# eaton-lab/tetrad

Hardware: AMD Instinct MI355X
Metric: resolved quartets/sec (whole node) (higher is better)
Workload: dtype u8 scan / u32 counts / f64 SVD; 1 GPU; c3: 128 taxa x 50000 SNPs, 1000000 random quartets, subsample_snps=True, results delivered to host arrays inside the step; quartets=1000000, taxa=128, snps=50000, subsample_snps=True, parallelism=one GPU, result D2H overlapped inside tq_resolve_to_host, launcher=none (one process)

## Files before the change

include/tetrad_hip.h:

```cpp
#ifndef TETRAD_HIP_H
#define TETRAD_HIP_H

#include <stdint.h>

#ifdef __cplusplus
extern "C" {
#endif

typedef struct tq_ctx tq_ctx;

enum {
    TQ_OK = 0,
    TQ_ERR_INVALID_ARG = -1,
    TQ_ERR_NO_DEVICE = -2,
    TQ_ERR_HIP = -3,
    TQ_ERR_NO_DATA = -4,
    TQ_ERR_LOCUS_ORDER = -5,
    TQ_ERR_OOM = -6
};

enum {
    TQ_FLAG_ZERO_DATA = 1,
    TQ_FLAG_DEGENERATE = 2,
    TQ_FLAG_BAD_INDEX = 4,
    TQ_FLAG_NO_CONVERGENCE = 8,
    TQ_FLAG_INVALID_DIAGNOSTIC = 16
};

int tq_create(tq_ctx **out, int device_id);
void tq_destroy(tq_ctx *ctx);
const char *tq_last_error(const tq_ctx *ctx);

int tq_set_data(tq_ctx *ctx, const uint8_t *tmparr, int64_t T, int64_t S,
                const uint32_t *locus, int64_t locus_stride);

int tq_set_source(tq_ctx *ctx, const uint8_t *seqarr, int64_t T, int64_t S0,
                  const int64_t *spans, int64_t nloci);
int tq_bootstrap(tq_ctx *ctx, const int64_t *lidxs, int64_t n, uint64_t seed_shuffle,
                 uint64_t seed_ambig, int64_t *out_S);
int tq_bootstrap_async(tq_ctx *ctx, const int64_t *lidxs, int64_t n, uint64_t seed_shuffle,
                       uint64_t seed_ambig, int64_t *out_S, void *stream);
int tq_get_data(tq_ctx *ctx, uint8_t *tmparr, uint32_t *tmpmap);
int tq_data_shape(tq_ctx *ctx, int64_t *T, int64_t *S);

int tq_resolve(tq_ctx *ctx, const uint32_t *quartets, int64_t Q, int subsample,
               uint32_t *rstat, double *rscor, uint8_t *flags);

int tq_host_alloc(int64_t bytes, void **out);
int tq_host_free(void *p);

int tq_resolve_to_host(tq_ctx *ctx, const uint32_t *d_quartets, int64_t Q, int subsample,
                       uint32_t *rstat, double *rscor, uint8_t *flags);

int tq_resolve_dev(tq_ctx *ctx, const uint32_t *d_quartets, int64_t Q, int subsample,
                   uint32_t *d_rstat, double *d_rscor, uint8_t *d_flags, void *stream);

int tq_resolve_range_dev(tq_ctx *ctx, uint64_t first_rank, int64_t Q, int subsample,
                         uint32_t *d_quartets, uint32_t *d_rstat, double *d_rscor,
                         uint8_t *d_flags, void *stream);

int tq_scan_dev(tq_ctx *ctx, const uint32_t *d_quartets, int64_t Q, int subsample, void *stream);
int tq_svd_dev(tq_ctx *ctx, int64_t q0, int64_t n, uint32_t *d_rstat, double *d_rscor,
               uint8_t *d_flags, void *stream);

int tq_unrank_dev(tq_ctx *ctx, const uint64_t *d_ranks, int64_t Q, uint32_t *d_quartets,
                  void *stream);

int tq_sample_quartets_dev(tq_ctx *ctx, uint64_t seed, int64_t Q, uint64_t *d_ranks,
                           uint32_t *d_quartets, void *stream);

int tq_resolve_debug(tq_ctx *ctx, const uint32_t *quartets, int64_t Q, int subsample,
                     uint32_t *rstat, double *rscor, uint8_t *flags,
                     uint32_t *cmats, double *svds, int32_t *ranks);

int tq_timing_enable(tq_ctx *ctx, int on);
int tq_timing_read(tq_ctx *ctx, double *kernel_ms, int64_t *launches);
int tq_timing_read_split(tq_ctx *ctx, double *total_ms, double *scan_ms, double *svd_ms, int64_t *calls);
int tq_timing_read_kernels(tq_ctx *ctx, double *ms, int n_ms, int64_t *calls);

int tq_set_option(tq_ctx *ctx, const char *name, int64_t value);

int tq_debug_fetch(tq_ctx *ctx, int which, void *dst, int64_t bytes);

int tq_debug_bdsqr(tq_ctx *ctx, const double *de, int64_t nmat, double *sv, uint32_t *work, int reps, double *ms);

int tq_format_tsv(const uint32_t *quartets, const uint32_t *rstat, const double *rscor, int64_t Q,
                  char *out, int64_t cap, int64_t *written);
int tq_format_qmc(const uint32_t *quartets, const uint32_t *rstat, const double *rscor, int64_t Q,
                  int weights, int64_t min_snps, double min_ratio, char *out, int64_t cap,
                  int64_t *written, int64_t *n_lines);

int tq_numpy_choice_tail(void *np_bitgen, uint64_t pop, int64_t size, int64_t *out);

int tq_unrank(const uint64_t *ranks, uint64_t first_rank, int64_t Q, int64_t T, uint32_t *quartets);

int tq_qmc_splits(const uint32_t *quartets, const uint32_t *rstat, const double *rscor, int64_t Q, int weights,
                  int64_t min_snps, double min_ratio, uint32_t *splits, double *weights_out, int64_t *n_rows);

int tq_qmc_tree(const uint32_t *splits, const double *weights, int64_t n, int64_t ntaxa, uint64_t seed,
                char *out, int64_t cap, int64_t *written);

typedef struct tq_conc tq_conc;
int tq_conc_create(tq_conc **out, const int32_t *parent, int64_t n_nodes, int64_t T, int64_t min_snps, double min_ratio,
                   tq_ctx *ctx);
void tq_conc_destroy(tq_conc *acc);
int tq_conc_reset(tq_conc *acc);
int tq_conc_add(tq_conc *acc, const uint32_t *quartets, const uint32_t *rstat, const double *rscor, const uint8_t *flags,
                int64_t n);
int tq_conc_add_dev(tq_conc *acc, const uint32_t *d_quartets, const uint32_t *d_rstat, const double *d_rscor,
                    const uint8_t *d_flags, int64_t n, void *stream);
int tq_conc_shape(const tq_conc *acc, int64_t *T, int64_t *n_edges, int64_t *mask_words);
int tq_conc_read(tq_conc *acc, int64_t *edge_counts, double *edge_sums, uint64_t *masks, int64_t *tip_counts,
                 int64_t *skipped);

typedef struct tq_stree tq_stree;
int tq_stree_create(tq_stree **out, int64_t ntaxa, int64_t capacity_rows, int weights, int64_t min_snps, double min_ratio,
                    tq_ctx *ctx);
void tq_stree_destroy(tq_stree *acc);
int tq_stree_reset(tq_stree *acc);
int tq_stree_add(tq_stree *acc, const uint32_t *quartets, const uint32_t *rstat, const double *rscor, const uint8_t *flags,
                 int64_t n);
int tq_stree_add_dev(tq_stree *acc, const uint32_t *d_quartets, const uint32_t *d_rstat, const double *d_rscor,
                     const uint8_t *d_flags, int64_t n, void *stream);
int tq_stree_graph(tq_stree *acc, uint64_t *G, uint64_t *B, int64_t *kept, int64_t *skipped, uint64_t *sum_k);
int tq_stree_rows(tq_stree *acc, uint32_t *splits, uint64_t *k, int64_t *n);
int tq_stree_build(tq_stree *acc, uint64_t seed, void *stream, char *out, int64_t cap, int64_t *written, int64_t *levels);
int tq_stree_level_stats(const tq_stree *acc, int64_t *n_levels, double *out);

int tq_set_species(tq_ctx *ctx, const int32_t *species_of, int64_t T, int64_t K);
int tq_resolve_species(tq_ctx *ctx, const uint32_t *squartets, int64_t Q, uint32_t *rstat, double *rscor,
                       uint8_t *flags);
int tq_resolve_species_dev(tq_ctx *ctx, const uint32_t *d_squartets, int64_t Q, uint32_t *d_rstat, double *d_rscor,
                           uint8_t *d_flags, void *stream);
int tq_resolve_species_debug(tq_ctx *ctx, const uint32_t *squartets, int64_t Q, uint32_t *rstat, double *rscor,
                             uint8_t *flags, uint32_t *cmats, double *svds, int32_t *ranks);

int tq_device_info(tq_ctx *ctx, int32_t *num_cu, int32_t *waves_per_cu, int64_t *row_pitch);

#ifdef __cplusplus
}
#endif
#endif
```

tetrad_amd/_lib.py:

```python
from __future__ import annotations

import ctypes
import os
import sys
import shutil
import subprocess
from pathlib import Path

CSRC = Path(__file__).resolve().parent / "csrc"
LIB_PATH = CSRC / "libtetrad_hip.so"
SRC_PATH = CSRC / "tetrad_hip.hip"
HEADER = Path(__file__).resolve().parents[1] / "include" / "tetrad_hip.h"

TQ_OK = 0
ERR_NAMES = {
    -1: "TQ_ERR_INVALID_ARG", -2: "TQ_ERR_NO_DEVICE", -3: "TQ_ERR_HIP",
    -4: "TQ_ERR_NO_DATA", -5: "TQ_ERR_LOCUS_ORDER", -6: "TQ_ERR_OOM",
}
FLAG_ZERO_DATA, FLAG_DEGENERATE, FLAG_BAD_INDEX, FLAG_NO_CONVERGENCE, FLAG_INVALID_DIAGNOSTIC = 1, 2, 4, 8, 16

SYMBOLS = [
    "tq_create", "tq_destroy", "tq_last_error", "tq_set_data", "tq_resolve",
    "tq_set_source", "tq_bootstrap", "tq_bootstrap_async", "tq_sample_quartets_dev", "tq_get_data", "tq_data_shape",
    "tq_host_alloc", "tq_host_free", "tq_resolve_to_host", "tq_scan_dev", "tq_svd_dev",
    "tq_resolve_dev", "tq_resolve_range_dev", "tq_unrank_dev", "tq_resolve_debug",
    "tq_timing_enable", "tq_timing_read", "tq_timing_read_split", "tq_timing_read_kernels",
    "tq_set_option", "tq_device_info", "tq_debug_fetch", "tq_debug_bdsqr",
    "tq_format_tsv", "tq_format_qmc", "tq_qmc_tree", "tq_qmc_splits", "tq_unrank", "tq_numpy_choice_tail",
    "tq_conc_create", "tq_conc_destroy", "tq_conc_reset", "tq_conc_add", "tq_conc_add_dev", "tq_conc_shape", "tq_conc_read",
    "tq_stree_create", "tq_stree_destroy", "tq_stree_reset", "tq_stree_add", "tq_stree_add_dev", "tq_stree_graph",
    "tq_stree_rows", "tq_stree_build", "tq_stree_level_stats",
    "tq_set_species", "tq_resolve_species", "tq_resolve_species_dev", "tq_resolve_species_debug",
]


class TetradHipError(RuntimeError):
    def __init__(self, code: int, message: str):
        self.code = code
        super().__init__(f"{ERR_NAMES.get(code, code)}: {message}")


def build(force: bool = False, verbose: bool = False) -> Path:
    hipcc = shutil.which("hipcc") or "/opt/rocm/bin/hipcc"
    sources = [SRC_PATH, HEADER, *CSRC.glob("*.hpp")]
    newest_src = max(p.stat().st_mtime for p in sources)
    if not force and LIB_PATH.exists() and LIB_PATH.stat().st_mtime >= newest_src:
        return LIB_PATH
    cmd = [hipcc, "-O3", "-std=c++17", "--offload-arch=gfx950", "-fPIC", "-shared", "-Wno-inline-asm",
           "-o", str(LIB_PATH), str(SRC_PATH)]
    if verbose:
        print(" ".join(cmd))
    subprocess.check_call(cmd)
    _stamp_commit()
    return LIB_PATH


def _stamp_commit() -> None:
    repo = CSRC.parents[1]
    try:
        head = subprocess.check_output(["git", "-C", str(repo), "rev-parse", "--short", "HEAD"],
                                       stderr=subprocess.DEVNULL).decode().strip()
        dirty = subprocess.check_output(["git", "-C", str(repo), "status", "--porcelain", "--untracked-files=no"],
                                        stderr=subprocess.DEVNULL).decode().strip()
        (repo / ".build_commit").write_text(head + ("+uncommitted" if dirty else "") + "\n")
    except Exception:
        pass


_lib = None
LOADED_PATH = None


def load() -> ctypes.CDLL:
    global _lib
    if _lib is not None:
        return _lib
    if not LIB_PATH.exists():
        raise ImportError(
            f"{LIB_PATH} is missing: run `python -c 'import __graft_entry__ as g; g.build()'` "
            "(hipcc, gfx950).  tetrad_amd has no CPU fallback.")
    try:
        import torch
    except ImportError:
        pass
    alt = os.environ.get("TQ_LIB_PATH")
    if alt:
        print(f"tetrad_amd: TQ_LIB_PATH is set -- loading {alt} instead of {LIB_PATH}", file=sys.stderr)
    global LOADED_PATH
    LOADED_PATH = alt if alt else str(LIB_PATH)
    lib = ctypes.CDLL(LOADED_PATH)
    c = ctypes
    vp, i64, i32 = c.c_void_p, c.c_int64, c.c_int
    lib.tq_create.argtypes = [c.POINTER(vp), i32]
    lib.tq_create.restype = i32
    lib.tq_destroy.argtypes = [vp]
    lib.tq_destroy.restype = None
    lib.tq_last_error.argtypes = [vp]
    lib.tq_last_error.restype = c.c_char_p
    lib.tq_set_data.argtypes = [vp, vp, i64, i64, vp, i64]
    lib.tq_set_data.restype = i32
    lib.tq_set_source.argtypes = [vp, vp, i64, i64, vp, i64]
    lib.tq_set_source.restype = i32
    lib.tq_bootstrap.argtypes = [vp, vp, i64, c.c_uint64, c.c_uint64, c.POINTER(i64)]
    lib.tq_bootstrap.restype = i32
    lib.tq_bootstrap_async.argtypes = [vp, vp, i64, c.c_uint64, c.c_uint64, c.POINTER(i64), vp]
    lib.tq_bootstrap_async.restype = i32
    lib.tq_sample_quartets_dev.argtypes = [vp, c.c_uint64, i64, vp, vp, vp]
    lib.tq_sample_quartets_dev.restype = i32
    lib.tq_get_data.argtypes = [vp, vp, vp]
    lib.tq_get_data.restype = i32
    lib.tq_data_shape.argtypes = [vp, c.POINTER(i64), c.POINTER(i64)]
    lib.tq_data_shape.restype = i32
    lib.tq_resolve.argtypes = [vp, vp, i64, i32, vp, vp, vp]
    lib.tq_resolve.restype = i32
    lib.tq_host_alloc.argtypes = [i64, c.POINTER(vp)]
    lib.tq_host_alloc.restype = i32
    lib.tq_host_free.argtypes = [vp]
    lib.tq_host_free.restype = i32
    lib.tq_resolve_to_host.argtypes = [vp, vp, i64, i32, vp, vp, vp]
    lib.tq_resolve_to_host.restype = i32
    lib.tq_scan_dev.argtypes = [vp, vp, i64, i32, vp]
    lib.tq_scan_dev.restype = i32
    lib.tq_svd_dev.argtypes = [vp, i64, i64, vp, vp, vp, vp]
    lib.tq_svd_dev.restype = i32
    lib.tq_timing_read_kernels.argtypes = [vp, c.POINTER(c.c_double), i32, c.POINTER(i64)]
    lib.tq_timing_read_kernels.restype = i32
    lib.tq_resolve_dev.argtypes = [vp, vp, i64, i32, vp, vp, vp, vp]
    lib.tq_resolve_dev.restype = i32
    lib.tq_resolve_range_dev.argtypes = [vp, c.c_uint64, i64, i32, vp, vp, vp, vp, vp]
    lib.tq_resolve_range_dev.restype = i32
    lib.tq_unrank_dev.argtypes = [vp, vp, i64, vp, vp]
    lib.tq_unrank_dev.restype = i32
    lib.tq_resolve_debug.argtypes = [vp, vp, i64, i32, vp, vp, vp, vp, vp, vp]
    lib.tq_resolve_debug.restype = i32
    lib.tq_timing_enable.argtypes = [vp, i32]
    lib.tq_timing_enable.restype = i32
    lib.tq_timing_read.argtypes = [vp, c.POINTER(c.c_double), c.POINTER(i64)]
    lib.tq_timing_read.restype = i32
    lib.tq_timing_read_split.argtypes = [vp, c.POINTER(c.c_double), c.POINTER(c.c_double),
                                         c.POINTER(c.c_double), c.POINTER(i64)]
    lib.tq_timing_read_split.restype = i32
    lib.tq_debug_fetch.argtypes = [vp, i32, vp, i64]
    lib.tq_debug_fetch.restype = i32
    lib.tq_debug_bdsqr.argtypes = [vp, vp, i64, vp, vp, i32, c.POINTER(c.c_double)]
    lib.tq_debug_bdsqr.restype = i32
    lib.tq_set_option.argtypes = [vp, c.c_char_p, i64]
    lib.tq_set_option.restype = i32
    lib.tq_format_tsv.argtypes = [vp, vp, vp, i64, vp, i64, c.POINTER(i64)]
    lib.tq_format_tsv.restype = i32
    lib.tq_format_qmc.argtypes = [vp, vp, vp, i64, i32, i64, c.c_double, vp, i64, c.POINTER(i64), c.POINTER(i64)]
    lib.tq_format_qmc.restype = i32
    lib.tq_qmc_splits.argtypes = [vp, vp, vp, i64, i32, i64, c.c_double, vp, vp, c.POINTER(i64)]
    lib.tq_qmc_splits.restype = i32
    lib.tq_numpy_choice_tail.argtypes = [vp, c.c_uint64, i64, vp]
    lib.tq_numpy_choice_tail.restype = i32
    lib.tq_unrank.argtypes = [vp, c.c_uint64, i64, i64, vp]
    lib.tq_unrank.restype = i32
    lib.tq_qmc_tree.argtypes = [vp, vp, i64, i64, c.c_uint64, vp, i64, c.POINTER(i64)]
    lib.tq_qmc_tree.restype = i32
    lib.tq_conc_create.argtypes = [c.POINTER(vp), vp, i64, i64, i64, c.c_double, vp]
    lib.tq_conc_create.restype = i32
    lib.tq_conc_destroy.argtypes = [vp]
    lib.tq_conc_destroy.restype = None
    lib.tq_conc_reset.argtypes = [vp]
    lib.tq_conc_reset.restype = i32
    lib.tq_conc_add.argtypes = [vp, vp, vp, vp, vp, i64]
    lib.tq_conc_add.restype = i32
    lib.tq_conc_add_dev.argtypes = [vp, vp, vp, vp, vp, i64, vp]
    lib.tq_conc_add_dev.restype = i32
    lib.tq_conc_shape.argtypes = [vp, c.POINTER(i64), c.POINTER(i64), c.POINTER(i64)]
    lib.tq_conc_shape.restype = i32
    lib.tq_conc_read.argtypes = [vp, vp, vp, vp, vp, c.POINTER(i64)]
    lib.tq_conc_read.restype = i32
    lib.tq_stree_create.argtypes = [c.POINTER(vp), i64, i64, i32, i64, c.c_double, vp]
    lib.tq_stree_create.restype = i32
    lib.tq_stree_destroy.argtypes = [vp]
    lib.tq_stree_destroy.restype = None
    lib.tq_stree_reset.argtypes = [vp]
    lib.tq_stree_reset.restype = i32
    lib.tq_stree_add.argtypes = [vp, vp, vp, vp, vp, i64]
    lib.tq_stree_add.restype = i32
    lib.tq_stree_add_dev.argtypes = [vp, vp, vp, vp, vp, i64, vp]
    lib.tq_stree_add_dev.restype = i32
    lib.tq_stree_graph.argtypes = [vp, vp, vp, c.POINTER(i64), c.POINTER(i64), c.POINTER(c.c_uint64)]
    lib.tq_stree_graph.restype = i32
    lib.tq_stree_rows.argtypes = [vp, vp, vp, c.POINTER(i64)]
    lib.tq_stree_rows.restype = i32
    lib.tq_stree_build.argtypes = [vp, c.c_uint64, vp, vp, i64, c.POINTER(i64), c.POINTER(i64)]
    lib.tq_stree_build.restype = i32
    lib.tq_stree_level_stats.argtypes = [vp, c.POINTER(i64), vp]
    lib.tq_stree_level_stats.restype = i32
    lib.tq_set_species.argtypes = [vp, vp, i64, i64]
    lib.tq_set_species.restype = i32
    lib.tq_resolve_species.argtypes = [vp, vp, i64, vp, vp, vp]
    lib.tq_resolve_species.restype = i32
    lib.tq_resolve_species_dev.argtypes = [vp, vp, i64, vp, vp, vp, vp]
    lib.tq_resolve_species_dev.restype = i32
    lib.tq_resolve_species_debug.argtypes = [vp, vp, i64, vp, vp, vp, vp, vp, vp]
    lib.tq_resolve_species_debug.restype = i32
    lib.tq_device_info.argtypes = [vp, c.POINTER(c.c_int32), c.POINTER(c.c_int32), c.POINTER(i64)]
    lib.tq_device_info.restype = i32
    _lib = lib
    return lib
```

tetrad_amd/csrc/prepare.hpp:

```cpp
#pragma once

__device__ __forceinline__ void store_planes3(uint32_t *planes3, uint32_t *runbeg, int64_t t, int64_t W, int64_t w,
                                              uint32_t mm, uint32_t b0, uint32_t b1, uint32_t rb)
{
    uint32_t *p3 = planes3 + (t * W + w) * 3;
    p3[0] = mm;
    p3[1] = b0;
    p3[2] = b1;
    if (t == 0) runbeg[w] = rb;
}

__global__ void tq_prepare_rows(const uint8_t *__restrict__ raw, const uint32_t *__restrict__ locus,
                                int64_t S, int64_t Sp, int64_t W, int32_t T, uint8_t *__restrict__ rows,
                                uint8_t *__restrict__ nib, uint8_t *__restrict__ nib5, uint4 *__restrict__ planes,
                                uint32_t *__restrict__ planes3, uint32_t *__restrict__ runbeg)
{
    int64_t gid = (int64_t)blockIdx.x * blockDim.x + threadIdx.x;
    if (gid >= (int64_t)T * W) return;
    int64_t t = gid / W, w = gid - t * W;
    const uint8_t *src = raw + t * S + w * 32;
    uint8_t *dst = rows + t * Sp;
    uint32_t mm = 0, b0 = 0, b1 = 0, rb = 0;
    uint32_t nw[4] = {0, 0, 0, 0}, n5[4] = {0, 0, 0, 0};
    for (int i = 0; i < 32; ++i) {
        int64_t s = w * 32 + i;
        uint8_t v = (s < S) ? src[i] : (uint8_t)0xFF;
        bool missing = v > 3;
        uint8_t code = missing ? (uint8_t)0 : v;
        dst[row_offset(s)] = code;
        nw[i >> 3] |= (uint32_t)code << (8 * (i & 3) + 4 * ((i >> 2) & 1));
        n5[i >> 3] |= (uint32_t)(missing ? 4 : code) << (8 * (i & 3) + 4 * ((i >> 2) & 1));
        mm |= (uint32_t)missing << i;
        b0 |= (uint32_t)(code & 1) << i;
        b1 |= (uint32_t)((code >> 1) & 1) << i;
        if (s < S) {
            bool beg = (s == 0) || (locus[s] != locus[s - 1]);
            rb |= (uint32_t)beg << i;
        }
    }
    planes[t * W + w] = make_uint4(mm, b0, b1, rb);
    store_planes3(planes3, runbeg, t, W, w, mm, b0, b1, rb);
    reinterpret_cast<uint4 *>(nib + t * (Sp / 2))[w] = make_uint4(nw[0], nw[1], nw[2], nw[3]);
    reinterpret_cast<uint4 *>(nib5 + t * (Sp / 2))[w] = make_uint4(n5[0], n5[1], n5[2], n5[3]);
}

__device__ __forceinline__ uint64_t choose_k(uint64_t n, int k)
{
    switch (k) {
    case 0: return 1;
    case 1: return n;
    case 2: return n < 2 ? 0 : n * (n - 1) / 2;
    default: return n < 3 ? 0 : n * (n - 1) / 2 * (n - 2) / 3;
    }
}

__global__ void tq_unrank_kernel(const uint64_t *__restrict__ ranks, uint64_t first_rank, int64_t Q,
                                 int32_t T, uint32_t *__restrict__ quartets)
{
    int64_t i = (int64_t)blockIdx.x * blockDim.x + threadIdx.x;
    if (i >= Q) return;
    uint64_t index = ranks ? ranks[i] : first_rank + (uint64_t)i;
    uint32_t out[4] = {0, 0, 0, 0};
    int nsel = 0;
    for (int t = 0; t < T && nsel < 4; ++t) {
        uint64_t c = choose_k((uint64_t)(T - t - 1), 4 - nsel - 1);
        if (c > index) {
            out[nsel++] = (uint32_t)t;
        } else {
            index -= c;
        }
    }
    uint4 v = make_uint4(out[0], out[1], out[2], out[3]);
    reinterpret_cast<uint4 *>(quartets)[i] = v;
}

__global__ void tq_key_kernel(const uint32_t *__restrict__ quartets, int64_t Q, uint32_t T, int with_c,
                              uint32_t *__restrict__ keys, uint32_t *__restrict__ idx)
{
    int64_t i = (int64_t)blockIdx.x * blockDim.x + threadIdx.x;
    if (i >= Q) return;
    const uint4 q = reinterpret_cast<const uint4 *>(quartets)[i];
    const uint32_t a = q.x < T ? q.x : T - 1, b = q.y < T ? q.y : T - 1, c = q.z < T ? q.z : T - 1;
    const uint32_t ab = a * T + b;
    keys[i] = with_c ? ab * T + c : ab;
    idx[i] = (uint32_t)i;
}


__device__ __forceinline__ uint32_t feistel_round(uint32_t x, uint32_t key)
{
    x ^= key;
    x *= 0x7FEB352Du;
    x ^= x >> 15;
    x *= 0x846CA68Bu;
    x ^= x >> 16;
    return x;
}

struct FeistelKeys {
    uint32_t k[6];
};

__device__ __forceinline__ FeistelKeys feistel_keys(uint64_t seed)
{
    FeistelKeys ks;
    uint64_t x = seed;
#pragma unroll
    for (int r = 0; r < 6; ++r) {
        x += 0x9E3779B97F4A7C15ull;
        uint64_t z = x;
        z = (z ^ (z >> 30)) * 0xBF58476D1CE4E5B9ull;
        z = (z ^ (z >> 27)) * 0x94D049BB133111EBull;
        z ^= z >> 31;
        ks.k[r] = (uint32_t)(z >> 16);
    }
    return ks;
}

__device__ __forceinline__ uint64_t feistel_permute(uint64_t v, int half_bits, const FeistelKeys &ks)
{
    const uint32_t mask = half_bits >= 32 ? 0xFFFFFFFFu : ((1u << half_bits) - 1u);
    uint32_t L = (uint32_t)(v >> half_bits) & mask, R = (uint32_t)v & mask;
#pragma unroll
    for (int r = 0; r < 6; ++r) {
        const uint32_t t = L ^ (feistel_round(R, ks.k[r]) & mask);
        L = R;
        R = t;
    }
    return ((uint64_t)L << half_bits) | (uint64_t)R;
}

__global__ void tq_sample_kernel(uint64_t seed, uint64_t N, int half_bits, int64_t Q, int32_t T,
                                 uint64_t *__restrict__ ranks_out, uint32_t *__restrict__ quartets)
{
    int64_t i = (int64_t)blockIdx.x * blockDim.x + threadIdx.x;
    if (i >= Q) return;
    const FeistelKeys ks = feistel_keys(seed);
    uint64_t v = (uint64_t)i;
    do {
        v = feistel_permute(v, half_bits, ks);
    } while (v >= N);
    if (ranks_out) ranks_out[i] = v;
    uint64_t index = v;
    uint32_t out[4] = {0, 0, 0, 0};
    int nsel = 0;
    for (int t = 0; t < T && nsel < 4; ++t) {
        uint64_t c = choose_k((uint64_t)(T - t - 1), 4 - nsel - 1);
        if (c > index) {
            out[nsel++] = (uint32_t)t;
        } else {
            index -= c;
        }
    }
    reinterpret_cast<uint4 *>(quartets)[i] = make_uint4(out[0], out[1], out[2], out[3]);
}
```

tetrad_amd/csrc/tetrad_hip.hip:

```cpp
#include <hip/hip_runtime.h>
#include <hipcub/hipcub.hpp>

#include <algorithm>
#include <chrono>
#include <cmath>
#include <cstdarg>
#include <cstdlib>
#include <utility>
#include <cstdint>
#include <cstdio>
#include <cstring>
#include <map>
#include <mutex>
#include <new>
#include <string>
#include <unordered_map>
#include <unordered_set>
#include <vector>

#include "../../include/tetrad_hip.h"

namespace {

#include "common.hpp"
#include "prepare.hpp"
#include "scan.hpp"
#include "scan_pb.hpp"
#include "scan_dp.hpp"
#include "scan_f4.hpp"
#include "jacobi.hpp"
#include "hqr.hpp"
#include "bootstrap.hpp"
#include "format.hpp"
#include "qmc.hpp"
#include "concordance.hpp"
#include "species.hpp"
#include "supertree.hpp"

}

enum { TAG_ORIGIN = -1, TAG_ORDER = 0, TAG_SCAN = 1, TAG_BIDIAG = 2, TAG_BDSQR = 3, TAG_SCORE = 4, TAG_COUNT = 5 };

struct tq_ctx {
    int device = 0;
    std::string err;
    hipDeviceProp_t prop{};
    int64_t T = 0, S = 0, Sp = 0, W = 0;
    uint8_t *d_rows = nullptr;
    uint8_t *d_nib = nullptr;
    uint8_t *d_nib5 = nullptr;
    uint4 *d_planes = nullptr;
    uint32_t *d_planes3 = nullptr;
    bool have_data = false;
    bool locus_runs_ok = false;
    int64_t plane_cap_W = 0;
    int64_t data_capacity = 0;
    uint8_t *d_seqarr = nullptr;
    int64_t *d_spans = nullptr;
    int64_t src_T = 0, src_S0 = 0, nloci = 0, max_width = 0;
    int64_t *d_lidxs = nullptr;
    std::vector<int64_t> h_spans;
    int64_t *h_lidx_stage[2] = {nullptr, nullptr};
    hipEvent_t ev_lidx[2] = {nullptr, nullptr};
    unsigned lidx_turn = 0;
    uint32_t *d_boot = nullptr;
    int64_t boot_cap = 0;
    void *d_boot_tmp = nullptr;
    size_t boot_tmp_bytes = 0;
    void *d_scratch = nullptr;
    size_t scratch_bytes = 0;
    uint32_t *d_cm = nullptr;
    int64_t cm_quartets = 0;
    uint32_t *d_sort = nullptr;
    void *d_sort_tmp = nullptr;
    size_t sort_tmp_bytes = 0;
    int order = 1;
    uint2 *d_units = nullptr;
    int scan_f4 = -1;
    int scan_dp = 1;
    int64_t dp_min_quartets = 32768;
    double *d_de = nullptr, *d_sv = nullptr;
    uint32_t *d_nsnps = nullptr;
    int64_t svd_quartets = 0;
    int64_t svd_chunk = 1 << 18;
    int svd_streams = 2;
    hipStream_t sX = nullptr;
    hipEvent_t evFork = nullptr, evJoin = nullptr;
    int svd_method = 1;
    int bidiag_layout = 1;
    int bdsqr_maxit = 60;
    uint64_t *d_bdsqr_stats = nullptr;
    int scan_wg = 4;
    int64_t wg_min_quartets = 4096;
    int xcd_remap = 1;
    int count_invariant = 0;
    int scan_pair = 0;
    int park_t = 1;
    int share_c = 0;
    int svd_wpc = 0;
    int stree_lds = 1;
    const uint32_t *scanned_q = nullptr;
    int64_t scanned_Q = 0;
    int64_t scanned_T = 0;
    int64_t sp_T = 0, sp_K = 0;
    std::vector<int32_t> sp_size;
    uint64_t sp_bound = 0;
    int32_t sp_max = 0;
    int32_t *d_sp_members = nullptr;
    uint32_t *d_sp_tab = nullptr;
    int64_t sp_tab_cap = 0;
    int species_method = -1;
    uint64_t data_gen = 0;
    uint64_t sp_tab_gen = ~0ull;
    hipStream_t sK = nullptr, sC = nullptr;
    std::vector<hipEvent_t> pipe_events;
    hipEvent_t evDevApi = nullptr;
    bool dev_api_pending = false;
    hipStream_t last_dev_stream = nullptr;
    int nrep = 1;
    int waves_per_cu = 0;
    int phases = 3;
    int scan_method = -1;
    int pb_ok = 0;
    int64_t batch = 1 << 23;
    bool timing = false;
    struct Mark { int tag; int lane; hipEvent_t ev; };
    std::vector<Mark> marks;
    std::vector<hipEvent_t> event_pool;
    int64_t timed_calls = 0;
};

namespace {

std::string g_create_err;

int fail(tq_ctx *ctx, int code, const char *fmt, ...)
{
    char buf[512];
    va_list ap;
    va_start(ap, fmt);
    vsnprintf(buf, sizeof buf, fmt, ap);
    va_end(ap);
    try {
        if (ctx) ctx->err = buf; else g_create_err = buf;
    } catch (...) {
    }
    return code;
}

#define TQ_HIP(ctx, call)                                                                     \
    do {                                                                                      \
        hipError_t e_ = (call);                                                               \
        if (e_ != hipSuccess)                                                                 \
            return fail(ctx, e_ == hipErrorOutOfMemory ? TQ_ERR_OOM : TQ_ERR_HIP, "%s failed: %s", \
                        #call, hipGetErrorString(e_));                                        \
    } while (0)

struct PinnedPool {
    std::mutex mu;
    std::map<uintptr_t, size_t> live;
    std::multimap<size_t, void *> idle;
    size_t idle_bytes = 0;
    static constexpr size_t IDLE_CAP = (size_t)4 << 30;
    static size_t round_up(size_t b)
    {
        size_t g = (size_t)1 << 16;
        while (g < b && g < ((size_t)1 << 24)) g <<= 1;
        if (g >= b) return g;
        const size_t step = (size_t)1 << 24;
        return (b + step - 1) / step * step;
    }
    int alloc(size_t bytes, void **out)
    {
        const size_t want = round_up(bytes ? bytes : 1);
        std::lock_guard<std::mutex> g(mu);
        try {
            auto it = idle.lower_bound(want);
            if (it != idle.end() && it->first <= want * 2) {
                void *p = it->second;
                const size_t sz = it->first;
                idle.erase(it);
                idle_bytes -= sz;
                live[(uintptr_t)p] = sz;
                *out = p;
                return TQ_OK;
            }
            void *p = nullptr;
            if (hipHostMalloc(&p, want, hipHostMallocPortable) != hipSuccess || !p) return TQ_ERR_OOM;
            live[(uintptr_t)p] = want;
            *out = p;
            return TQ_OK;
        } catch (...) {
            return TQ_ERR_OOM;
        }
    }
    int release(void *p)
    {
        std::lock_guard<std::mutex> g(mu);
        auto it = live.find((uintptr_t)p);
        if (it == live.end()) return TQ_ERR_INVALID_ARG;
        const size_t sz = it->second;
        live.erase(it);
        bool cached = false;
        if (idle_bytes + sz <= IDLE_CAP) {
            try {
                idle.emplace(sz, p);
                idle_bytes += sz;
                cached = true;
            } catch (...) {
            }
        }
        if (!cached) (void)hipHostFree(p);
        return TQ_OK;
    }
    bool owns(const void *p, size_t bytes)
    {
        std::lock_guard<std::mutex> g(mu);
        auto it = live.upper_bound((uintptr_t)p);
        if (it == live.begin()) return false;
        --it;
        return (uintptr_t)p + bytes <= it->first + it->second;
    }
};

PinnedPool &pool()
{
    static PinnedPool *p = new PinnedPool();
    return *p;
}

bool is_pinned(const void *p, size_t bytes)
{
    if (!p) return false;
    if (pool().owns(p, bytes)) return true;
    hipPointerAttribute_t a{};
    if (hipPointerGetAttributes(&a, p) != hipSuccess) {
        (void)hipGetLastError();
        return false;
    }
    return a.type == hipMemoryTypeHost;
}

void free_data(tq_ctx *ctx)
{
    if (ctx->d_rows) (void)hipFree(ctx->d_rows);
    if (ctx->d_nib) (void)hipFree(ctx->d_nib);
    if (ctx->d_nib5) (void)hipFree(ctx->d_nib5);
    if (ctx->d_planes) (void)hipFree(ctx->d_planes);
    if (ctx->d_planes3) (void)hipFree(ctx->d_planes3);
    ctx->d_rows = nullptr;
    ctx->d_nib = nullptr;
    ctx->d_nib5 = nullptr;
    ctx->d_planes = nullptr;
    ctx->d_planes3 = nullptr;
    ctx->have_data = false;
    ctx->data_capacity = 0;
    ctx->scanned_Q = 0;
}

void free_source(tq_ctx *ctx)
{
    if (ctx->d_seqarr) (void)hipFree(ctx->d_seqarr);
    if (ctx->d_spans) (void)hipFree(ctx->d_spans);
    if (ctx->d_lidxs) (void)hipFree(ctx->d_lidxs);
    if (ctx->d_boot) (void)hipFree(ctx->d_boot);
    if (ctx->d_boot_tmp) (void)hipFree(ctx->d_boot_tmp);
    ctx->d_seqarr = nullptr;
    ctx->d_spans = nullptr;
    ctx->d_lidxs = nullptr;
    ctx->d_boot = nullptr;
    ctx->d_boot_tmp = nullptr;
    ctx->boot_cap = 0;
    ctx->nloci = 0;
    for (int i = 0; i < 2; ++i) {
        if (ctx->h_lidx_stage[i]) (void)pool().release(ctx->h_lidx_stage[i]);
        if (ctx->ev_lidx[i]) (void)hipEventDestroy(ctx->ev_lidx[i]);
        ctx->h_lidx_stage[i] = nullptr;
        ctx->ev_lidx[i] = nullptr;
    }
}

int ensure_scratch(tq_ctx *ctx, size_t bytes)
{
    if (bytes <= ctx->scratch_bytes) return TQ_OK;
    if (ctx->d_scratch) (void)hipFree(ctx->d_scratch);
    ctx->d_scratch = nullptr;
    ctx->scratch_bytes = 0;
    TQ_HIP(ctx, hipMalloc(&ctx->d_scratch, bytes));
    ctx->scratch_bytes = bytes;
    return TQ_OK;
}

int ensure_cm(tq_ctx *ctx, int64_t quartets)
{
    if (quartets <= ctx->cm_quartets) return TQ_OK;
    if (ctx->d_cm) (void)hipFree(ctx->d_cm);
    if (ctx->d_sort) (void)hipFree(ctx->d_sort);
    if (ctx->d_sort_tmp) (void)hipFree(ctx->d_sort_tmp);
    if (ctx->d_units) (void)hipFree(ctx->d_units);
    ctx->d_cm = nullptr;
    ctx->d_sort = nullptr;
    ctx->d_sort_tmp = nullptr;
    ctx->d_units = nullptr;
    ctx->cm_quartets = 0;
    ctx->scanned_Q = 0;
    TQ_HIP(ctx, hipMalloc((void **)&ctx->d_cm, (size_t)quartets * 1024));
    TQ_HIP(ctx, hipMalloc((void **)&ctx->d_sort, (size_t)quartets * 16));
    size_t tmp = 0;
    uint32_t *k = ctx->d_sort;
    TQ_HIP(ctx, hipcub::DeviceRadixSort::SortPairs(nullptr, tmp, k, k, k, k, (int)quartets));
    size_t tmp2 = 0;
    TQ_HIP(ctx, hipcub::DeviceScan::InclusiveSum(nullptr, tmp2, k, k, (int)quartets));
    if (tmp2 > tmp) tmp = tmp2;
    TQ_HIP(ctx, hipMalloc(&ctx->d_sort_tmp, tmp ? tmp : 16));
    TQ_HIP(ctx, hipMalloc((void **)&ctx->d_units, ((size_t)quartets + 2) * sizeof(uint2)));
    ctx->sort_tmp_bytes = tmp;
    ctx->cm_quartets = quartets;
    return TQ_OK;
}

int ensure_svd(tq_ctx *ctx, int64_t quartets)
{
    if (!ctx->sX) {
        TQ_HIP(ctx, hipStreamCreateWithFlags(&ctx->sX, hipStreamNonBlocking));
        TQ_HIP(ctx, hipEventCreateWithFlags(&ctx->evFork, hipEventDisableTiming));
        TQ_HIP(ctx, hipEventCreateWithFlags(&ctx->evJoin, hipEventDisableTiming));
    }
    if (quartets <= ctx->svd_quartets) return TQ_OK;
    if (ctx->d_de) (void)hipFree(ctx->d_de);
    if (ctx->d_sv) (void)hipFree(ctx->d_sv);
    if (ctx->d_nsnps) (void)hipFree(ctx->d_nsnps);
    ctx->d_de = ctx->d_sv = nullptr;
    ctx->d_nsnps = nullptr;
    ctx->svd_quartets = 0;
    TQ_HIP(ctx, hipMalloc((void **)&ctx->d_de, 2 * (size_t)quartets * 3 * 32 * sizeof(double)));
    TQ_HIP(ctx, hipMalloc((void **)&ctx->d_sv, 2 * (size_t)quartets * 3 * 16 * sizeof(double)));
    TQ_HIP(ctx, hipMalloc((void **)&ctx->d_nsnps, 2 * (size_t)quartets * sizeof(uint32_t)));
    ctx->svd_quartets = quartets;
    return TQ_OK;
}

int mark(tq_ctx *ctx, int tag, hipStream_t stream, int lane = 0)
{
    if (!ctx->timing) return TQ_OK;
    hipEvent_t ev;
    if (!ctx->event_pool.empty()) {
        ev = ctx->event_pool.back();
        ctx->event_pool.pop_back();
    } else {
        TQ_HIP(ctx, hipEventCreate(&ev));
    }
    try {
        ctx->marks.push_back({tag, lane, ev});
    } catch (...) {
        (void)hipEventDestroy(ev);
        return fail(ctx, TQ_ERR_OOM, "out of host memory");
    }
    TQ_HIP(ctx, hipEventRecord(ev, stream));
    return TQ_OK;
}

int make_order(tq_ctx *ctx, const uint32_t *dq, int64_t n, bool input_sorted, hipStream_t stream,
               const uint32_t **order)
{
    *order = nullptr;
    if (!ctx->order || n < 32768 || ctx->T > 65535 || input_sorted) return TQ_OK;
    uint32_t *keys_in = ctx->d_sort, *idx_in = keys_in + ctx->cm_quartets;
    uint32_t *keys_out = idx_in + ctx->cm_quartets, *idx_out = keys_out + ctx->cm_quartets;
    const uint64_t T = (uint64_t)ctx->T;
    const int with_c = T * T * T <= 0xFFFFFFFFull;
    hipLaunchKernelGGL(tq_key_kernel, dim3((unsigned)((n + 255) / 256)), dim3(256), 0, stream, dq, n,
                       (uint32_t)ctx->T, with_c, keys_in, idx_in);
    TQ_HIP(ctx, hipGetLastError());
    int bits = 1;
    while (bits < 32 && (1ull << bits) < (with_c ? T * T * T : T * T)) ++bits;
    size_t tmp = ctx->sort_tmp_bytes;
    TQ_HIP(ctx, hipcub::DeviceRadixSort::SortPairs(ctx->d_sort_tmp, tmp, keys_in, keys_out, idx_in, idx_out, (int)n,
                                                   0, bits, stream));
    *order = idx_out;
    return TQ_OK;
}

bool use_dp(const tq_ctx *ctx, int64_t n, int subsample, bool input_sorted)
{
    const uint64_t T = (uint64_t)ctx->T;
    return !subsample && ctx->scan_dp && ctx->scan_f4 <= 0 && ctx->scan_method < 0 && ctx->scan_wg == 4 && !ctx->count_invariant &&
           !ctx->share_c && !ctx->scan_pair && ctx->waves_per_cu == 0 && (ctx->order || input_sorted) &&
           n >= ctx->dp_min_quartets && n >= 2 && n <= 0x7FFFFFFF && T * T * T <= 0xFFFFFFFFull &&
           T * (uint64_t)ctx->Sp < 0xFFFF0000ull;
}

int make_units(tq_ctx *ctx, const uint32_t *dq, int64_t n, bool input_sorted, hipStream_t stream)
{
    uint32_t *keys_in = ctx->d_sort, *idx_in = keys_in + ctx->cm_quartets;
    uint32_t *keys_out = idx_in + ctx->cm_quartets, *idx_out = keys_out + ctx->cm_quartets;
    const uint64_t T = (uint64_t)ctx->T;
    const unsigned blocks = (unsigned)((n + 255) / 256);
    hipLaunchKernelGGL(tq_key_kernel, dim3(blocks), dim3(256), 0, stream, dq, n, (uint32_t)ctx->T, 1, keys_in, idx_in);
    TQ_HIP(ctx, hipGetLastError());
    const uint32_t *keys = keys_in, *idx = idx_in;
    uint32_t *flags = keys_out;
    if (!input_sorted) {
        int bits = 1;
        while (bits < 32 && (1ull << bits) < T * T * T) ++bits;
        size_t tmp = ctx->sort_tmp_bytes;
        TQ_HIP(ctx, hipcub::DeviceRadixSort::SortPairs(ctx->d_sort_tmp, tmp, keys_in, keys_out, idx_in, idx_out, (int)n,
                                                       0, bits, stream));
        keys = keys_out;
        idx = idx_out;
        flags = keys_in;
    }
    hipLaunchKernelGGL(tq_dp_flag_kernel, dim3(blocks), dim3(256), 0, stream, keys, idx, dq, n, (uint32_t)ctx->T, flags);
    TQ_HIP(ctx, hipGetLastError());
    size_t tmp = ctx->sort_tmp_bytes;
    TQ_HIP(ctx, hipcub::DeviceScan::InclusiveSum(ctx->d_sort_tmp, tmp, flags, flags, (int)n, stream));
    hipLaunchKernelGGL(tq_dp_units_kernel, dim3(blocks), dim3(256), 0, stream, keys, idx, (const uint32_t *)flags, n,
                       ctx->d_units, reinterpret_cast<uint32_t *>(ctx->d_units + ctx->cm_quartets));
    TQ_HIP(ctx, hipGetLastError());
    return TQ_OK;
}

DevData dev_data(const tq_ctx *ctx)
{
    DevData d;
    d.rows = ctx->d_rows;
    d.nib = ctx->d_nib;
    d.nib5 = ctx->d_nib5;
    d.planes = ctx->d_planes;
    d.planes3 = ctx->d_planes3;
    d.runbeg = ctx->d_planes3 + (size_t)ctx->T * (size_t)ctx->plane_cap_W * 3;
    d.pitch = ctx->Sp;
    d.W = ctx->W;
    d.T = (int32_t)ctx->T;
    d.ntiles = (int32_t)(ctx->Sp / TILE);
    d.inv = ctx->count_invariant ? 0xFFFFFFFFu : 0u;
    return d;
}

template <typename K>
int grid_for(tq_ctx *ctx, K kern, int64_t items, int64_t *grid, int wpc_kernel = 0)
{
    int wpc = wpc_kernel > 0 ? wpc_kernel : ctx->waves_per_cu;
    if (wpc <= 0) {
        int nb = 0;
        TQ_HIP(ctx, hipOccupancyMaxActiveBlocksPerMultiprocessor(&nb, kern, WAVE, 0));
        wpc = nb > 0 ? nb : 8;
    }
    int64_t g = (int64_t)ctx->prop.multiProcessorCount * wpc;
    if (g > items) g = items;
    if (g < 1) g = 1;
    *grid = g;
    return TQ_OK;
}

template <int NREP, bool SUB, int METHOD>
int launch_scan(tq_ctx *ctx, const uint32_t *dq, const uint32_t *order, int64_t Q, hipStream_t stream)
{
    auto kern = tq_scan_kernel<NREP, SUB, METHOD>;
    int64_t grid;
    int rc = grid_for(ctx, kern, Q, &grid);
    if (rc) return rc;
    hipLaunchKernelGGL(kern, dim3((unsigned)grid), dim3(WAVE), 0, stream, dev_data(ctx), dq, order, Q, ctx->d_cm);
    TQ_HIP(ctx, hipGetLastError());
    return TQ_OK;
}

template <bool SUB, int METHOD, int NW, bool SHC = false, bool PARK_T = false>
int launch_scan_wg(tq_ctx *ctx, const uint32_t *dq, const uint32_t *order, int64_t Q, hipStream_t stream)
{
    auto kern = tq_scan_wg_kernel<SUB, METHOD, NW, SHC, PARK_T>;
    const int wgs = ctx->waves_per_cu > 0 ? (ctx->waves_per_cu + NW - 1) / NW : 0;
    const int64_t nblk = (Q + NW - 1) / NW;
    int64_t grid = wgs > 0 ? (int64_t)ctx->prop.multiProcessorCount * wgs : nblk;
    int64_t xcd_chunk = 0;
    if (grid >= nblk) {
        grid = nblk;
        if (ctx->xcd_remap && nblk >= 64) {
            xcd_chunk = (nblk + 7) / 8;
            grid = xcd_chunk * 8;
        }
    }
    if (grid < 1) grid = 1;
    hipLaunchKernelGGL(kern, dim3((unsigned)grid), dim3(NW * WAVE), 0, stream, dev_data(ctx), dq, order, Q,
                       ctx->d_cm, xcd_chunk);
    TQ_HIP(ctx, hipGetLastError());
    return TQ_OK;
}

template <bool SUB>
int launch_scan_pb(tq_ctx *ctx, const uint32_t *dq, const uint32_t *order, int64_t Q, hipStream_t stream)
{
    auto kern = tq_scan_pb_kernel<SUB>;
    const int64_t nblk = (Q + PB_NW - 1) / PB_NW;
    int64_t grid = nblk, xcd_chunk = 0;
    if (ctx->xcd_remap && nblk >= 64) {
        xcd_chunk = (nblk + 7) / 8;
        grid = xcd_chunk * 8;
    }
    if (grid < 1) grid = 1;
    hipLaunchKernelGGL(kern, dim3((unsigned)grid), dim3(PB_NW * WAVE), 0, stream, dev_data(ctx), dq, order, Q, ctx->d_cm,
                       xcd_chunk, (uint32_t *)nullptr);
    TQ_HIP(ctx, hipGetLastError());
    return TQ_OK;
}

int probe_scan_pb(tq_ctx *ctx)
{
    uint32_t *d = nullptr, h[2] = {0, 0};
    TQ_HIP(ctx, hipMalloc(&d, sizeof h));
    hipError_t e = hipMemset(d, 0, sizeof h);
    if (e == hipSuccess) {
        DevData none{};
        hipLaunchKernelGGL(tq_scan_pb_kernel<false>, dim3(1), dim3(PB_NW * WAVE), 0, 0, none, (const uint32_t *)nullptr,
                           (const uint32_t *)nullptr, (int64_t)-1, (uint32_t *)nullptr, (int64_t)0, d);
        hipLaunchKernelGGL(tq_scan_pb_kernel<true>, dim3(1), dim3(PB_NW * WAVE), 0, 0, none, (const uint32_t *)nullptr,
                           (const uint32_t *)nullptr, (int64_t)-1, (uint32_t *)nullptr, (int64_t)0, d + 1);
        e = hipGetLastError();
    }
    if (e == hipSuccess) e = hipMemcpy(h, d, sizeof h, hipMemcpyDeviceToHost);
    (void)hipFree(d);
    if (e != hipSuccess) return fail(ctx, TQ_ERR_HIP, "probe of tq_scan_pb_kernel failed: %s", hipGetErrorString(e));
    ctx->pb_ok = (h[0] == 0x80000000u && h[1] == 0x80000000u) ? 1 : -1;
    return TQ_OK;
}

template <bool SUB, int METHOD, int NW>
int launch_scan_wg2(tq_ctx *ctx, const uint32_t *dq, const uint32_t *order, int64_t Q, hipStream_t stream)
{
    auto kern = tq_scan_wg2_kernel<SUB, METHOD, NW>;
    const int64_t nblk = (Q + 2 * NW - 1) / (2 * NW);
    int64_t grid = nblk, xcd_chunk = 0;
    if (ctx->xcd_remap && nblk >= 64) {
        xcd_chunk = (nblk + 7) / 8;
        grid = xcd_chunk * 8;
    }
    if (grid < 1) grid = 1;
    hipLaunchKernelGGL(kern, dim3((unsigned)grid), dim3(NW * WAVE), 0, stream, dev_data(ctx), dq, order, Q, ctx->d_cm,
                       xcd_chunk);
    TQ_HIP(ctx, hipGetLastError());
    return TQ_OK;
}

int launch_scan_dp(tq_ctx *ctx, const uint32_t *dq, int64_t Q, hipStream_t stream)
{
    const int64_t least = ((Q + 1) / 2 + DP_NW - 1) / DP_NW;
    const int64_t grid = (least + 7) / 8 * 8;
    hipLaunchKernelGGL(tq_scan_dp_kernel<DP_NW>, dim3((unsigned)grid), dim3(DP_NW * WAVE), 0, stream, dev_data(ctx), dq,
                       (const uint2 *)ctx->d_units, reinterpret_cast<const uint32_t *>(ctx->d_units + ctx->cm_quartets),
                       ctx->d_cm);
    TQ_HIP(ctx, hipGetLastError());
    return TQ_OK;
}

int launch_scan_n(tq_ctx *ctx, const uint32_t *dq, const uint32_t *order, int64_t Q, int subsample,
                  hipStream_t stream)
{
    if (ctx->scan_pair && ctx->scan_wg == 4 && Q >= 64 && !ctx->count_invariant && !ctx->share_c && ctx->waves_per_cu == 0 &&
        ctx->scan_method < 2 && (uint64_t)ctx->T * (uint64_t)ctx->Sp < 0xFFFF0000ull) {
        const int m = ctx->scan_method < 0 ? (subsample ? 1 : 0) : ctx->scan_method;
        if (subsample)
            return m ? launch_scan_wg2<true, 1, 4>(ctx, dq, order, Q, stream) : launch_scan_wg2<true, 0, 4>(ctx, dq, order, Q, stream);
        return m ? launch_scan_wg2<false, 1, 4>(ctx, dq, order, Q, stream) : launch_scan_wg2<false, 0, 4>(ctx, dq, order, Q, stream);
    }
    const bool f4 = ctx->scan_f4 < 0 ? (subsample != 0 && ctx->scan_method < 0 && ctx->park_t) : ctx->scan_f4 != 0;
    if (f4 && (ctx->scan_wg == 4 || ctx->scan_wg == 8 || ctx->scan_wg == 2) && Q >= ctx->wg_min_quartets && !ctx->count_invariant &&
        !ctx->share_c && !ctx->scan_pair && ctx->waves_per_cu == 0 && (ctx->scan_method < 0 || ctx->scan_method == 1) &&
        (uint64_t)ctx->T * (uint64_t)ctx->Sp < 0xFFFF0000ull) {
        const int nw = ctx->scan_wg;
        const int64_t nblk = (Q + nw - 1) / nw;
        int64_t grid = nblk, xcd_chunk = 0;
        if (ctx->xcd_remap && nblk >= 64) {
            xcd_chunk = (nblk + 7) / 8;
            grid = xcd_chunk * 8;
        }
#define TQ_F4_CASE(SUBF, NWF)                                                                                         \
        if ((subsample != 0) == SUBF && nw == NWF)                                                                    \
            hipLaunchKernelGGL((tq_scan_f4_kernel<SUBF, NWF>), dim3((unsigned)grid), dim3(NWF * WAVE), 0, stream,      \
                               dev_data(ctx), dq, order, Q, ctx->d_cm, xcd_chunk);
        TQ_F4_CASE(true, 4) TQ_F4_CASE(false, 4) TQ_F4_CASE(true, 8) TQ_F4_CASE(false, 8) TQ_F4_CASE(true, 2) TQ_F4_CASE(false, 2)
#undef TQ_F4_CASE
        TQ_HIP(ctx, hipGetLastError());
        return TQ_OK;
    }
    const bool pb_fits = ctx->pb_ok == 1 && ctx->scan_wg == 4 && Q >= 64 && !ctx->count_invariant && !ctx->share_c &&
                         !ctx->scan_pair && ctx->waves_per_cu == 0 && ctx->Sp / TILE <= PB_MAX_TILES &&
                         (uint64_t)ctx->T * (uint64_t)ctx->Sp < 0xFFFF0000ull;
    if (pb_fits && ctx->scan_method == 6)
        return subsample ? launch_scan_pb<true>(ctx, dq, order, Q, stream) : launch_scan_pb<false>(ctx, dq, order, Q, stream);
    if (ctx->scan_wg >= 2 && Q >= ctx->wg_min_quartets && !ctx->count_invariant &&
        (uint64_t)ctx->T * (uint64_t)ctx->Sp < 0xFFFF0000ull) {
        int m = ctx->scan_method < 0 ? (subsample ? 1 : 0) : ctx->scan_method;
        if (m == 6) m = subsample ? 1 : 0;
#define TQ_WG_CASE(NW)                                                                                   \
    if (ctx->scan_wg == NW) {                                                                            \
        if (m == 2) return launch_scan_wg<true, 2, NW>(ctx, dq, order, Q, stream);                       \
        if (m == 3) return launch_scan_wg<true, 3, NW>(ctx, dq, order, Q, stream);                       \
        if (NW == 4 && m == 4) return launch_scan_wg<true, 4, 4>(ctx, dq, order, Q, stream);             \
        if (NW == 4 && m == 5) return launch_scan_wg<true, 5, 4>(ctx, dq, order, Q, stream);             \
        if (subsample)                                                                                   \
            return m ? launch_scan_wg<true, 1, NW>(ctx, dq, order, Q, stream)                            \
                     : launch_scan_wg<true, 0, NW>(ctx, dq, order, Q, stream);                           \
        return m ? launch_scan_wg<false, 1, NW>(ctx, dq, order, Q, stream)                               \
                 : launch_scan_wg<false, 0, NW>(ctx, dq, order, Q, stream);                              \
    }
        TQ_WG_CASE(2)
        if (ctx->scan_wg == 4 && ctx->park_t && m == 1 && !ctx->share_c)
            return subsample ? launch_scan_wg<true, 1, 4, false, true>(ctx, dq, order, Q, stream)
                             : launch_scan_wg<false, 1, 4, false, true>(ctx, dq, order, Q, stream);
        if ((ctx->scan_wg == 8 || ctx->scan_wg == 6) && ctx->park_t && m == 1 && subsample && !ctx->share_c)
            return ctx->scan_wg == 8 ? launch_scan_wg<true, 1, 8, false, true>(ctx, dq, order, Q, stream)
                                     : launch_scan_wg<true, 1, 6, false, true>(ctx, dq, order, Q, stream);
        if (ctx->scan_wg == 4 && ctx->share_c && m <= 1) {
            if (subsample)
                return m ? launch_scan_wg<true, 1, 4, true>(ctx, dq, order, Q, stream)
                         : launch_scan_wg<true, 0, 4, true>(ctx, dq, order, Q, stream);
            return m ? launch_scan_wg<false, 1, 4, true>(ctx, dq, order, Q, stream)
                     : launch_scan_wg<false, 0, 4, true>(ctx, dq, order, Q, stream);
        }
        TQ_WG_CASE(4)
        TQ_WG_CASE(3)
        TQ_WG_CASE(6)
        TQ_WG_CASE(16)
        TQ_WG_CASE(8)
#undef TQ_WG_CASE
    }
#define TQ_SCAN_CASE(N)                                                                              \
    case N:                                                                                          \
        if (method == 0)                                                                             \
            return subsample ? launch_scan<N, true, 0>(ctx, dq, order, Q, stream)                    \
                             : launch_scan<N, false, 0>(ctx, dq, order, Q, stream);                  \
        return subsample ? launch_scan<N, true, 1>(ctx, dq, order, Q, stream)                        \
                         : launch_scan<N, false, 1>(ctx, dq, order, Q, stream)
    const int method = (ctx->scan_method < 0 || ctx->scan_method == 6) ? (subsample ? 1 : 0) : ctx->scan_method;
    switch (ctx->nrep) {
        TQ_SCAN_CASE(2);
        TQ_SCAN_CASE(4);
        TQ_SCAN_CASE(8);
        TQ_SCAN_CASE(16);
        TQ_SCAN_CASE(32);
    default:
        TQ_SCAN_CASE(1);
    }
#undef TQ_SCAN_CASE
}

template <bool DEBUG>
int launch_svd(tq_ctx *ctx, const uint32_t *cm, const uint32_t *dq, int64_t n, const OutPtrs &out, hipStream_t stream,
               int lane)
{
    auto kern = tq_svd_kernel<DEBUG>;
    int64_t grid;
    int rc = grid_for(ctx, kern, (n + QPW - 1) / QPW, &grid);
    if (rc) return rc;
    hipLaunchKernelGGL(kern, dim3((unsigned)grid), dim3(WAVE), 0, stream, cm, dq, n, (int32_t)ctx->scanned_T, out);
    TQ_HIP(ctx, hipGetLastError());
    return mark(ctx, TAG_BIDIAG, stream, lane);
}

template <bool DEBUG>
int launch_hqr(tq_ctx *ctx, const uint32_t *cm, const uint32_t *dq, int64_t n, const OutPtrs &out, hipStream_t stream,
               int lane)
{
    double *de = ctx->d_de + (size_t)lane * (size_t)ctx->svd_quartets * 96;
    double *sv = ctx->d_sv + (size_t)lane * (size_t)ctx->svd_quartets * 48;
    uint32_t *nsnps = ctx->d_nsnps + (size_t)lane * (size_t)ctx->svd_quartets;
    int64_t grid;
    auto k1 = ctx->bidiag_layout ? tq_bidiag2_kernel<DEBUG> : tq_bidiag_kernel<DEBUG>;
    const int svd_wpc = ctx->svd_wpc > 0 ? ctx->svd_wpc : (1 << 20);
    const int tsplit = n < 32768 ? 1 : 0;
    int rc = grid_for(ctx, k1, (tsplit ? 3 : 1) * ((n + 15) / 16), &grid, svd_wpc);
    if (rc) return rc;
    hipLaunchKernelGGL(k1, dim3((unsigned)grid), dim3(WAVE), 0, stream, cm, n, de, nsnps, out.cmats, tsplit);
    TQ_HIP(ctx, hipGetLastError());
    if ((rc = mark(ctx, TAG_BIDIAG, stream, lane))) return rc;
    const int64_t nmat = 3 * n;
    rc = grid_for(ctx, tq_bdsqr_kernel, (nmat + WAVE - 1) / WAVE, &grid, svd_wpc);
    if (rc) return rc;
    hipLaunchKernelGGL(tq_bdsqr_kernel, dim3((unsigned)grid), dim3(WAVE), 0, stream, (const double *)de, nmat, sv,
                       ctx->bdsqr_maxit, (unsigned long long *)ctx->d_bdsqr_stats);
    TQ_HIP(ctx, hipGetLastError());
    if ((rc = mark(ctx, TAG_BDSQR, stream, lane))) return rc;
    hipLaunchKernelGGL(tq_score_kernel<DEBUG>, dim3((unsigned)((n + 255) / 256)), dim3(256), 0, stream,
                       (const double *)sv, (const uint32_t *)nsnps, dq, n, (int32_t)ctx->scanned_T, out);
    TQ_HIP(ctx, hipGetLastError());
    return mark(ctx, TAG_SCORE, stream, lane);
}

bool diagnostic_mode(const tq_ctx *ctx)
{
    return (ctx->scan_method >= 2 && ctx->scan_method <= 5) || ctx->phases != 3;
}

OutPtrs offset_out(const OutPtrs &o, int64_t q0)
{
    OutPtrs r = o;
    r.rstat = o.rstat + q0 * 2;
    r.rscor = o.rscor + q0 * 3;
    r.flags = o.flags ? o.flags + q0 : nullptr;
    r.cmats = o.cmats ? o.cmats + q0 * 768 : nullptr;
    r.svds = o.svds ? o.svds + q0 * 48 : nullptr;
    r.ranks = o.ranks ? o.ranks + q0 * 3 : nullptr;
    return r;
}

int check_ready(tq_ctx *ctx, int subsample)
{
    if (!ctx->have_data) return fail(ctx, TQ_ERR_NO_DATA, "tq_set_data has not been called");
    if (subsample && !ctx->locus_runs_ok)
        return fail(ctx, TQ_ERR_LOCUS_ORDER,
                    "subsample mode needs each locus id in one contiguous run of sites (and no id 0xFFFFFFFF)");
    return TQ_OK;
}

int stage_scan(tq_ctx *ctx, const uint32_t *dq, int64_t n, int subsample, bool input_sorted, hipStream_t stream)
{
    int rc = ensure_cm(ctx, n);
    if (rc) return rc;
    ctx->scanned_Q = 0;
    if ((rc = mark(ctx, TAG_ORIGIN, stream))) return rc;
    if (ctx->phases & 1) {
        if (use_dp(ctx, n, subsample, input_sorted)) {
            rc = make_units(ctx, dq, n, input_sorted, stream);
            if (rc) return rc;
            if ((rc = mark(ctx, TAG_ORDER, stream))) return rc;
            rc = launch_scan_dp(ctx, dq, n, stream);
        } else {
            const uint32_t *order = nullptr;
            rc = make_order(ctx, dq, n, input_sorted, stream, &order);
            if (rc) return rc;
            if ((rc = mark(ctx, TAG_ORDER, stream))) return rc;
            rc = launch_scan_n(ctx, dq, order, n, subsample, stream);
        }
        if (rc) return rc;
        if ((rc = mark(ctx, TAG_SCAN, stream))) return rc;
    }
    ctx->scanned_q = dq;
    ctx->scanned_Q = n;
    ctx->scanned_T = ctx->T;
    return TQ_OK;
}

int species_ready(tq_ctx *ctx, const char *who)
{
    if (!ctx->have_data) return fail(ctx, TQ_ERR_NO_DATA, "%s: tq_set_data has not been called", who);
    if (!ctx->sp_K) return fail(ctx, TQ_ERR_NO_DATA, "%s: no species map (call tq_set_species first)", who);
    if (ctx->sp_T != ctx->T)
        return fail(ctx, TQ_ERR_INVALID_ARG, "%s: the species map covers T=%lld samples, the resident replicate has T=%lld",
                    who, (long long)ctx->sp_T, (long long)ctx->T);
    if ((unsigned __int128)ctx->S * ctx->sp_bound >= ((unsigned __int128)1 << 32))
        return fail(ctx, TQ_ERR_INVALID_ARG,
                    "%s: pooled counts may exceed u32: S=%lld x product of the four largest species sizes %llu >= 2^32",
                    who, (long long)ctx->S, (unsigned long long)ctx->sp_bound);
    if (ctx->species_method == 1 && ctx->sp_max > SPECIES_MFMA_MAX)
        return fail(ctx, TQ_ERR_INVALID_ARG, "%s: species_method 1 (MFMA, i8 operands) takes species of at most %d lineages, "
                    "the map has one of %d", who, SPECIES_MFMA_MAX, (int)ctx->sp_max);
    return TQ_OK;
}

int stage_species(tq_ctx *ctx, const uint32_t *dsq, int64_t n, hipStream_t stream)
{
    int rc = ensure_cm(ctx, n);
    if (rc) return rc;
    ctx->scanned_Q = 0;
    if ((rc = mark(ctx, TAG_ORIGIN, stream))) return rc;
    if (ctx->sp_tab_gen != ctx->data_gen) {
        const int64_t entries = ctx->sp_K * ctx->Sp;
        if (entries > ctx->sp_tab_cap) {
            if (ctx->d_sp_tab) {
                TQ_HIP(ctx, hipDeviceSynchronize());
                (void)hipFree(ctx->d_sp_tab);
            }
            ctx->d_sp_tab = nullptr;
            ctx->sp_tab_cap = 0;
            TQ_HIP(ctx, hipMalloc((void **)&ctx->d_sp_tab, (size_t)entries * 8));
            ctx->sp_tab_cap = entries;
        }
        hipLaunchKernelGGL(tq_species_table_kernel, dim3((unsigned)((entries + 255) / 256)), dim3(256), 0, stream,
                           (const uint8_t *)ctx->d_nib5, ctx->Sp, ctx->S, (const int32_t *)(ctx->d_sp_members + ctx->sp_K + 1),
                           (const int32_t *)ctx->d_sp_members, (int32_t)ctx->sp_K, ctx->d_sp_tab,
                           (uint8_t *)(ctx->d_sp_tab + entries));
        TQ_HIP(ctx, hipGetLastError());
        ctx->sp_tab_gen = ctx->data_gen;
    }
    if ((rc = mark(ctx, TAG_ORDER, stream))) return rc;
    const bool mfma = ctx->species_method == 1 || (ctx->species_method < 0 && ctx->sp_max <= SPECIES_MFMA_MAX);
    const int32_t *offsets = ctx->d_sp_members;
    if (mfma)
        hipLaunchKernelGGL(tq_species_mfma_kernel, dim3((unsigned)n), dim3(WAVE * SPECIES_WAVES), 0, stream,
                           (const uint8_t *)(ctx->d_sp_tab + ctx->sp_K * ctx->Sp), ctx->Sp, ctx->S, dsq, n,
                           (int32_t)ctx->sp_K, offsets, ctx->d_cm);
    else
        hipLaunchKernelGGL(tq_species_pool_kernel, dim3((unsigned)n), dim3(WAVE * SPECIES_WAVES), 0, stream,
                           (const uint32_t *)ctx->d_sp_tab, ctx->Sp, ctx->S, dsq, n, (int32_t)ctx->sp_K, offsets, ctx->d_cm);
    TQ_HIP(ctx, hipGetLastError());
    if ((rc = mark(ctx, TAG_SCAN, stream))) return rc;
    ctx->scanned_q = dsq;
    ctx->scanned_Q = n;
    ctx->scanned_T = ctx->sp_K;
    return TQ_OK;
}

int64_t svd_chunk_rows(const tq_ctx *ctx, int64_t n)
{
    int64_t chunk = ctx->svd_chunk < n ? ctx->svd_chunk : n;
    if (ctx->svd_streams > 1 && n >= 65536 && n < 2 * ctx->svd_chunk && chunk > (n + 1) / 2) chunk = (n + 1) / 2;
    return chunk < 1 ? 1 : chunk;
}

template <typename F>
int stage_svd(tq_ctx *ctx, int64_t q0, int64_t n, bool debug, const OutPtrs &out, hipStream_t stream, F &&after_chunk)
{
    if (q0 < 0 || n < 0 || q0 + n > ctx->scanned_Q)
        return fail(ctx, TQ_ERR_INVALID_ARG, "rows [%lld,+%lld) are outside the scanned batch of %lld quartets",
                    (long long)q0, (long long)n, (long long)ctx->scanned_Q);
    const int64_t chunk = svd_chunk_rows(ctx, n);
    int rc = ensure_svd(ctx, chunk);
    if (rc) return rc;
    const bool diag = diagnostic_mode(ctx);
    if (diag && !out.flags)
        return fail(ctx, TQ_ERR_INVALID_ARG, "a timing-diagnostic mode is set (scan_method 2..5 or phases 1 / 2): its rows are "
                                             "not results and are only handed out with a flags array (TQ_FLAG_INVALID_DIAGNOSTIC)");
    const bool two = ctx->svd_streams > 1 && n > chunk;
    if (two) {
        TQ_HIP(ctx, hipEventRecord(ctx->evFork, stream));
        TQ_HIP(ctx, hipStreamWaitEvent(ctx->sX, ctx->evFork, 0));
    }
    int64_t ci = 0;
    for (int64_t c0 = 0; c0 < n; c0 += chunk, ++ci) {
        const int64_t cn = (n - c0) < chunk ? (n - c0) : chunk;
        const int lane = two ? (int)(ci & 1) : 0;
        hipStream_t st = lane ? ctx->sX : stream;
        if (!(ctx->phases & 2)) {
            if (hipMemsetAsync(out.flags + c0, TQ_FLAG_INVALID_DIAGNOSTIC, (size_t)cn, st) != hipSuccess) {
                rc = fail(ctx, TQ_ERR_HIP, "hipMemsetAsync(flags) failed");
                break;
            }
        }
        if (ctx->phases & 2) {
            const uint32_t *cm = ctx->d_cm + (size_t)(q0 + c0) * 256;
            const uint32_t *dq = ctx->scanned_q + (q0 + c0) * 4;
            OutPtrs o = offset_out(out, c0);
            o.flag_or = diag ? (uint32_t)TQ_FLAG_INVALID_DIAGNOSTIC : 0u;
            if ((rc = mark(ctx, TAG_ORIGIN, st, lane))) break;
            if (ctx->svd_method == 0)
                rc = debug ? launch_svd<true>(ctx, cm, dq, cn, o, st, lane) : launch_svd<false>(ctx, cm, dq, cn, o, st, lane);
            else
                rc = debug ? launch_hqr<true>(ctx, cm, dq, cn, o, st, lane) : launch_hqr<false>(ctx, cm, dq, cn, o, st, lane);
            if (rc) break;
        }
        if ((rc = after_chunk(c0, cn, st))) break;
    }
    if (two) {
        if (hipEventRecord(ctx->evJoin, ctx->sX) != hipSuccess || hipStreamWaitEvent(stream, ctx->evJoin, 0) != hipSuccess)
            if (!rc) rc = fail(ctx, TQ_ERR_HIP, "stream join failed");
    }
    return rc;
}

struct NoChunkHook {
    int operator()(int64_t, int64_t, hipStream_t) const { return TQ_OK; }
};

template <typename F>
int launch(tq_ctx *ctx, const uint32_t *dq, int64_t Q, int subsample, bool debug, bool input_sorted,
           const OutPtrs &out, hipStream_t stream, F &&after_chunk, bool species = false)
{
    int rc = species ? species_ready(ctx, "species resolve") : check_ready(ctx, subsample);
    if (rc) return rc;
    if (Q == 0) return TQ_OK;
    if (ctx->timing) ctx->timed_calls++;
    const int64_t batch = Q < ctx->batch ? Q : ctx->batch;
    for (int64_t q0 = 0; q0 < Q; q0 += batch) {
        const int64_t n = (Q - q0) < batch ? (Q - q0) : batch;
        rc = species ? stage_species(ctx, dq + q0 * 4, n, stream) : stage_scan(ctx, dq + q0 * 4, n, subsample, input_sorted, stream);
        if (rc) return rc;
        rc = stage_svd(ctx, 0, n, debug, offset_out(out, q0), stream,
                       [&](int64_t c0, int64_t cn, hipStream_t st) { return after_chunk(q0 + c0, cn, st); });
        if (rc) return rc;
    }
    ctx->scanned_Q = 0;
    return TQ_OK;
}

size_t align_up(size_t v, size_t a) { return (v + a - 1) / a * a; }

int ensure_streams(tq_ctx *ctx)
{
    if (!ctx->sK) {
        TQ_HIP(ctx, hipStreamCreateWithFlags(&ctx->sK, hipStreamNonBlocking));
        TQ_HIP(ctx, hipStreamCreateWithFlags(&ctx->sC, hipStreamNonBlocking));
    }
    if (ctx->dev_api_pending) {
        TQ_HIP(ctx, hipStreamWaitEvent(ctx->sK, ctx->evDevApi, 0));
        ctx->dev_api_pending = false;
    }
    return TQ_OK;
}

int enter_dev_api(tq_ctx *ctx, hipStream_t stream)
{
    if (ctx->dev_api_pending && ctx->evDevApi && stream != ctx->last_dev_stream)
        TQ_HIP(ctx, hipStreamWaitEvent(stream, ctx->evDevApi, 0));
    return TQ_OK;
}

int note_dev_api(tq_ctx *ctx, hipStream_t stream, int rc)
{
    if (!ctx->evDevApi) TQ_HIP(ctx, hipEventCreateWithFlags(&ctx->evDevApi, hipEventDisableTiming));
    TQ_HIP(ctx, hipEventRecord(ctx->evDevApi, stream));
    ctx->dev_api_pending = true;
    ctx->last_dev_stream = stream;
    return rc;
}

int pipe_event(tq_ctx *ctx, size_t i, hipEvent_t *ev)
{
    try {
        while (ctx->pipe_events.size() <= i) {
            hipEvent_t e;
            TQ_HIP(ctx, hipEventCreateWithFlags(&e, hipEventDisableTiming));
            ctx->pipe_events.push_back(e);
        }
    } catch (...) {
        return fail(ctx, TQ_ERR_OOM, "out of host memory");
    }
    *ev = ctx->pipe_events[i];
    return TQ_OK;
}

struct HostSink {
    tq_ctx *ctx;
    uint32_t *rstat;
    double *rscor;
    uint8_t *flags;
    const OutPtrs *dev;
// ... 246 lines not shown
            hipLaunchKernelGGL((tq_conc_kernel<true, 128, 128>), dim3(G), dim3(CONC_THREADS), 0, stream, a);
        } else if (t.T <= 256) {
            hipLaunchKernelGGL((tq_conc_kernel<true, 256, 256>), dim3(G), dim3(CONC_THREADS), 0, stream, a);
        } else {
            for (int32_t e0 = 0; e0 < t.E || e0 == 0; e0 += CONC_EDGE_TILE) {
                a.e_lo = e0;
                a.e_n = std::min<int32_t>(CONC_EDGE_TILE, t.E - e0);
                a.tips = e0 == 0;
                hipLaunchKernelGGL((tq_conc_kernel<false, CONC_T_MAX, CONC_EDGE_TILE>), dim3(G), dim3(CONC_THREADS), 0,
                                   stream, a);
            }
        }
        hipLaunchKernelGGL(tq_conc_fold_kernel, dim3((unsigned)((acc->words + CONC_THREADS - 1) / CONC_THREADS)),
                           dim3(CONC_THREADS), 0, stream, (const uint64_t *)acc->d_slab, G, acc->words, t.E, acc->d_tot);
        const hipError_t e = hipGetLastError();
        if (e != hipSuccess) return fail(ctx, TQ_ERR_HIP, "tq_conc_add_dev: launch failed: %s", hipGetErrorString(e));
    }
    return TQ_OK;
}

int conc_wait(tq_conc *acc)
{
    if (!acc->pending) return TQ_OK;
    TQ_HIP(acc->ctx, hipSetDevice(acc->ctx->device));
    TQ_HIP(acc->ctx, hipEventSynchronize(acc->ev));
    acc->pending = false;
    return TQ_OK;
}

}

struct tq_stree {
    tq_ctx *ctx = nullptr;
    int64_t ntaxa = 0, capacity = 0;
    int weights = 0;
    uint32_t min_snps = 1;
    double min_ratio = 1.0;
    int mode = 0;
    int64_t rows_in = 0;
    std::vector<uint64_t> h_t, h_k;
    int64_t h_skipped = 0;
    unsigned __int128 h_sum = 0;
    uint64_t *d_root_t = nullptr, *d_root_k = nullptr;
    uint64_t *d_wt[2] = {nullptr, nullptr}, *d_wk[2] = {nullptr, nullptr};
    uint32_t *d_wn[2] = {nullptr, nullptr};
    unsigned long long *d_cnt = nullptr, *d_mat = nullptr;
    StreeNode *d_nodes = nullptr;
    uint32_t *d_map = nullptr;
    uint64_t *p_mat = nullptr;
    StreeNode *p_nodes = nullptr;
    uint32_t *p_map = nullptr;
    unsigned long long *p_cnt = nullptr;
    int64_t max_cells = 0, max_nodes = 0;
    int num_cu = 1;
    hipEvent_t ev = nullptr;
    bool pending = false;
    hipStream_t last = nullptr;
    hipStream_t own = nullptr;
    std::vector<StreeLevelStat> stats;
};

namespace {

void stree_free_dev(tq_stree *a)
{
    void *dev[] = {a->d_root_t, a->d_root_k, a->d_wt[0], a->d_wt[1], a->d_wk[0], a->d_wk[1], a->d_wn[0], a->d_wn[1],
                   a->d_cnt, a->d_mat, a->d_nodes, a->d_map};
    for (void *p : dev)
        if (p) (void)hipFree(p);
    void *pin[] = {a->p_mat, a->p_nodes, a->p_map, a->p_cnt};
    for (void *p : pin)
        if (p) (void)hipHostFree(p);
    if (a->ev) (void)hipEventDestroy(a->ev);
    if (a->own) (void)hipStreamDestroy(a->own);
}

#define STREE_HIP(call)                                                                       \
    do {                                                                                      \
        hipError_t e_ = (call);                                                               \
        if (e_ != hipSuccess) {                                                               \
            err = std::string(#call) + " failed: " + hipGetErrorString(e_);                   \
            return e_ == hipErrorOutOfMemory ? TQ_ERR_OOM : TQ_ERR_HIP;                       \
        }                                                                                     \
    } while (0)

struct StreeDevBackend : StreeBackend {
    tq_stree *a = nullptr;
    hipStream_t st = nullptr;
    int cur = -1;
    int64_t n_live = 0;

    void fill(StreePassArgs &p) const
    {
        p.t4 = cur < 0 ? a->d_root_t : a->d_wt[cur];
        p.k = cur < 0 ? a->d_root_k : a->d_wk[cur];
        p.node = cur < 0 ? nullptr : a->d_wn[cur];
        p.n_live = &a->d_cnt[cur < 0 ? SC_KEPT : SC_LIVE0 + cur];
        p.nodes = a->d_nodes;
        p.mat = a->d_mat;
    }
    int begin(int64_t &live, std::string &err) override
    {
        STREE_HIP(hipMemcpyAsync(a->p_cnt, a->d_cnt, SC_WORDS * 8, hipMemcpyDeviceToHost, st));
        STREE_HIP(hipStreamSynchronize(st));
        cur = -1;
        live = n_live = (int64_t)a->p_cnt[SC_KEPT];
        return TQ_OK;
    }
    int graphs(const std::vector<StreeNode> &nodes, int64_t cells, int, const uint64_t *&mat, std::string &err) override
    {
        if (cells > a->max_cells || (int64_t)nodes.size() > a->max_nodes) {
            err = "a level exceeds the cells or nodes the accumulator was created for";
            return TQ_ERR_INVALID_ARG;
        }
        memcpy(a->p_nodes, nodes.data(), nodes.size() * sizeof(StreeNode));
        STREE_HIP(hipMemcpyAsync(a->d_nodes, a->p_nodes, nodes.size() * sizeof(StreeNode), hipMemcpyHostToDevice, st));
        STREE_HIP(hipMemsetAsync(a->d_mat, 0, (size_t)(2 * cells) * 8, st));
        StreePassArgs p{};
        fill(p);
        p.n_nodes = (int32_t)nodes.size();
        p.cells = cells;
        if (a->ctx->stree_lds && cells <= STREE_LDS_CELLS && n_live >= 4096) {
            const int pairs = (int)std::max<int64_t>(1, std::min<int64_t>((n_live + 16383) / 16384, 64));
            hipLaunchKernelGGL(tq_stree_graph_lds_kernel, dim3(2 * pairs), dim3(STREE_LDS_THREADS), 0, st, p);
        } else {
            const int G = (int)std::max<int64_t>(1, std::min<int64_t>((n_live + STREE_THREADS - 1) / STREE_THREADS,
                                                                     8 * (int64_t)a->num_cu));
            hipLaunchKernelGGL(tq_stree_graph_kernel, dim3(G), dim3(STREE_THREADS), 0, st, p);
        }
        STREE_HIP(hipGetLastError());
        STREE_HIP(hipMemcpyAsync(a->p_mat, a->d_mat, (size_t)(2 * cells) * 8, hipMemcpyDeviceToHost, st));
        STREE_HIP(hipStreamSynchronize(st));
        mat = a->p_mat;
        return TQ_OK;
    }
    int partition(const std::vector<StreeNode> &nodes, const std::vector<uint32_t> &map, int, int64_t &live,
                  std::string &err) override
    {
        if ((int64_t)nodes.size() > a->max_nodes || (int64_t)map.size() > 3 * a->max_nodes) {
            err = "a level exceeds the nodes the accumulator was created for";
            return TQ_ERR_INVALID_ARG;
        }
        const int dst = cur < 0 ? 0 : cur ^ 1;
        memcpy(a->p_nodes, nodes.data(), nodes.size() * sizeof(StreeNode));
        memcpy(a->p_map, map.data(), map.size() * 4);
        STREE_HIP(hipMemcpyAsync(a->d_nodes, a->p_nodes, nodes.size() * sizeof(StreeNode), hipMemcpyHostToDevice, st));
        STREE_HIP(hipMemcpyAsync(a->d_map, a->p_map, map.size() * 4, hipMemcpyHostToDevice, st));
        STREE_HIP(hipMemsetAsync(&a->d_cnt[SC_LIVE0 + dst], 0, 8, st));
        StreePassArgs p{};
        fill(p);
        p.n_nodes = (int32_t)nodes.size();
        p.map = a->d_map;
        p.out_t4 = a->d_wt[dst];
        p.out_k = a->d_wk[dst];
        p.out_node = a->d_wn[dst];
        p.out_live = &a->d_cnt[SC_LIVE0 + dst];
        const int G = (int)std::max<int64_t>(1, std::min<int64_t>((n_live + STREE_THREADS - 1) / STREE_THREADS,
                                                                 8 * (int64_t)a->num_cu));
        hipLaunchKernelGGL(tq_stree_partition_kernel, dim3(G), dim3(STREE_THREADS), 0, st, p);
        STREE_HIP(hipGetLastError());
        STREE_HIP(hipMemcpyAsync(&a->p_cnt[SC_LIVE0 + dst], &a->d_cnt[SC_LIVE0 + dst], 8, hipMemcpyDeviceToHost, st));
        STREE_HIP(hipStreamSynchronize(st));
        cur = dst;
        live = n_live = (int64_t)a->p_cnt[SC_LIVE0 + dst];
        return TQ_OK;
    }
};

int stree_join(tq_stree *acc, hipStream_t st)
{
    TQ_HIP(acc->ctx, hipSetDevice(acc->ctx->device));
    if (acc->pending && st != acc->last) TQ_HIP(acc->ctx, hipStreamWaitEvent(st, acc->ev, 0));
    return TQ_OK;
}

int stree_counts(tq_stree *acc, hipStream_t st, int64_t &kept, int64_t &skipped, unsigned __int128 &sum)
{
    if (acc->mode == 2) {
        if (int rc = stree_join(acc, st)) return rc;
        TQ_HIP(acc->ctx, hipMemcpyAsync(acc->p_cnt, acc->d_cnt, SC_WORDS * 8, hipMemcpyDeviceToHost, st));
        TQ_HIP(acc->ctx, hipStreamSynchronize(st));
        kept = (int64_t)acc->p_cnt[SC_KEPT];
        skipped = (int64_t)acc->p_cnt[SC_SKIPPED];
        sum = (unsigned __int128)acc->p_cnt[SC_SUM_LO] + ((unsigned __int128)acc->p_cnt[SC_SUM_HI] << 32);
    } else {
        kept = (int64_t)acc->h_t.size();
        skipped = acc->h_skipped;
        sum = acc->h_sum;
    }
    return TQ_OK;
}

}

extern "C" {

int tq_create(tq_ctx **out, int device_id)
{
    if (!out) return fail(nullptr, TQ_ERR_INVALID_ARG, "tq_create: out is NULL");
    *out = nullptr;
    int n = 0;
    hipError_t e = hipGetDeviceCount(&n);
    if (e != hipSuccess || n <= 0)
        return fail(nullptr, TQ_ERR_NO_DEVICE, "no HIP device available (%s)", hipGetErrorString(e));
    if (device_id < 0 || device_id >= n)
        return fail(nullptr, TQ_ERR_INVALID_ARG, "device_id %d out of range (0..%d)", device_id, n - 1);
    tq_ctx *ctx = new (std::nothrow) tq_ctx();
    if (!ctx) return fail(nullptr, TQ_ERR_OOM, "out of host memory");
    ctx->device = device_id;
    e = hipSetDevice(device_id);
    if (e == hipSuccess) e = hipGetDeviceProperties(&ctx->prop, device_id);
    if (e != hipSuccess) {
        int rc = fail(nullptr, TQ_ERR_HIP, "device %d not usable: %s", device_id, hipGetErrorString(e));
        delete ctx;
        return rc;
    }
    if (int rc = probe_scan_pb(ctx)) {
        g_create_err = ctx->err;
        delete ctx;
        return rc;
    }
    *out = ctx;
    return TQ_OK;
}

void tq_destroy(tq_ctx *ctx)
{
    if (!ctx) return;
    (void)hipSetDevice(ctx->device);
    free_data(ctx);
    free_source(ctx);
    if (ctx->d_scratch) (void)hipFree(ctx->d_scratch);
    if (ctx->d_cm) (void)hipFree(ctx->d_cm);
    if (ctx->d_sort) (void)hipFree(ctx->d_sort);
    if (ctx->d_sort_tmp) (void)hipFree(ctx->d_sort_tmp);
    if (ctx->d_units) (void)hipFree(ctx->d_units);
    if (ctx->d_de) (void)hipFree(ctx->d_de);
    if (ctx->d_sv) (void)hipFree(ctx->d_sv);
    if (ctx->d_nsnps) (void)hipFree(ctx->d_nsnps);
    if (ctx->d_bdsqr_stats) (void)hipFree(ctx->d_bdsqr_stats);
    if (ctx->d_sp_members) (void)hipFree(ctx->d_sp_members);
    if (ctx->d_sp_tab) (void)hipFree(ctx->d_sp_tab);
    if (ctx->sK) (void)hipStreamDestroy(ctx->sK);
    if (ctx->sC) (void)hipStreamDestroy(ctx->sC);
    if (ctx->sX) {
        (void)hipStreamDestroy(ctx->sX);
        (void)hipEventDestroy(ctx->evFork);
        (void)hipEventDestroy(ctx->evJoin);
    }
    if (ctx->evDevApi) (void)hipEventDestroy(ctx->evDevApi);
    for (auto e : ctx->pipe_events) (void)hipEventDestroy(e);
    for (auto &m : ctx->marks) (void)hipEventDestroy(m.ev);
    for (auto e : ctx->event_pool) (void)hipEventDestroy(e);
    delete ctx;
}

const char *tq_last_error(const tq_ctx *ctx) { return ctx ? ctx->err.c_str() : g_create_err.c_str(); }

int tq_host_alloc(int64_t bytes, void **out)
{
    if (!out || bytes < 0) return TQ_ERR_INVALID_ARG;
    *out = nullptr;
    return pool().alloc((size_t)bytes, out);
}

int tq_host_free(void *p)
{
    if (!p) return TQ_OK;
    return pool().release(p);
}

int tq_set_data(tq_ctx *ctx, const uint8_t *tmparr, int64_t T, int64_t S, const uint32_t *locus,
                int64_t locus_stride)
{
    if (!ctx) return TQ_ERR_INVALID_ARG;
    if (!tmparr || !locus) return fail(ctx, TQ_ERR_INVALID_ARG, "tq_set_data: NULL pointer");
    if (T < 1 || S < 1 || locus_stride < 1 || T > 0x7FFFFFFF)
        return fail(ctx, TQ_ERR_INVALID_ARG, "tq_set_data: bad shape T=%lld S=%lld stride=%lld", (long long)T,
                    (long long)S, (long long)locus_stride);
    TQ_HIP(ctx, hipSetDevice(ctx->device));
    free_data(ctx);
    ctx->data_gen++;

    std::vector<uint32_t> loc;
    bool ok = true, sorted = true;
    try {
        loc.resize((size_t)S);
        for (int64_t i = 0; i < S; ++i) {
            loc[(size_t)i] = locus[i * locus_stride];
            if (loc[(size_t)i] == 0xFFFFFFFFu) ok = false;
            if (i && loc[(size_t)i] < loc[(size_t)i - 1]) sorted = false;
        }
        if (ok && !sorted) {
            std::unordered_set<uint32_t> seen;
            seen.insert(loc[0]);
            for (int64_t i = 1; i < S && ok; ++i)
                if (loc[(size_t)i] != loc[(size_t)i - 1] && !seen.insert(loc[(size_t)i]).second) ok = false;
        }
    } catch (const std::bad_alloc &) {
        return fail(ctx, TQ_ERR_OOM, "tq_set_data: out of host memory");
    }
    ctx->locus_runs_ok = ok;

    const int64_t Sp = (int64_t)align_up((size_t)S, TILE);
    const int64_t W = Sp / 32;
    ctx->T = T; ctx->S = S; ctx->Sp = Sp; ctx->W = W;
    ctx->data_capacity = Sp;
    uint8_t *d_raw = nullptr;
    uint32_t *d_loc = nullptr;
    hipError_t e = hipMalloc((void **)&ctx->d_rows, (size_t)(T * Sp));
    if (e == hipSuccess) e = hipMalloc((void **)&ctx->d_nib, (size_t)(T * Sp / 2));
    if (e == hipSuccess) e = hipMalloc((void **)&ctx->d_nib5, (size_t)(T * Sp / 2));
    if (e == hipSuccess) e = hipMalloc((void **)&ctx->d_planes, (size_t)(T * W) * sizeof(uint4));
    if (e == hipSuccess) e = hipMalloc((void **)&ctx->d_planes3, (size_t)(T * W * 3 + W) * sizeof(uint32_t));
    ctx->plane_cap_W = W;
    if (e == hipSuccess) e = hipMalloc((void **)&d_raw, (size_t)(T * S));
    if (e == hipSuccess) e = hipMalloc((void **)&d_loc, (size_t)S * sizeof(uint32_t));
    if (e != hipSuccess) {
        if (d_raw) (void)hipFree(d_raw);
        if (d_loc) (void)hipFree(d_loc);
        free_data(ctx);
        return fail(ctx, e == hipErrorOutOfMemory ? TQ_ERR_OOM : TQ_ERR_HIP, "tq_set_data: hipMalloc failed: %s",
                    hipGetErrorString(e));
    }
    e = hipMemcpy(d_raw, tmparr, (size_t)(T * S), hipMemcpyHostToDevice);
    if (e == hipSuccess) e = hipMemcpy(d_loc, loc.data(), (size_t)S * sizeof(uint32_t), hipMemcpyHostToDevice);
    if (e == hipSuccess) {
        const int64_t n = T * W;
        hipLaunchKernelGGL(tq_prepare_rows, dim3((unsigned)((n + 255) / 256)), dim3(256), 0, 0, d_raw, d_loc, S, Sp,
                           W, (int32_t)T, ctx->d_rows, ctx->d_nib, ctx->d_nib5, ctx->d_planes,
                           ctx->d_planes3,
                           ctx->d_planes3 + (size_t)T * (size_t)W * 3);
        e = hipGetLastError();
        if (e == hipSuccess) e = hipDeviceSynchronize();
    }
    (void)hipFree(d_raw);
    (void)hipFree(d_loc);
    if (e != hipSuccess) {
        free_data(ctx);
        return fail(ctx, TQ_ERR_HIP, "tq_set_data: %s", hipGetErrorString(e));
    }
    ctx->have_data = true;
    return TQ_OK;
}

int tq_resolve_dev(tq_ctx *ctx, const uint32_t *d_quartets, int64_t Q, int subsample, uint32_t *d_rstat,
                   double *d_rscor, uint8_t *d_flags, void *stream)
{
    if (!ctx) return TQ_ERR_INVALID_ARG;
    if (Q < 0 || (Q > 0 && (!d_quartets || !d_rstat || !d_rscor)))
        return fail(ctx, TQ_ERR_INVALID_ARG, "tq_resolve_dev: NULL pointer or negative Q");
    TQ_HIP(ctx, hipSetDevice(ctx->device));
    OutPtrs out{d_rstat, d_rscor, d_flags, nullptr, nullptr, nullptr};
    if (int rc = enter_dev_api(ctx, (hipStream_t)stream)) return rc;
    return note_dev_api(ctx, (hipStream_t)stream,
                        launch(ctx, d_quartets, Q, subsample, false, false, out, (hipStream_t)stream, NoChunkHook()));
}

int tq_scan_dev(tq_ctx *ctx, const uint32_t *d_quartets, int64_t Q, int subsample, void *stream)
{
    if (!ctx) return TQ_ERR_INVALID_ARG;
    if (Q < 1 || !d_quartets) return fail(ctx, TQ_ERR_INVALID_ARG, "tq_scan_dev: NULL pointer or Q < 1");
    if (Q > ctx->batch)
        return fail(ctx, TQ_ERR_INVALID_ARG, "tq_scan_dev: Q=%lld exceeds the scan batch of %lld quartets (option 'batch')",
                    (long long)Q, (long long)ctx->batch);
    int rc = check_ready(ctx, subsample);
    if (rc) return rc;
    TQ_HIP(ctx, hipSetDevice(ctx->device));
    if (ctx->timing) ctx->timed_calls++;
    if ((rc = enter_dev_api(ctx, (hipStream_t)stream))) return rc;
    return note_dev_api(ctx, (hipStream_t)stream, stage_scan(ctx, d_quartets, Q, subsample, false, (hipStream_t)stream));
}

int tq_svd_dev(tq_ctx *ctx, int64_t q0, int64_t n, uint32_t *d_rstat, double *d_rscor, uint8_t *d_flags, void *stream)
{
    if (!ctx) return TQ_ERR_INVALID_ARG;
    if (n < 0 || (n > 0 && (!d_rstat || !d_rscor)))
        return fail(ctx, TQ_ERR_INVALID_ARG, "tq_svd_dev: NULL pointer or negative n");
    if (ctx->scanned_Q == 0) return fail(ctx, TQ_ERR_NO_DATA, "tq_svd_dev: no scanned batch (call tq_scan_dev first)");
    if (n == 0) return TQ_OK;
    TQ_HIP(ctx, hipSetDevice(ctx->device));
    OutPtrs out{d_rstat, d_rscor, d_flags, nullptr, nullptr, nullptr};
    if (int rc = enter_dev_api(ctx, (hipStream_t)stream)) return rc;
    return note_dev_api(ctx, (hipStream_t)stream, stage_svd(ctx, q0, n, false, out, (hipStream_t)stream, NoChunkHook()));
}

int tq_unrank_dev(tq_ctx *ctx, const uint64_t *d_ranks, int64_t Q, uint32_t *d_quartets, void *stream)
{
    if (!ctx) return TQ_ERR_INVALID_ARG;
    if (!ctx->have_data) return fail(ctx, TQ_ERR_NO_DATA, "tq_set_data has not been called");
    if (Q < 0 || (Q > 0 && (!d_ranks || !d_quartets)))
        return fail(ctx, TQ_ERR_INVALID_ARG, "tq_unrank_dev: NULL pointer or negative Q");
    if (Q == 0) return TQ_OK;
    TQ_HIP(ctx, hipSetDevice(ctx->device));
    hipLaunchKernelGGL(tq_unrank_kernel, dim3((unsigned)((Q + 255) / 256)), dim3(256), 0, (hipStream_t)stream,
                       d_ranks, (uint64_t)0, Q, (int32_t)ctx->T, d_quartets);
    TQ_HIP(ctx, hipGetLastError());
    return TQ_OK;
}

int tq_resolve_range_dev(tq_ctx *ctx, uint64_t first_rank, int64_t Q, int subsample, uint32_t *d_quartets,
                         uint32_t *d_rstat, double *d_rscor, uint8_t *d_flags, void *stream)
{
    if (!ctx) return TQ_ERR_INVALID_ARG;
    if (!ctx->have_data) return fail(ctx, TQ_ERR_NO_DATA, "tq_set_data has not been called");
    if (Q < 0 || (Q > 0 && (!d_rstat || !d_rscor)))
        return fail(ctx, TQ_ERR_INVALID_ARG, "tq_resolve_range_dev: NULL pointer or negative Q");
    if (Q == 0) return TQ_OK;
    const uint64_t T = (uint64_t)ctx->T;
    const uint64_t total = T < 4 ? 0 : T * (T - 1) / 2 * (T - 2) / 3 * (T - 3) / 4;
    if (first_rank + (uint64_t)Q > total)
        return fail(ctx, TQ_ERR_INVALID_ARG, "rank range [%llu,+%lld) exceeds C(%lld,4)=%llu",
                    (unsigned long long)first_rank, (long long)Q, (long long)ctx->T, (unsigned long long)total);
    TQ_HIP(ctx, hipSetDevice(ctx->device));
    uint32_t *dq = d_quartets;
    if (!dq) {
        int rc = ensure_scratch(ctx, (size_t)Q * 16);
        if (rc) return rc;
        dq = (uint32_t *)ctx->d_scratch;
    }
    hipLaunchKernelGGL(tq_unrank_kernel, dim3((unsigned)((Q + 255) / 256)), dim3(256), 0, (hipStream_t)stream,
                       (const uint64_t *)nullptr, first_rank, Q, (int32_t)ctx->T, dq);
    TQ_HIP(ctx, hipGetLastError());
    OutPtrs out{d_rstat, d_rscor, d_flags, nullptr, nullptr, nullptr};
    if (int rc2 = enter_dev_api(ctx, (hipStream_t)stream)) return rc2;
    return note_dev_api(ctx, (hipStream_t)stream,
                        launch(ctx, dq, Q, subsample, false, true, out, (hipStream_t)stream, NoChunkHook()));
}

int tq_resolve_to_host(tq_ctx *ctx, const uint32_t *d_quartets, int64_t Q, int subsample, uint32_t *rstat,
                       double *rscor, uint8_t *flags)
{
    if (!ctx) return TQ_ERR_INVALID_ARG;
    if (Q < 0 || (Q > 0 && (!d_quartets || !rstat || !rscor)))
        return fail(ctx, TQ_ERR_INVALID_ARG, "tq_resolve_to_host: NULL pointer or negative Q");
    int rc = check_ready(ctx, subsample);
    if (rc) return rc;
    if (Q == 0) return TQ_OK;
    TQ_HIP(ctx, hipSetDevice(ctx->device));
    if ((rc = ensure_streams(ctx))) return rc;
    const size_t o_rstat = 0;
    const size_t o_rscor = align_up(o_rstat + (size_t)Q * 8, 256);
    const size_t o_flags = align_up(o_rscor + (size_t)Q * 24, 256);
    if ((rc = ensure_scratch(ctx, align_up(o_flags + (size_t)Q, 256)))) return rc;
    char *base = (char *)ctx->d_scratch;
    return resolve_to_host(ctx, d_quartets, Q, subsample, false, rstat, rscor, flags, (uint32_t *)(base + o_rstat),
                           (double *)(base + o_rscor), (uint8_t *)(base + o_flags));
}

int tq_resolve_debug(tq_ctx *ctx, const uint32_t *quartets, int64_t Q, int subsample, uint32_t *rstat,
                     double *rscor, uint8_t *flags, uint32_t *cmats, double *svds, int32_t *ranks)
{
    if (!ctx) return TQ_ERR_INVALID_ARG;
    if (Q < 0 || (Q > 0 && (!quartets || !rstat || !rscor)))
        return fail(ctx, TQ_ERR_INVALID_ARG, "tq_resolve: NULL pointer or negative Q");
    int rc = check_ready(ctx, subsample);
    if (rc) return rc;
    if (Q == 0) return TQ_OK;
    TQ_HIP(ctx, hipSetDevice(ctx->device));
    constexpr int64_t CHECK_FIRST = 1 << 16;
    auto check_indices = [ctx, quartets, Q]() -> int {
        const uint32_t T = (uint32_t)ctx->T;
        uint32_t worst = 0;
        for (int64_t i = 0; i < 4 * Q; ++i) worst = quartets[i] > worst ? quartets[i] : worst;
        if (worst < T) return TQ_OK;
        for (int64_t i = 0; i < 4 * Q; ++i)
            if (quartets[i] >= T)
                return fail(ctx, TQ_ERR_INVALID_ARG, "quartet %lld has taxon index %u >= T=%lld", (long long)(i / 4),
                            quartets[i], (long long)ctx->T);
        return TQ_OK;
    };
    bool input_sorted = false;
    if (Q <= CHECK_FIRST) {
        if ((rc = check_indices())) return rc;
        bool sorted = true;
        uint64_t prev_key = 0;
        for (int64_t i = 0; i < Q; ++i) {
            const uint32_t *q = quartets + i * 4;
            const uint64_t key = ((uint64_t)q[0] << 42) | ((uint64_t)q[1] << 21) | (uint64_t)q[2];
            sorted &= key >= prev_key;
            prev_key = key;
        }
        input_sorted = sorted && ctx->T < (1 << 21);
    }
    HostScratch h;
    if ((rc = host_scratch(ctx, quartets, Q, cmats, svds, ranks, &h))) return rc;
    if (!(cmats || svds || ranks)) {
        if (Q <= CHECK_FIRST)
            return resolve_to_host(ctx, h.dq(), Q, subsample, input_sorted, rstat, rscor, flags, h.rstat(), h.rscor(),
                                   h.flags());
        return resolve_to_host(ctx, h.dq(), Q, subsample, false, rstat, rscor, flags, h.rstat(), h.rscor(), h.flags(),
                               check_indices);
    }
    if (Q > CHECK_FIRST && (rc = check_indices())) {
        (void)hipStreamSynchronize(ctx->sK);
        return rc;
    }
    return debug_to_host(ctx, h, Q, subsample, false, input_sorted, rstat, rscor, flags, cmats, svds, ranks);
}

int tq_resolve(tq_ctx *ctx, const uint32_t *quartets, int64_t Q, int subsample, uint32_t *rstat, double *rscor,
               uint8_t *flags)
{
    return tq_resolve_debug(ctx, quartets, Q, subsample, rstat, rscor, flags, nullptr, nullptr, nullptr);
}

int tq_set_species(tq_ctx *ctx, const int32_t *species_of, int64_t T, int64_t K)
{
    if (!ctx) return TQ_ERR_INVALID_ARG;
    if (!species_of) return fail(ctx, TQ_ERR_INVALID_ARG, "tq_set_species: NULL pointer");
    if (K < 4 || K > 0x7FFFFFFF)
        return fail(ctx, TQ_ERR_INVALID_ARG, "tq_set_species: K=%lld species (a species quartet needs K >= 4)", (long long)K);
    const int64_t known = ctx->have_data ? ctx->T : ctx->d_seqarr ? ctx->src_T : 0;
    if (T < 1 || (known && T != known))
        return fail(ctx, TQ_ERR_INVALID_ARG, "tq_set_species: T=%lld, the resident / source data have T=%lld", (long long)T,
                    (long long)known);
    std::vector<int32_t> size, members;
    try {
        size.assign((size_t)K, 0);
        for (int64_t i = 0; i < T; ++i) {
            const int32_t k = species_of[i];
            if (k < -1 || k >= K)
                return fail(ctx, TQ_ERR_INVALID_ARG, "tq_set_species: sample %lld has species id %d outside [-1, %lld)",
                            (long long)i, k, (long long)K);
            if (k >= 0 && ++size[(size_t)k] > 255)
                return fail(ctx, TQ_ERR_INVALID_ARG, "tq_set_species: species %d has more than 255 lineages", k);
        }
        members.assign((size_t)(K + 1 + T), 0);
        for (int64_t k = 0; k < K; ++k) members[(size_t)k + 1] = members[(size_t)k] + size[(size_t)k];
        std::vector<int32_t> fill(members.begin(), members.begin() + K);
        for (int64_t i = 0; i < T; ++i)
            if (species_of[i] >= 0) members[(size_t)(K + 1 + fill[(size_t)species_of[i]]++)] = (int32_t)i;
    } catch (const std::bad_alloc &) {
        return fail(ctx, TQ_ERR_OOM, "tq_set_species: out of host memory");
    }
    std::vector<int32_t> top(size);
    std::sort(top.begin(), top.end(), [](int32_t a, int32_t b) { return a > b; });
    uint64_t bound = 1;
    for (int i = 0; i < 4; ++i) bound *= (uint64_t)top[(size_t)i];
    TQ_HIP(ctx, hipSetDevice(ctx->device));
    TQ_HIP(ctx, hipDeviceSynchronize());
    if (ctx->d_sp_members) (void)hipFree(ctx->d_sp_members);
    ctx->d_sp_members = nullptr;
    ctx->sp_K = 0;
    TQ_HIP(ctx, hipMalloc((void **)&ctx->d_sp_members, members.size() * sizeof(int32_t)));
    TQ_HIP(ctx, hipMemcpy(ctx->d_sp_members, members.data(), members.size() * sizeof(int32_t), hipMemcpyHostToDevice));
    ctx->sp_size.swap(size);
    ctx->sp_T = T;
    ctx->sp_K = K;
    ctx->sp_bound = bound;
    ctx->sp_max = top[0];
    ctx->sp_tab_gen = ~0ull;
    return TQ_OK;
}

int tq_resolve_species_dev(tq_ctx *ctx, const uint32_t *d_squartets, int64_t Q, uint32_t *d_rstat, double *d_rscor,
                           uint8_t *d_flags, void *stream)
{
    if (!ctx) return TQ_ERR_INVALID_ARG;
    if (Q < 0 || (Q > 0 && (!d_squartets || !d_rstat || !d_rscor)))
        return fail(ctx, TQ_ERR_INVALID_ARG, "tq_resolve_species_dev: NULL pointer or negative Q");
    if (int rc = species_ready(ctx, "tq_resolve_species_dev")) return rc;
    if (Q == 0) return TQ_OK;
    TQ_HIP(ctx, hipSetDevice(ctx->device));
    if (int rc = enter_dev_api(ctx, (hipStream_t)stream)) return rc;
    OutPtrs out{d_rstat, d_rscor, d_flags, nullptr, nullptr, nullptr};
    return note_dev_api(ctx, (hipStream_t)stream,
                        launch(ctx, d_squartets, Q, 0, false, false, out, (hipStream_t)stream, NoChunkHook(), true));
}

int tq_resolve_species_debug(tq_ctx *ctx, const uint32_t *squartets, int64_t Q, uint32_t *rstat, double *rscor,
                             uint8_t *flags, uint32_t *cmats, double *svds, int32_t *ranks)
{
    if (!ctx) return TQ_ERR_INVALID_ARG;
    if (Q < 0 || (Q > 0 && (!squartets || !rstat || !rscor)))
        return fail(ctx, TQ_ERR_INVALID_ARG, "tq_resolve_species: NULL pointer or negative Q");
    int rc = species_ready(ctx, "tq_resolve_species");
    if (rc) return rc;
    if (Q == 0) return TQ_OK;
    const uint32_t K = (uint32_t)ctx->sp_K;
    const bool per_row = (unsigned __int128)ctx->S * ((uint64_t)ctx->sp_max * ctx->sp_max * ctx->sp_max * ctx->sp_max) >=
                         ((unsigned __int128)1 << 32);
    for (int64_t i = 0; i < Q; ++i) {
        const uint32_t *q = squartets + 4 * i;
        if ((q[0] >= K) | (q[1] >= K) | (q[2] >= K) | (q[3] >= K))
            return fail(ctx, TQ_ERR_INVALID_ARG, "species quartet %lld has a species id >= K=%u", (long long)i, K);
        if (per_row) {
            const uint64_t p = (uint64_t)ctx->sp_size[q[0]] * ctx->sp_size[q[1]] * ctx->sp_size[q[2]] * ctx->sp_size[q[3]];
            if ((unsigned __int128)ctx->S * p >= ((unsigned __int128)1 << 32))
                return fail(ctx, TQ_ERR_INVALID_ARG, "species quartet %lld: S=%lld x its lineage product %llu >= 2^32",
                            (long long)i, (long long)ctx->S, (unsigned long long)p);
        }
    }
    TQ_HIP(ctx, hipSetDevice(ctx->device));
    HostScratch h;
    if ((rc = host_scratch(ctx, squartets, Q, cmats, svds, ranks, &h))) return rc;
    if (!(cmats || svds || ranks)) return species_to_host(ctx, h.dq(), Q, rstat, rscor, flags, h.rstat(), h.rscor(), h.flags());
    return debug_to_host(ctx, h, Q, 0, true, false, rstat, rscor, flags, cmats, svds, ranks);
}

int tq_resolve_species(tq_ctx *ctx, const uint32_t *squartets, int64_t Q, uint32_t *rstat, double *rscor, uint8_t *flags)
{
    return tq_resolve_species_debug(ctx, squartets, Q, rstat, rscor, flags, nullptr, nullptr, nullptr);
}

int tq_timing_enable(tq_ctx *ctx, int on)
{
    if (!ctx) return TQ_ERR_INVALID_ARG;
    ctx->timing = on != 0;
    return TQ_OK;
}

int tq_timing_read_kernels(tq_ctx *ctx, double *ms, int n_ms, int64_t *calls)
{
    if (!ctx || (n_ms > 0 && !ms)) return TQ_ERR_INVALID_ARG;
    double t[TAG_COUNT] = {0, 0, 0, 0, 0};
    hipEvent_t prev[2] = {nullptr, nullptr};
    int rc = TQ_OK;
    for (auto &m : ctx->marks) {
        if (!rc && hipEventSynchronize(m.ev) != hipSuccess) rc = fail(ctx, TQ_ERR_HIP, "timing event failed");
        if (!rc && m.tag >= 0 && m.tag < TAG_COUNT && prev[m.lane]) {
            float a = 0.f;
            if (hipEventElapsedTime(&a, prev[m.lane], m.ev) == hipSuccess) t[m.tag] += a;
        }
        prev[m.lane] = m.ev;
        ctx->event_pool.push_back(m.ev);
    }
    ctx->marks.clear();
    for (int i = 0; i < n_ms; ++i) ms[i] = i < TAG_COUNT ? t[i] : 0.0;
    if (calls) *calls = ctx->timed_calls;
    ctx->timed_calls = 0;
    return rc;
}

int tq_timing_read_split(tq_ctx *ctx, double *total_ms, double *scan_ms, double *svd_ms, int64_t *calls)
{
    double t[TAG_COUNT];
    const int rc = tq_timing_read_kernels(ctx, t, TAG_COUNT, calls);
    if (rc) return rc;
    const double a = t[TAG_ORDER] + t[TAG_SCAN], b = t[TAG_BIDIAG] + t[TAG_BDSQR] + t[TAG_SCORE];
    if (total_ms) *total_ms = a + b;
    if (scan_ms) *scan_ms = a;
    if (svd_ms) *svd_ms = b;
    return TQ_OK;
}

int tq_timing_read(tq_ctx *ctx, double *kernel_ms, int64_t *launches)
{
    return tq_timing_read_split(ctx, kernel_ms, nullptr, nullptr, launches);
}

int tq_set_option(tq_ctx *ctx, const char *name, int64_t value)
{
    if (!ctx || !name) return TQ_ERR_INVALID_ARG;
    if (!strcmp(name, "nrep")) {
        if (value == 1 || value == 2 || value == 4 || value == 8 || value == 16 || value == 32) ctx->nrep = (int)value;
        else if (value != 0) return fail(ctx, TQ_ERR_INVALID_ARG, "nrep must be 1,2,4,8,16 or 32");
        else ctx->nrep = 1;
        return TQ_OK;
    }
    if (!strcmp(name, "waves_per_cu")) {
        if (value < 0 || value > (1 << 20)) return fail(ctx, TQ_ERR_INVALID_ARG, "waves_per_cu must be 0..2^20");
        ctx->waves_per_cu = (int)value;
        return TQ_OK;
    }
    if (!strcmp(name, "xcd_remap")) {
        ctx->xcd_remap = value != 0;
        return TQ_OK;
    }
    if (!strcmp(name, "count_invariant")) {
        ctx->count_invariant = value != 0;
        return TQ_OK;
    }
    if (!strcmp(name, "scan_pair")) {
        ctx->scan_pair = value != 0;
        return TQ_OK;
    }
    if (!strcmp(name, "scan_f4")) {
        if (value < -1 || value > 1) return fail(ctx, TQ_ERR_INVALID_ARG, "scan_f4 must be -1 (subsample mode only), 0 or 1");
        ctx->scan_f4 = (int)value;
        return TQ_OK;
    }
    if (!strcmp(name, "scan_dp")) {
        if (value != 0 && value != 1) return fail(ctx, TQ_ERR_INVALID_ARG, "scan_dp must be 0 or 1");
        ctx->scan_dp = (int)value;
        return TQ_OK;
    }
    if (!strcmp(name, "dp_min_quartets")) {
        if (value < 0) return fail(ctx, TQ_ERR_INVALID_ARG, "dp_min_quartets must be >= 0");
        ctx->dp_min_quartets = value ? value : 32768;
        return TQ_OK;
    }
    if (!strcmp(name, "wg_min_quartets")) {
        if (value < 0) return fail(ctx, TQ_ERR_INVALID_ARG, "wg_min_quartets must be >= 0");
        ctx->wg_min_quartets = value ? value : 4096;
        return TQ_OK;
    }
    if (!strcmp(name, "bidiag_layout")) {
        if (value < -1 || value > 1) return fail(ctx, TQ_ERR_INVALID_ARG, "bidiag_layout must be -1 (default), 0 or 1");
        ctx->bidiag_layout = value < 0 ? 1 : (int)value;
        return TQ_OK;
    }
    if (!strcmp(name, "park_t")) {
        ctx->park_t = value != 0;
        return TQ_OK;
    }
    if (!strcmp(name, "share_c")) {
        ctx->share_c = value != 0;
        return TQ_OK;
    }
    if (!strcmp(name, "stree_lds")) {
        if (value < 0 || value > 1) return fail(ctx, TQ_ERR_INVALID_ARG, "stree_lds must be 0 or 1");
        ctx->stree_lds = (int)value;
        return TQ_OK;
    }
    if (!strcmp(name, "svd_wpc")) {
        if (value < 0 || value > (1 << 20)) return fail(ctx, TQ_ERR_INVALID_ARG, "svd_wpc must be 0..2^20");
        ctx->svd_wpc = (int)value;
        return TQ_OK;
    }
    if (!strcmp(name, "svd_chunk")) {
        if (value < 0) return fail(ctx, TQ_ERR_INVALID_ARG, "svd_chunk must be >= 0");
        ctx->svd_chunk = value ? value : (1 << 18);
        return TQ_OK;
    }
    if (!strcmp(name, "svd_streams")) {
        if (value < 0 || value > 2) return fail(ctx, TQ_ERR_INVALID_ARG, "svd_streams must be 0 (default), 1 or 2");
        ctx->svd_streams = value ? (int)value : 2;
        return TQ_OK;
    }
    if (!strcmp(name, "bdsqr_stats")) {
        if (ctx->d_bdsqr_stats) (void)hipFree(ctx->d_bdsqr_stats);
        ctx->d_bdsqr_stats = nullptr;
        if (value) {
            TQ_HIP(ctx, hipMalloc((void **)&ctx->d_bdsqr_stats, 8 * sizeof(uint64_t)));
            TQ_HIP(ctx, hipMemset(ctx->d_bdsqr_stats, 0, 8 * sizeof(uint64_t)));
        }
        return TQ_OK;
    }
    if (!strcmp(name, "bdsqr_maxit")) {
        if (value < 0 || value > 1000) return fail(ctx, TQ_ERR_INVALID_ARG, "bdsqr_maxit must be 0..1000");
        ctx->bdsqr_maxit = value ? (int)value : 60;
        return TQ_OK;
    }
    if (!strcmp(name, "scan_wg")) {
        if (value != 0 && value != 1 && value != 2 && value != 3 && value != 4 && value != 6 && value != 8 && value != 16)
            return fail(ctx, TQ_ERR_INVALID_ARG, "scan_wg must be 0 (default), 1, 2, 3, 4, 6, 8 or 16");
        ctx->scan_wg = value ? (int)value : 4;
        return TQ_OK;
    }
    if (!strcmp(name, "svd_method")) {
        if (value != 0 && value != 1) return fail(ctx, TQ_ERR_INVALID_ARG, "svd_method must be 0 (Jacobi) or 1 (HQR)");
        ctx->svd_method = (int)value;
        return TQ_OK;
    }
    if (!strcmp(name, "order")) {
        if (value != 0 && value != 1) return fail(ctx, TQ_ERR_INVALID_ARG, "order must be 0 or 1");
        ctx->order = (int)value;
        return TQ_OK;
    }
    if (!strcmp(name, "scan_method")) {
        if (value < -1 || value > 6)
            return fail(ctx, TQ_ERR_INVALID_ARG, "scan_method must be -1 (auto), 0, 1, 6 (or 2..5: timing diagnostics)");
        ctx->scan_method = (int)value;
        return TQ_OK;
    }
    if (!strcmp(name, "batch")) {
        if (value < 0) return fail(ctx, TQ_ERR_INVALID_ARG, "batch must be >= 0");
        if (value > 0x7FFFFFFFll) value = 0x7FFFFFFFll;
        ctx->batch = value ? value : (1 << 23);
        return TQ_OK;
    }
    if (!strcmp(name, "species_method")) {
        if (value < -1 || value > 1)
            return fail(ctx, TQ_ERR_INVALID_ARG, "species_method must be -1 (auto), 0 (VALU form) or 1 (MFMA form)");
        ctx->species_method = (int)value;
        return TQ_OK;
    }
    if (!strcmp(name, "phases")) {
        if (value != 0 && value != 1 && value != 2 && value != 3)
            return fail(ctx, TQ_ERR_INVALID_ARG, "phases must be 1, 2 or 3");
        ctx->phases = value ? (int)value : 3;
        return TQ_OK;
    }
    return fail(ctx, TQ_ERR_INVALID_ARG, "unknown option '%s'", name);
}

int tq_set_source(tq_ctx *ctx, const uint8_t *seqarr, int64_t T, int64_t S0, const int64_t *spans, int64_t nloci)
{
    if (!ctx) return TQ_ERR_INVALID_ARG;
    if (!seqarr || !spans) return fail(ctx, TQ_ERR_INVALID_ARG, "tq_set_source: NULL pointer");
    if (T < 1 || S0 < 1 || nloci < 1 || T > 0x7FFFFFFF)
        return fail(ctx, TQ_ERR_INVALID_ARG, "tq_set_source: bad shape T=%lld S0=%lld nloci=%lld", (long long)T,
                    (long long)S0, (long long)nloci);
    int64_t maxw = 0;
    for (int64_t i = 0; i < nloci; ++i) {
        const int64_t a = spans[2 * i], b = spans[2 * i + 1];
        if (a < 0 || b <= a || b > S0)
            return fail(ctx, TQ_ERR_INVALID_ARG, "tq_set_source: span %lld = [%lld,%lld) outside [0,%lld)",
                        (long long)i, (long long)a, (long long)b, (long long)S0);
        if (b - a > maxw) maxw = b - a;
    }
    TQ_HIP(ctx, hipSetDevice(ctx->device));
    free_source(ctx);
    TQ_HIP(ctx, hipMalloc((void **)&ctx->d_seqarr, (size_t)(T * S0)));
    TQ_HIP(ctx, hipMalloc((void **)&ctx->d_spans, (size_t)nloci * 16));
    TQ_HIP(ctx, hipMalloc((void **)&ctx->d_lidxs, (size_t)nloci * 8));
    TQ_HIP(ctx, hipMemcpy(ctx->d_seqarr, seqarr, (size_t)(T * S0), hipMemcpyHostToDevice));
    TQ_HIP(ctx, hipMemcpy(ctx->d_spans, spans, (size_t)nloci * 16, hipMemcpyHostToDevice));
    try {
        ctx->h_spans.assign(spans, spans + 2 * nloci);
    } catch (const std::bad_alloc &) {
        return fail(ctx, TQ_ERR_OOM, "tq_set_source: out of host memory");
    }
    for (int i = 0; i < 2; ++i) {
        if (pool().alloc((size_t)nloci * 8, (void **)&ctx->h_lidx_stage[i]) != TQ_OK)
            return fail(ctx, TQ_ERR_OOM, "tq_set_source: out of page-locked host memory");
        TQ_HIP(ctx, hipEventCreateWithFlags(&ctx->ev_lidx[i], hipEventDisableTiming));
    }
    ctx->src_T = T;
    ctx->src_S0 = S0;
    ctx->nloci = nloci;
    ctx->max_width = maxw;
    return TQ_OK;
}

int tq_bootstrap_async(tq_ctx *ctx, const int64_t *lidxs, int64_t n, uint64_t seed_shuffle, uint64_t seed_ambig,
                       int64_t *out_S, void *stream_)
{
    if (!ctx) return TQ_ERR_INVALID_ARG;
    if (!ctx->d_seqarr) return fail(ctx, TQ_ERR_NO_DATA, "tq_set_source has not been called");
    if (!lidxs || n != ctx->nloci)
        return fail(ctx, TQ_ERR_INVALID_ARG, "tq_bootstrap: lidxs must hold nloci=%lld locus indices", (long long)ctx->nloci);
    hipStream_t stream = (hipStream_t)stream_;
    int64_t S = 0;
    for (int64_t i = 0; i < n; ++i) {
        if (lidxs[i] < 0 || lidxs[i] >= ctx->nloci)
            return fail(ctx, TQ_ERR_INVALID_ARG, "tq_bootstrap: locus index %lld out of range", (long long)lidxs[i]);
        S += ctx->h_spans[2 * lidxs[i] + 1] - ctx->h_spans[2 * lidxs[i]];
    }
    TQ_HIP(ctx, hipSetDevice(ctx->device));
    if (int rc0 = enter_dev_api(ctx, stream)) return rc0;
    const int64_t T = ctx->src_T;
    const int64_t cap = n * ctx->max_width;
    if (cap > ctx->boot_cap) {
        TQ_HIP(ctx, hipDeviceSynchronize());
        if (ctx->d_boot) (void)hipFree(ctx->d_boot);
        if (ctx->d_boot_tmp) (void)hipFree(ctx->d_boot_tmp);
        ctx->d_boot = nullptr;
        ctx->d_boot_tmp = nullptr;
        ctx->boot_cap = 0;
        TQ_HIP(ctx, hipMalloc((void **)&ctx->d_boot, (size_t)(2 * (n + 1) + 2 * cap) * sizeof(uint32_t)));
        size_t tmp = 0;
        uint32_t *u = ctx->d_boot;
        TQ_HIP(ctx, hipcub::DeviceScan::ExclusiveSum(nullptr, tmp, u, u, (int)(n + 1)));
        size_t tmp2 = 0;
        TQ_HIP(ctx, hipcub::DeviceScan::ExclusiveSum(nullptr, tmp2, u, u, (int)(cap / 32 + 2)));
        if (tmp2 > tmp) tmp = tmp2;
        TQ_HIP(ctx, hipMalloc(&ctx->d_boot_tmp, tmp ? tmp : 16));
        ctx->boot_tmp_bytes = tmp;
        ctx->boot_cap = cap;
    }
    if (S < 1 || S > ctx->boot_cap) return fail(ctx, TQ_ERR_INVALID_ARG, "tq_bootstrap: replicate length %lld", (long long)S);
    const int64_t Sp = (int64_t)align_up((size_t)S, TILE);
    const int64_t W = Sp / 32;
    if (Sp > ctx->data_capacity || T != ctx->T) {
        TQ_HIP(ctx, hipDeviceSynchronize());
        free_data(ctx);
        const int64_t capSp = (int64_t)align_up((size_t)(Sp + Sp / 8), TILE);
        TQ_HIP(ctx, hipMalloc((void **)&ctx->d_rows, (size_t)(T * capSp)));
        TQ_HIP(ctx, hipMalloc((void **)&ctx->d_nib, (size_t)(T * capSp / 2)));
        TQ_HIP(ctx, hipMalloc((void **)&ctx->d_nib5, (size_t)(T * capSp / 2)));
        TQ_HIP(ctx, hipMalloc((void **)&ctx->d_planes, (size_t)(T * (capSp / 32)) * sizeof(uint4)));
        TQ_HIP(ctx, hipMalloc((void **)&ctx->d_planes3, (size_t)(T * (capSp / 32) * 3 + capSp / 32) * sizeof(uint32_t)));
        ctx->plane_cap_W = capSp / 32;
        ctx->data_capacity = capSp;
    }
    uint32_t *widths = ctx->d_boot, *offsets = widths + (n + 1);
    uint32_t *src_col = offsets + (n + 1), *site_locus = src_col + ctx->boot_cap;
    const unsigned turn = ctx->lidx_turn++ & 1u;
    TQ_HIP(ctx, hipEventSynchronize(ctx->ev_lidx[turn]));
    memcpy(ctx->h_lidx_stage[turn], lidxs, (size_t)n * 8);
    TQ_HIP(ctx, hipMemcpyAsync(ctx->d_lidxs, ctx->h_lidx_stage[turn], (size_t)n * 8, hipMemcpyHostToDevice, stream));
    TQ_HIP(ctx, hipEventRecord(ctx->ev_lidx[turn], stream));
    TQ_HIP(ctx, hipMemsetAsync(widths + n, 0, sizeof(uint32_t), stream));
    hipLaunchKernelGGL(tq_boot_width_kernel, dim3((unsigned)((n + 255) / 256)), dim3(256), 0, stream, ctx->d_spans,
                       ctx->d_lidxs, n, ctx->nloci, widths);
    size_t tmp = ctx->boot_tmp_bytes;
    TQ_HIP(ctx, hipcub::DeviceScan::ExclusiveSum(ctx->d_boot_tmp, tmp, widths, offsets, (int)(n + 1), stream));
    hipLaunchKernelGGL(tq_boot_perm_kernel, dim3((unsigned)((n + 255) / 256)), dim3(256), 0, stream, ctx->d_spans,
                       ctx->d_lidxs, offsets, n, ctx->nloci, seed_shuffle, src_col, site_locus);
    const int64_t nw = T * W;
    hipLaunchKernelGGL(tq_boot_build_kernel, dim3((unsigned)((nw + 255) / 256)), dim3(256), 0, stream, ctx->d_seqarr,
                       ctx->src_S0, src_col, site_locus, S, Sp, W, (int32_t)T, seed_ambig, ctx->d_rows, ctx->d_nib, ctx->d_nib5,
                       ctx->d_planes, ctx->d_planes3, ctx->d_planes3 + (size_t)T * (size_t)ctx->plane_cap_W * 3);
    TQ_HIP(ctx, hipGetLastError());
    ctx->T = T;
    ctx->S = S;
    ctx->Sp = Sp;
    ctx->W = W;
    ctx->have_data = true;
    ctx->locus_runs_ok = true;
    ctx->scanned_Q = 0;
    ctx->data_gen++;
    if (out_S) *out_S = S;
    return note_dev_api(ctx, stream, TQ_OK);
}

int tq_bootstrap(tq_ctx *ctx, const int64_t *lidxs, int64_t n, uint64_t seed_shuffle, uint64_t seed_ambig,
                 int64_t *out_S)
{
    const int rc = tq_bootstrap_async(ctx, lidxs, n, seed_shuffle, seed_ambig, out_S, nullptr);
    if (rc) return rc;
    TQ_HIP(ctx, hipStreamSynchronize(nullptr));
    return TQ_OK;
}

int tq_sample_quartets_dev(tq_ctx *ctx, uint64_t seed, int64_t Q, uint64_t *d_ranks, uint32_t *d_quartets, void *stream)
{
    if (!ctx) return TQ_ERR_INVALID_ARG;
    if (!ctx->have_data && !ctx->d_seqarr) return fail(ctx, TQ_ERR_NO_DATA, "no data on the device (T unknown)");
    if (Q < 0 || (Q > 0 && !d_quartets)) return fail(ctx, TQ_ERR_INVALID_ARG, "tq_sample_quartets_dev: NULL pointer or negative Q");
    const uint64_t T = (uint64_t)(ctx->have_data ? ctx->T : ctx->src_T);
    const uint64_t total = T < 4 ? 0 : T * (T - 1) / 2 * (T - 2) / 3 * (T - 3) / 4;
    if ((uint64_t)Q > total)
        return fail(ctx, TQ_ERR_INVALID_ARG, "cannot draw %lld distinct quartets from C(%llu,4)=%llu", (long long)Q,
                    (unsigned long long)T, (unsigned long long)total);
    if (Q == 0) return TQ_OK;
    int half = 1;
    while (half < 32 && (1ull << (2 * half)) < total) ++half;
    TQ_HIP(ctx, hipSetDevice(ctx->device));
    hipLaunchKernelGGL(tq_sample_kernel, dim3((unsigned)((Q + 255) / 256)), dim3(256), 0, (hipStream_t)stream, seed, total,
                       half, Q, (int32_t)T, d_ranks, d_quartets);
    TQ_HIP(ctx, hipGetLastError());
    return TQ_OK;
}

int tq_get_data(tq_ctx *ctx, uint8_t *tmparr, uint32_t *tmpmap)
{
    if (!ctx) return TQ_ERR_INVALID_ARG;
    if (!ctx->have_data) return fail(ctx, TQ_ERR_NO_DATA, "no replicate on the device");
    if (!tmparr || !tmpmap) return fail(ctx, TQ_ERR_INVALID_ARG, "tq_get_data: NULL pointer");
    TQ_HIP(ctx, hipSetDevice(ctx->device));
    TQ_HIP(ctx, hipDeviceSynchronize());
    const int64_t T = ctx->T, S = ctx->S, W = ctx->W;
    const size_t bytes = align_up((size_t)(T * S), 256) + align_up((size_t)S * 8, 256) + align_up((size_t)(W + 1) * 8, 256);
    int rc = ensure_scratch(ctx, bytes);
    if (rc) return rc;
    uint8_t *d_arr = (uint8_t *)ctx->d_scratch;
    uint32_t *d_map = (uint32_t *)((char *)ctx->d_scratch + align_up((size_t)(T * S), 256));
    uint32_t *d_cnt = (uint32_t *)((char *)d_map + align_up((size_t)S * 8, 256));
    uint32_t *d_base = d_cnt + (W + 1);
    hipLaunchKernelGGL(tq_export_kernel, dim3((unsigned)((T * S + 255) / 256)), dim3(256), 0, 0, ctx->d_rows,
                       ctx->d_planes, S, ctx->Sp, W, (int32_t)T, d_arr, d_map);
    hipLaunchKernelGGL(tq_export_runcount_kernel, dim3((unsigned)((W + 255) / 256)), dim3(256), 0, 0, ctx->d_planes, W,
                       d_cnt);
    size_t tmp = 0;
    TQ_HIP(ctx, hipcub::DeviceScan::ExclusiveSum(nullptr, tmp, d_cnt, d_base, (int)W));
    void *d_tmp = nullptr;
    TQ_HIP(ctx, hipMalloc(&d_tmp, tmp ? tmp : 16));
    hipError_t e = hipcub::DeviceScan::ExclusiveSum(d_tmp, tmp, d_cnt, d_base, (int)W);
    if (e == hipSuccess) {
        hipLaunchKernelGGL(tq_export_locus_kernel, dim3((unsigned)((W + 255) / 256)), dim3(256), 0, 0, ctx->d_planes,
                           (const uint32_t *)d_base, S, W, d_map);
        e = hipGetLastError();
    }
    if (e == hipSuccess) e = hipMemcpy(tmparr, d_arr, (size_t)(T * S), hipMemcpyDeviceToHost);
    if (e == hipSuccess) e = hipMemcpy(tmpmap, d_map, (size_t)S * 8, hipMemcpyDeviceToHost);
    (void)hipFree(d_tmp);
    if (e != hipSuccess) return fail(ctx, TQ_ERR_HIP, "tq_get_data: %s", hipGetErrorString(e));
    return TQ_OK;
}

int tq_data_shape(tq_ctx *ctx, int64_t *T, int64_t *S)
{
    if (!ctx) return TQ_ERR_INVALID_ARG;
    if (T) *T = ctx->have_data ? ctx->T : 0;
    if (S) *S = ctx->have_data ? ctx->S : 0;
    return TQ_OK;
}

int tq_debug_fetch(tq_ctx *ctx, int which, void *dst, int64_t bytes)
{
    if (!ctx || !dst || bytes < 0) return TQ_ERR_INVALID_ARG;
    const void *src = which == 0 ? (const void *)ctx->d_cm : which == 1 ? (const void *)ctx->d_de
                      : which == 2 ? (const void *)ctx->d_sv : which == 3 ? (const void *)ctx->d_bdsqr_stats : nullptr;
    if (!src) return fail(ctx, TQ_ERR_INVALID_ARG, "tq_debug_fetch: nothing to fetch (which=%d)", which);
    TQ_HIP(ctx, hipSetDevice(ctx->device));
    TQ_HIP(ctx, hipDeviceSynchronize());
    TQ_HIP(ctx, hipMemcpy(dst, src, (size_t)bytes, hipMemcpyDeviceToHost));
    return TQ_OK;
}

int tq_debug_bdsqr(tq_ctx *ctx, const double *de, int64_t nmat, double *sv, uint32_t *work, int reps, double *ms)
{
    if (!ctx || !de || nmat < 1 || reps < 1) return TQ_ERR_INVALID_ARG;
    TQ_HIP(ctx, hipSetDevice(ctx->device));
    double *d_de = nullptr, *d_sv = nullptr;
    uint32_t *d_work = nullptr;
    hipEvent_t e0 = nullptr, e1 = nullptr;
    int rc = TQ_OK;
    auto step = [&](hipError_t e, const char *what) {
        if (!rc && e != hipSuccess) rc = fail(ctx, e == hipErrorOutOfMemory ? TQ_ERR_OOM : TQ_ERR_HIP, "tq_debug_bdsqr: %s: %s", what, hipGetErrorString(e));
    };
    step(hipMalloc(&d_de, (size_t)nmat * 256), "hipMalloc");
    if (!rc) step(hipMalloc(&d_sv, (size_t)nmat * 128), "hipMalloc");
    if (!rc) step(hipMalloc(&d_work, (size_t)nmat * 4), "hipMalloc");
    if (!rc) step(hipMemcpy(d_de, de, (size_t)nmat * 256, hipMemcpyHostToDevice), "H2D");
    if (!rc) step(hipEventCreate(&e0), "event");
    if (!rc) step(hipEventCreate(&e1), "event");
    const unsigned grid = (unsigned)((nmat + WAVE - 1) / WAVE);
    if (!rc) {
        hipLaunchKernelGGL(tq_bdsqr_kernel, dim3(grid), dim3(WAVE), 0, 0, (const double *)d_de, nmat, d_sv, ctx->bdsqr_maxit,
                           (unsigned long long *)nullptr, d_work);
        step(hipGetLastError(), "launch");
        if (!rc) step(hipEventRecord(e0, 0), "record");
        for (int i = 0; i < reps && !rc; ++i)
            hipLaunchKernelGGL(tq_bdsqr_kernel, dim3(grid), dim3(WAVE), 0, 0, (const double *)d_de, nmat, d_sv, ctx->bdsqr_maxit,
                               (unsigned long long *)nullptr, (uint32_t *)nullptr);
        if (!rc) step(hipEventRecord(e1, 0), "record");
        if (!rc) step(hipEventSynchronize(e1), "sync");
        float t = 0.f;
        if (!rc) step(hipEventElapsedTime(&t, e0, e1), "elapsed");
        if (ms) *ms = (double)t / reps;
    }
    if (!rc && sv) step(hipMemcpy(sv, d_sv, (size_t)nmat * 128, hipMemcpyDeviceToHost), "D2H");
    if (!rc && work) step(hipMemcpy(work, d_work, (size_t)nmat * 4, hipMemcpyDeviceToHost), "D2H");
    if (e0) (void)hipEventDestroy(e0);
    if (e1) (void)hipEventDestroy(e1);
    if (d_de) (void)hipFree(d_de);
    if (d_sv) (void)hipFree(d_sv);
    if (d_work) (void)hipFree(d_work);
    return rc;
}

int tq_format_tsv(const uint32_t *quartets, const uint32_t *rstat, const double *rscor, int64_t Q, char *out,
                  int64_t cap, int64_t *written)
{
    if (Q < 0 || cap < 0 || !written || (Q > 0 && (!quartets || !rstat || !rscor || !out))) return TQ_ERR_INVALID_ARG;
    const int64_t n = format_tsv(quartets, rstat, rscor, Q, out, cap);
    *written = n < 0 ? -n : n;
    return n < 0 ? TQ_ERR_OOM : TQ_OK;
}

int tq_format_qmc(const uint32_t *quartets, const uint32_t *rstat, const double *rscor, int64_t Q, int weights,
                  int64_t min_snps, double min_ratio, char *out, int64_t cap, int64_t *written, int64_t *n_lines)
{
    if (Q < 0 || cap < 0 || !written || weights < 0 || weights > 3 ||
        (Q > 0 && (!quartets || !rstat || !rscor || !out)))
        return TQ_ERR_INVALID_ARG;
    const int64_t n = format_qmc(quartets, rstat, rscor, Q, weights, min_snps, min_ratio, out, cap, n_lines);
    *written = n < 0 ? -n : n;
    return n < 0 ? TQ_ERR_OOM : TQ_OK;
}

int tq_qmc_splits(const uint32_t *quartets, const uint32_t *rstat, const double *rscor, int64_t Q, int weights,
                  int64_t min_snps, double min_ratio, uint32_t *splits, double *wout, int64_t *n_rows)
{
    if (Q < 0 || !n_rows || weights < 0 || weights > 3 || (Q > 0 && (!quartets || !rstat || !rscor || !splits || !wout)))
        return TQ_ERR_INVALID_ARG;
    *n_rows = qmc_splits(quartets, rstat, rscor, Q, weights, min_snps, min_ratio, splits, wout);
    return TQ_OK;
}

int tq_numpy_choice_tail(void *np_bitgen, uint64_t pop, int64_t size, int64_t *out)
{
    if (!np_bitgen || !out || size < 1 || (uint64_t)size > pop || pop < 2 || pop > 0xFFFFFFFEull) return TQ_ERR_INVALID_ARG;
    return numpy_choice_tail((NpBitgen *)np_bitgen, pop, size, out);
}

int tq_unrank(const uint64_t *ranks, uint64_t first_rank, int64_t Q, int64_t T, uint32_t *quartets)
{
    if (Q < 0 || T < 4 || T > 100000 || (Q > 0 && !quartets)) return TQ_ERR_INVALID_ARG;
    const uint64_t t = (uint64_t)T, total = t * (t - 1) / 2 * (t - 2) / 3 * (t - 3) / 4;
    if (ranks) {
        for (int64_t i = 0; i < Q; ++i)
            if (ranks[i] >= total) return TQ_ERR_INVALID_ARG;
    } else if (first_rank + (uint64_t)Q > total) {
        return TQ_ERR_INVALID_ARG;
    }
    unrank_host(ranks, first_rank, Q, (int32_t)T, quartets);
    return TQ_OK;
}

int tq_qmc_tree(const uint32_t *splits, const double *weights, int64_t n, int64_t ntaxa, uint64_t seed, char *out,
                int64_t cap, int64_t *written)
{
    if (n < 0 || cap < 0 || !written || ntaxa < 1 || ntaxa > (1 << 24) || (n > 0 && !splits) || (cap > 0 && !out))
        return TQ_ERR_INVALID_ARG;
    try {
        std::string nwk;
        const int rc = qmc_tree(splits, weights, n, ntaxa, seed, nwk);
        if (rc) return rc;
        *written = (int64_t)nwk.size();
        if ((int64_t)nwk.size() > cap) return TQ_ERR_OOM;
        memcpy(out, nwk.data(), nwk.size());
        return TQ_OK;
    } catch (const std::bad_alloc &) {
        *written = 0;
        return TQ_ERR_OOM;
    }
}

int tq_conc_create(tq_conc **out, const int32_t *parent, int64_t n_nodes, int64_t T, int64_t min_snps, double min_ratio,
                   tq_ctx *ctx)
{
    if (!out) return fail(ctx, TQ_ERR_INVALID_ARG, "tq_conc_create: out is NULL");
    *out = nullptr;
    if (!parent) return fail(ctx, TQ_ERR_INVALID_ARG, "tq_conc_create: parent is NULL");
    if (std::isnan(min_ratio)) return fail(ctx, TQ_ERR_INVALID_ARG, "tq_conc_create: min_ratio is NaN");
    tq_conc *acc = new (std::nothrow) tq_conc();
    if (!acc) return fail(ctx, TQ_ERR_OOM, "out of host memory");
    try {
        const std::string err = conc_build_tree(parent, n_nodes, T, acc->t);
        if (!err.empty()) {
            delete acc;
            return fail(ctx, TQ_ERR_INVALID_ARG, "tq_conc_create: %s", err.c_str());
        }
        acc->ctx = ctx;
        acc->min_snps = (uint32_t)std::min<int64_t>(std::max<int64_t>(1, min_snps), 0xFFFFFFFFll);
        acc->min_ratio = min_ratio;
        acc->words = (int64_t)acc->t.E * CONC_EDGE_WORDS + 2 * T + 1;
        acc->hi.assign(acc->words, 0);
        acc->hf.assign(acc->words, 0.0);
    } catch (const std::bad_alloc &) {
        delete acc;
        return fail(ctx, TQ_ERR_OOM, "tq_conc_create: out of host memory");
    }
    if (ctx) {
        const ConcTree &t = acc->t;
        acc->num_cu = std::max(1, ctx->prop.multiProcessorCount);
        acc->gmax = (int)std::max<int64_t>(1, std::min<int64_t>(acc->num_cu, (int64_t(64) << 20) / (acc->words * 8)));
        hipError_t e = hipSetDevice(ctx->device);
        if (e == hipSuccess) e = hipMalloc((void **)&acc->d_lca, (size_t)T * T * 2);
        if (e == hipSuccess) e = hipMalloc((void **)&acc->d_dep, (size_t)t.N * 2);
        if (e == hipSuccess) e = hipMalloc((void **)&acc->d_eid, (size_t)t.N * 4);
        if (e == hipSuccess) e = hipMalloc((void **)&acc->d_slab, (size_t)acc->gmax * acc->words * 8);
        if (e == hipSuccess) e = hipMalloc((void **)&acc->d_tot, (size_t)acc->words * 8);
        if (e == hipSuccess) e = hipMemcpy(acc->d_lca, t.lca.data(), (size_t)T * T * 2, hipMemcpyHostToDevice);
        if (e == hipSuccess) e = hipMemcpy(acc->d_dep, t.dep.data(), (size_t)t.N * 2, hipMemcpyHostToDevice);
        if (e == hipSuccess) e = hipMemcpy(acc->d_eid, t.eid.data(), (size_t)t.N * 4, hipMemcpyHostToDevice);
        if (e == hipSuccess) e = hipMemset(acc->d_tot, 0, (size_t)acc->words * 8);
        if (e == hipSuccess) e = hipEventCreateWithFlags(&acc->ev, hipEventDisableTiming);
        if (e != hipSuccess) {
            conc_free_dev(acc);
            delete acc;
            return fail(ctx, e == hipErrorOutOfMemory ? TQ_ERR_OOM : TQ_ERR_HIP, "tq_conc_create: %s", hipGetErrorString(e));
        }
    }
    *out = acc;
    return TQ_OK;
}

void tq_conc_destroy(tq_conc *acc)
{
    if (!acc) return;
    if (acc->ctx) {
        (void)hipSetDevice(acc->ctx->device);
        if (acc->pending) (void)hipEventSynchronize(acc->ev);
        conc_free_dev(acc);
    }
    delete acc;
}

int tq_conc_reset(tq_conc *acc)
{
    if (!acc) return TQ_ERR_INVALID_ARG;
    std::fill(acc->hi.begin(), acc->hi.end(), 0);
    std::fill(acc->hf.begin(), acc->hf.end(), 0.0);
    if (acc->ctx) {
        if (int rc = conc_wait(acc)) return rc;
        TQ_HIP(acc->ctx, hipMemset(acc->d_tot, 0, (size_t)acc->words * 8));
    }
    return TQ_OK;
}

int tq_conc_add(tq_conc *acc, const uint32_t *quartets, const uint32_t *rstat, const double *rscor, const uint8_t *flags,
                int64_t n)
{
    if (!acc) return TQ_ERR_INVALID_ARG;
    if (n < 0 || (n > 0 && (!quartets || !rstat || !rscor)))
        return fail(acc->ctx, TQ_ERR_INVALID_ARG, "tq_conc_add: NULL pointer or negative n");
    conc_add_host(acc->t, acc->min_snps, acc->min_ratio, quartets, rstat, rscor, flags, n, acc->hi, acc->hf);
    return TQ_OK;
}

int tq_conc_add_dev(tq_conc *acc, const uint32_t *d_quartets, const uint32_t *d_rstat, const double *d_rscor,
                    const uint8_t *d_flags, int64_t n, void *stream)
{
    if (!acc) return TQ_ERR_INVALID_ARG;
    tq_ctx *ctx = acc->ctx;
    if (!ctx) return fail(nullptr, TQ_ERR_INVALID_ARG, "tq_conc_add_dev: the accumulator was created without a context");
    if (n < 0 || (n > 0 && (!d_quartets || !d_rstat || !d_rscor)))
        return fail(ctx, TQ_ERR_INVALID_ARG, "tq_conc_add_dev: NULL pointer or negative n");
    if (n == 0) return TQ_OK;
    hipStream_t st = (hipStream_t)stream;
    TQ_HIP(ctx, hipSetDevice(ctx->device));
    if (acc->pending && st != acc->last) TQ_HIP(ctx, hipStreamWaitEvent(st, acc->ev, 0));
    if (int rc = conc_launch(acc, d_quartets, d_rstat, d_rscor, d_flags, n, st)) return rc;
    TQ_HIP(ctx, hipEventRecord(acc->ev, st));
    acc->pending = true;
    acc->last = st;
    return TQ_OK;
}

int tq_conc_shape(const tq_conc *acc, int64_t *T, int64_t *n_edges, int64_t *mask_words)
{
    if (!acc) return TQ_ERR_INVALID_ARG;
    if (T) *T = acc->t.T;
    if (n_edges) *n_edges = acc->t.E;
    if (mask_words) *mask_words = acc->t.W;
    return TQ_OK;
}

int tq_conc_read(tq_conc *acc, int64_t *edge_counts, double *edge_sums, uint64_t *masks, int64_t *tip_counts,
                 int64_t *skipped)
{
    if (!acc) return TQ_ERR_INVALID_ARG;
    const ConcTree &t = acc->t;
    std::vector<uint64_t> dv;
    try {
        dv.assign(acc->words, 0);
    } catch (const std::bad_alloc &) {
        return fail(acc->ctx, TQ_ERR_OOM, "tq_conc_read: out of host memory");
    }
    if (acc->ctx) {
        if (int rc = conc_wait(acc)) return rc;
        TQ_HIP(acc->ctx, hipMemcpy(dv.data(), acc->d_tot, (size_t)acc->words * 8, hipMemcpyDeviceToHost));
    }
    for (int32_t e = 0; e < t.E; ++e) {
        const uint64_t *d = &dv[(size_t)e * CONC_EDGE_WORDS];
        const uint64_t *h = &acc->hi[(size_t)e * CONC_EDGE_WORDS];
        if (edge_counts) {
            int64_t *o = edge_counts + 6 * (int64_t)e;
            o[0] = (int64_t)t.nqrts[e];
            for (int k = 0; k < 5; ++k) o[1 + k] = (int64_t)(d[k] + h[k]);
        }
        if (edge_sums)
            for (int k = 0; k < 2; ++k) {
                double dvf;
                memcpy(&dvf, &d[CW_WEIGHT + k], 8);
                edge_sums[2 * (int64_t)e + k] = dvf + acc->hf[(size_t)e * CONC_EDGE_WORDS + CW_WEIGHT + k];
            }
    }
    if (masks) memcpy(masks, t.masks.data(), t.masks.size() * 8);
    const int64_t tb = (int64_t)t.E * CONC_EDGE_WORDS;
    if (tip_counts)
        for (int64_t i = 0; i < 2 * (int64_t)t.T; ++i) tip_counts[i] = (int64_t)(dv[tb + i] + acc->hi[tb + i]);
    if (skipped) *skipped = (int64_t)(dv[tb + 2 * t.T] + acc->hi[tb + 2 * t.T]);
    return TQ_OK;
}

int tq_stree_create(tq_stree **out, int64_t ntaxa, int64_t capacity_rows, int weights, int64_t min_snps, double min_ratio,
                    tq_ctx *ctx)
{
    if (!out) return fail(ctx, TQ_ERR_INVALID_ARG, "tq_stree_create: out is NULL");
    *out = nullptr;
    if (ntaxa < 1 || ntaxa > 65535) return fail(ctx, TQ_ERR_INVALID_ARG, "tq_stree_create: ntaxa must be 1..65535");
    if (ctx && (ntaxa < 4 || ntaxa > STREE_T_MAX))
        return fail(ctx, TQ_ERR_INVALID_ARG, "tq_stree_create: the device path takes 4 <= ntaxa <= %d", STREE_T_MAX);
    if (capacity_rows < 0 || capacity_rows >= (int64_t(1) << 31))
        return fail(ctx, TQ_ERR_INVALID_ARG, "tq_stree_create: capacity_rows must be 0..2^31-1");
    if (weights < 0 || weights > 3) return fail(ctx, TQ_ERR_INVALID_ARG, "tq_stree_create: no weight strategy %d", weights);
    if (std::isnan(min_ratio)) return fail(ctx, TQ_ERR_INVALID_ARG, "tq_stree_create: min_ratio is NaN");
    tq_stree *acc = new (std::nothrow) tq_stree();
    if (!acc) return fail(ctx, TQ_ERR_OOM, "out of host memory");
    acc->ctx = ctx;
    acc->ntaxa = ntaxa;
    acc->capacity = capacity_rows;
    acc->weights = weights;
    acc->min_snps = (uint32_t)std::min<int64_t>(std::max<int64_t>(1, min_snps), 0xFFFFFFFFll);
    acc->min_ratio = min_ratio;
    if (ctx) {
        acc->num_cu = std::max(1, ctx->prop.multiProcessorCount);
        acc->max_nodes = 3 * ntaxa;
        acc->max_cells = 3 * ntaxa * ntaxa / 2 + 16;
        const size_t rows = (size_t)std::max<int64_t>(1, capacity_rows);
        hipError_t e = hipSetDevice(ctx->device);
        if (e == hipSuccess) e = hipMalloc((void **)&acc->d_root_t, rows * 8);
        if (e == hipSuccess) e = hipMalloc((void **)&acc->d_root_k, rows * 8);
        for (int b = 0; b < 2; ++b) {
            if (e == hipSuccess) e = hipMalloc((void **)&acc->d_wt[b], rows * 8);
            if (e == hipSuccess) e = hipMalloc((void **)&acc->d_wk[b], rows * 8);
            if (e == hipSuccess) e = hipMalloc((void **)&acc->d_wn[b], rows * 4);
        }
        if (e == hipSuccess) e = hipMalloc((void **)&acc->d_cnt, SC_WORDS * 8);
        if (e == hipSuccess) e = hipMalloc((void **)&acc->d_mat, (size_t)acc->max_cells * 16);
// ... 259 lines not shown
```

tetrad_amd/engine.py:

```python
from __future__ import annotations

import ctypes

import numpy as np

from . import _lib
from ._lib import TetradHipError


def _ptr(a):
    return ctypes.c_void_p(a.ctypes.data) if a is not None else None


class _PinnedBlock:
    __slots__ = ("ptr", "nbytes", "_free", "__weakref__")

    def __init__(self, nbytes: int):
        lib = _lib.load()
        p = ctypes.c_void_p()
        rc = lib.tq_host_alloc(int(nbytes), ctypes.byref(p))
        if rc != 0 or not p.value:
            raise TetradHipError(rc or -6, f"tq_host_alloc({nbytes}) failed")
        self.ptr, self.nbytes, self._free = p.value, int(nbytes), lib.tq_host_free

    @property
    def __array_interface__(self):
        return {"shape": (self.nbytes,), "typestr": "|u1", "data": (self.ptr, False), "version": 3}

    def __del__(self):
        try:
            self._free(ctypes.c_void_p(self.ptr))
        except Exception:
            pass


def pinned_empty(shape, dtype) -> np.ndarray:
    dtype = np.dtype(dtype)
    shape = (shape,) if np.isscalar(shape) else tuple(shape)
    n = int(np.prod(shape, dtype=np.int64)) * dtype.itemsize
    raw = np.asarray(_PinnedBlock(max(n, 1)))
    return raw[:n].view(dtype).reshape(shape)


class QuartetEngine:
    def __init__(self, device_id: int = 0):
        self._lib = _lib.load()
        h = ctypes.c_void_p()
        rc = self._lib.tq_create(ctypes.byref(h), int(device_id))
        if rc != 0:
            raise TetradHipError(rc, self._lib.tq_last_error(None).decode())
        self._h = h
        self.device_id = int(device_id)
        self.T = self.S = 0
        self.data_generation = 0

    def close(self):
        if getattr(self, "_h", None):
            self._lib.tq_destroy(self._h)
            self._h = None

    def __enter__(self):
        return self

    def __exit__(self, *exc):
        self.close()

    def __del__(self):
        try:
            self.close()
        except Exception:
            pass

    def _check(self, rc: int):
        if rc != 0:
            raise TetradHipError(rc, self._lib.tq_last_error(self._h).decode())

    def set_data(self, tmparr: np.ndarray, tmpmap: np.ndarray):
        tmparr = np.ascontiguousarray(tmparr, dtype=np.uint8)
        if tmparr.ndim != 2:
            raise ValueError("tmparr must be 2-D [ntaxa, nsites]")
        tmpmap = np.asarray(tmpmap)
        if tmpmap.ndim == 2:
            tm = np.ascontiguousarray(tmpmap, dtype=np.uint32)
            stride = tm.shape[1]
        else:
            tm = np.ascontiguousarray(tmpmap, dtype=np.uint32)
            stride = 1
        if tm.shape[0] != tmparr.shape[1]:
            raise ValueError("tmpmap rows must equal tmparr columns")
        T, S = tmparr.shape
        self.data_generation += 1
        self._check(self._lib.tq_set_data(self._h, _ptr(tmparr), T, S, _ptr(tm), stride))
        self.T, self.S = T, S

    def set_source(self, seqarr: np.ndarray, spans: np.ndarray):
        seqarr = np.ascontiguousarray(seqarr, dtype=np.uint8)
        spans = np.ascontiguousarray(spans, dtype=np.int64).reshape(-1, 2)
        T, S0 = seqarr.shape
        self._check(self._lib.tq_set_source(self._h, _ptr(seqarr), T, S0, _ptr(spans), spans.shape[0]))
        self.nloci = spans.shape[0]

    def bootstrap(self, lidxs: np.ndarray, seed_shuffle: int, seed_ambig: int, stream: int | None = None) -> int:
        lidxs = np.ascontiguousarray(lidxs, dtype=np.int64)
        S = ctypes.c_int64()
        self.data_generation += 1
        if stream is None:
            self._check(self._lib.tq_bootstrap(self._h, _ptr(lidxs), lidxs.shape[0], int(seed_shuffle),
                                               int(seed_ambig), ctypes.byref(S)))
        else:
            self._check(self._lib.tq_bootstrap_async(self._h, _ptr(lidxs), lidxs.shape[0], int(seed_shuffle),
                                                     int(seed_ambig), ctypes.byref(S), stream or None))
        T = ctypes.c_int64()
        self._check(self._lib.tq_data_shape(self._h, ctypes.byref(T), None))
        self.T, self.S = T.value, S.value
        return S.value

    def get_data(self):
        T, S = ctypes.c_int64(), ctypes.c_int64()
        self._check(self._lib.tq_data_shape(self._h, ctypes.byref(T), ctypes.byref(S)))
        tmparr = np.zeros((T.value, S.value), np.uint8)
        tmpmap = np.zeros((S.value, 2), np.uint32)
        self._check(self._lib.tq_get_data(self._h, _ptr(tmparr), _ptr(tmpmap)))
        return tmparr, tmpmap

    def set_option(self, name: str, value: int) -> int:
        self._check(self._lib.tq_set_option(self._h, name.encode(), int(value)))
        return int(value)

    def resolve(self, quartets: np.ndarray, subsample_snps: bool = True, debug: bool = False):
        q = quartets
        if not (isinstance(q, np.ndarray) and q.dtype == np.uint32 and q.flags.c_contiguous):
            src = np.asarray(quartets)
            q = pinned_empty((src.size // 4, 4), np.uint32)
            q[...] = src.reshape(-1, 4)
        q = q.reshape(-1, 4)
        Q = q.shape[0]
        rstat = pinned_empty((Q, 2), np.uint32)
        rscor = pinned_empty((Q, 3), np.float64)
        flags = pinned_empty(Q, np.uint8)
        if debug:
            cm = np.zeros((Q, 3, 16, 16), np.uint32)
            sv = np.zeros((Q, 3, 16), np.float64)
            rk = np.zeros((Q, 3), np.int32)
            self._check(self._lib.tq_resolve_debug(
                self._h, _ptr(q), Q, int(bool(subsample_snps)), _ptr(rstat), _ptr(rscor),
                _ptr(flags), _ptr(cm), _ptr(sv), _ptr(rk)))
            return rstat, rscor, flags, dict(cmats=cm, svds=sv, ranks=rk)
        self._check(self._lib.tq_resolve(
            self._h, _ptr(q), Q, int(bool(subsample_snps)), _ptr(rstat), _ptr(rscor), _ptr(flags)))
        return rstat, rscor, flags

    def resolve_to_host(self, d_quartets: int, Q: int, subsample_snps: bool = True, out=None):
        if out is None:
            out = (pinned_empty((Q, 2), np.uint32), pinned_empty((Q, 3), np.float64), pinned_empty(Q, np.uint8))
        rstat, rscor, flags = out
        self._check(self._lib.tq_resolve_to_host(
            self._h, d_quartets, Q, int(bool(subsample_snps)), _ptr(rstat), _ptr(rscor), _ptr(flags)))
        return rstat, rscor, flags

    def set_species(self, species_of, K: int | None = None):
        sp = np.ascontiguousarray(species_of, dtype=np.int32).reshape(-1)
        if K is None:
            K = int(sp.max()) + 1 if sp.size else 0
        self._check(self._lib.tq_set_species(self._h, _ptr(sp), sp.shape[0], int(K)))

    def resolve_species(self, squartets: np.ndarray, debug: bool = False):
        q = squartets
        if not (isinstance(q, np.ndarray) and q.dtype == np.uint32 and q.flags.c_contiguous):
            src = np.asarray(squartets)
            q = pinned_empty((src.size // 4, 4), np.uint32)
            q[...] = src.reshape(-1, 4)
        q = q.reshape(-1, 4)
        Q = q.shape[0]
        rstat = pinned_empty((Q, 2), np.uint32)
        rscor = pinned_empty((Q, 3), np.float64)
        flags = pinned_empty(Q, np.uint8)
        if debug:
            cm = np.zeros((Q, 3, 16, 16), np.uint32)
            sv = np.zeros((Q, 3, 16), np.float64)
            rk = np.zeros((Q, 3), np.int32)
            self._check(self._lib.tq_resolve_species_debug(self._h, _ptr(q), Q, _ptr(rstat), _ptr(rscor), _ptr(flags),
                                                           _ptr(cm), _ptr(sv), _ptr(rk)))
            return rstat, rscor, flags, dict(cmats=cm, svds=sv, ranks=rk)
        self._check(self._lib.tq_resolve_species(self._h, _ptr(q), Q, _ptr(rstat), _ptr(rscor), _ptr(flags)))
        return rstat, rscor, flags

    def resolve_species_dev(self, d_squartets: int, Q: int, d_rstat: int, d_rscor: int, d_flags: int = 0,
                            stream: int = 0):
        self._check(self._lib.tq_resolve_species_dev(self._h, d_squartets, Q, d_rstat, d_rscor, d_flags or None,
                                                     stream or None))

    def resolve_dev(self, d_quartets: int, Q: int, subsample_snps: bool, d_rstat: int,
                    d_rscor: int, d_flags: int = 0, stream: int = 0):
        self._check(self._lib.tq_resolve_dev(
            self._h, d_quartets, Q, int(bool(subsample_snps)), d_rstat, d_rscor,
            d_flags or None, stream or None))

    def resolve_range_dev(self, first_rank: int, Q: int, subsample_snps: bool, d_quartets: int,
                          d_rstat: int, d_rscor: int, d_flags: int = 0, stream: int = 0):
        self._check(self._lib.tq_resolve_range_dev(
            self._h, first_rank, Q, int(bool(subsample_snps)), d_quartets or None, d_rstat,
            d_rscor, d_flags or None, stream or None))

    def scan_dev(self, d_quartets: int, Q: int, subsample_snps: bool, stream: int = 0):
        self._check(self._lib.tq_scan_dev(self._h, d_quartets, Q, int(bool(subsample_snps)), stream or None))

    def svd_dev(self, q0: int, n: int, d_rstat: int, d_rscor: int, d_flags: int = 0, stream: int = 0):
        self._check(self._lib.tq_svd_dev(self._h, q0, n, d_rstat, d_rscor, d_flags or None, stream or None))

    def sample_quartets_dev(self, seed: int, Q: int, d_quartets: int, d_ranks: int = 0, stream: int = 0):
        self._check(self._lib.tq_sample_quartets_dev(self._h, int(seed) & (2**64 - 1), Q, d_ranks or None, d_quartets,
                                                     stream or None))

    def unrank_dev(self, d_ranks: int, Q: int, d_quartets: int, stream: int = 0):
        self._check(self._lib.tq_unrank_dev(self._h, d_ranks, Q, d_quartets, stream or None))

    def timing_enable(self, on: bool = True):
        self._check(self._lib.tq_timing_enable(self._h, int(on)))

    def timing_read(self):
        ms = ctypes.c_double()
        n = ctypes.c_int64()
        self._check(self._lib.tq_timing_read(self._h, ctypes.byref(ms), ctypes.byref(n)))
        return ms.value, n.value

    def timing_read_split(self):
        tot, a, b = ctypes.c_double(), ctypes.c_double(), ctypes.c_double()
        n = ctypes.c_int64()
        self._check(self._lib.tq_timing_read_split(
            self._h, ctypes.byref(tot), ctypes.byref(a), ctypes.byref(b), ctypes.byref(n)))
        return tot.value, a.value, b.value, n.value

    KERNEL_TAGS = ("order", "scan", "bidiag", "bdsqr", "score")

    def timing_read_kernels(self):
        ms = (ctypes.c_double * 5)()
        n = ctypes.c_int64()
        self._check(self._lib.tq_timing_read_kernels(self._h, ms, 5, ctypes.byref(n)))
        return dict(zip(self.KERNEL_TAGS, list(ms))), n.value

    def debug_fetch(self, which: str, n: int) -> np.ndarray:
        shape, dt, code = {"cm": ((n, 256), np.uint32, 0), "de": ((3 * n, 32), np.float64, 1),
                           "sv": ((3 * n, 16), np.float64, 2), "bdsqr_stats": ((8,), np.uint64, 3)}[which]
        out = np.zeros(shape, dt)
        self._check(self._lib.tq_debug_fetch(self._h, code, _ptr(out), out.nbytes))
        return out

    def debug_bdsqr(self, de: np.ndarray, reps: int = 5):
        de = np.ascontiguousarray(de, dtype=np.float64)
        nmat = de.shape[0]
        sv = np.zeros((nmat, 16), np.float64)
        work = np.zeros(nmat, np.uint32)
        ms = ctypes.c_double()
        self._check(self._lib.tq_debug_bdsqr(self._h, _ptr(de), nmat, _ptr(sv), _ptr(work), reps, ctypes.byref(ms)))
        return sv, work & 0xFFFF, work >> 16, ms.value

    def device_info(self):
        cu = ctypes.c_int32()
        w = ctypes.c_int32()
        pitch = ctypes.c_int64()
        self._check(self._lib.tq_device_info(self._h, ctypes.byref(cu), ctypes.byref(w), ctypes.byref(pitch)))
        return dict(num_cu=cu.value, waves_per_cu=w.value, row_pitch=pitch.value)
```

Before: 107.4 million quartets/s.

## Pack locus runs into 32-site words to shorten subsample scans

Adds a host-side bin-packing of locus runs (SNPs from the same locus) into 32-site words, ordered so fuller bins come first. A second packed copy of rows, nibbles and planes is built on device, and the subsample scan kernels use it. In subsample mode each quartet stops at the first informative site of each locus, so packing is meant to cut the number of words each wave has to step through. A sampled cost model decides automatically whether packing pays. The price is extra device memory, extra setup work in tq_set_data, and packed data whose column order differs from the original site order.

```diff
diff --git a/include/tetrad_hip.h b/include/tetrad_hip.h
--- a/include/tetrad_hip.h
+++ b/include/tetrad_hip.h
@@ -90,6 +90,9 @@
                   int weights, int64_t min_snps, double min_ratio, char *out, int64_t cap,
                   int64_t *written, int64_t *n_lines);
 
+int tq_pack_sites(const uint8_t *tmparr, int64_t T, int64_t S, const uint32_t *locus, int64_t locus_stride, uint32_t *src,
+                  int64_t cap, int64_t *packed_sites, int32_t *pays, double *estimate);
+
 int tq_numpy_choice_tail(void *np_bitgen, uint64_t pop, int64_t size, int64_t *out);
 
 int tq_unrank(const uint64_t *ranks, uint64_t first_rank, int64_t Q, int64_t T, uint32_t *quartets);
diff --git a/tetrad_amd/_lib.py b/tetrad_amd/_lib.py
--- a/tetrad_amd/_lib.py
+++ b/tetrad_amd/_lib.py
@@ -31,6 +31,7 @@
     "tq_stree_create", "tq_stree_destroy", "tq_stree_reset", "tq_stree_add", "tq_stree_add_dev", "tq_stree_graph",
     "tq_stree_rows", "tq_stree_build", "tq_stree_level_stats",
     "tq_set_species", "tq_resolve_species", "tq_resolve_species_dev", "tq_resolve_species_debug",
+    "tq_pack_sites",
 ]
 
 
@@ -198,6 +199,8 @@
     lib.tq_resolve_species_dev.restype = i32
     lib.tq_resolve_species_debug.argtypes = [vp, vp, i64, vp, vp, vp, vp, vp, vp]
     lib.tq_resolve_species_debug.restype = i32
+    lib.tq_pack_sites.argtypes = [vp, i64, i64, vp, i64, vp, i64, c.POINTER(i64), c.POINTER(c.c_int32), vp]
+    lib.tq_pack_sites.restype = i32
     lib.tq_device_info.argtypes = [vp, c.POINTER(c.c_int32), c.POINTER(c.c_int32), c.POINTER(i64)]
     lib.tq_device_info.restype = i32
     _lib = lib
diff --git a/tetrad_amd/csrc/pack.hpp b/tetrad_amd/csrc/pack.hpp
--- /dev/null
+++ b/tetrad_amd/csrc/pack.hpp
@@ -0,0 +1,151 @@
+#pragma once
+
+constexpr uint32_t PACK_PAD = 0xFFFFFFFFu;
+
+constexpr double PACK_STEP_COST = 18.0, PACK_TRIP_COST = 15.0, PACK_MIN_GAIN = 0.03;
+constexpr int PACK_SAMPLE = 24;
+
+inline size_t pack_round_up(size_t v, size_t a) { return (v + a - 1) / a * a; }
+
+struct LocusRun {
+    int64_t start, len;
+};
+
+inline void locus_runs(const uint32_t *loc, int64_t S, std::vector<LocusRun> &runs)
+{
+    runs.clear();
+    for (int64_t s = 0; s < S;) {
+        int64_t e = s + 1;
+        while (e < S && loc[e] == loc[s]) ++e;
+        runs.push_back({s, e - s});
+        s = e;
+    }
+}
+
+inline void pack_sites(const std::vector<LocusRun> &runs, std::vector<uint32_t> &src)
+{
+    const size_t n = runs.size();
+    std::vector<uint32_t> by_len;
+    by_len.reserve(n);
+    {
+        std::vector<uint32_t> bucket[33];
+        for (size_t i = 0; i < n; ++i) {
+            if (runs[i].len > 32) by_len.push_back((uint32_t)i);
+            else bucket[runs[i].len].push_back((uint32_t)i);
+        }
+        for (int l = 32; l >= 1; --l) by_len.insert(by_len.end(), bucket[l].begin(), bucket[l].end());
+    }
+    struct Bin {
+        uint32_t count;
+    };
+    std::vector<Bin> bins;
+    std::vector<uint32_t> bin_of(n);
+    std::vector<uint32_t> open[33];
+    for (uint32_t i : by_len) {
+        const int64_t len = runs[i].len;
+        const int need = (int)(len > 32 ? (len - 1) % 32 + 1 : len);
+        int r = 33;
+        if (len <= 32)
+            for (r = need; r <= 32 && open[r].empty(); ++r) {}
+        uint32_t b;
+        if (r <= 32) {
+            b = open[r].back();
+            open[r].pop_back();
+        } else {
+            b = (uint32_t)bins.size();
+            bins.push_back({0});
+            r = 32;
+        }
+        bin_of[i] = b;
+        bins[b].count++;
+        if (r - need > 0) open[r - need].push_back(b);
+    }
+    const size_t nb = bins.size();
+    std::vector<uint32_t> first(nb + 1, 0), member(n);
+    for (size_t i = 0; i < n; ++i) first[bin_of[i] + 1]++;
+    for (size_t b = 0; b < nb; ++b) first[b + 1] += first[b];
+    {
+        std::vector<uint32_t> fill(first.begin(), first.end() - 1);
+        for (uint32_t i : by_len) member[fill[bin_of[i]]++] = i;
+    }
+    std::vector<uint32_t> order;
+    order.reserve(nb);
+    {
+        std::vector<uint32_t> bucket[33];
+        for (size_t b = 0; b < nb; ++b) bucket[bins[b].count].push_back((uint32_t)b);
+        for (int c = 32; c >= 1; --c) order.insert(order.end(), bucket[c].begin(), bucket[c].end());
+    }
+    src.clear();
+    for (uint32_t b : order) {
+        for (uint32_t k = first[b]; k < first[b + 1]; ++k) {
+            const LocusRun &run = runs[member[k]];
+            for (int64_t s = 0; s < run.len; ++s) src.push_back((uint32_t)(run.start + s));
+        }
+        src.resize(pack_round_up(src.size(), 32), PACK_PAD);
+    }
+    src.resize(pack_round_up(src.size() ? src.size() : 1, TILE), PACK_PAD);
+}
+
+inline double pack_estimate(const uint8_t *tmparr, int64_t T, int64_t S, const std::vector<LocusRun> &runs,
+                          const std::vector<uint32_t> &src, double cost[2], double trips[2])
+{
+    const int64_t Wn = (int64_t)pack_round_up((size_t)S, TILE) / 32, Wp = (int64_t)src.size() / 32;
+    cost[0] = PACK_STEP_COST * (double)(Wn / WAVE);
+    cost[1] = PACK_STEP_COST * (double)(Wp / WAVE);
+    trips[0] = trips[1] = 0.0;
+    if (T < 4) return 0.0;
+    std::vector<uint32_t> pos((size_t)S);
+    for (size_t p = 0; p < src.size(); ++p)
+        if (src[p] != PACK_PAD) pos[src[p]] = (uint32_t)p;
+    std::vector<uint8_t> cn((size_t)Wn), cp((size_t)Wp);
+    uint64_t x = 0x9E3779B97F4A7C15ull ^ (uint64_t)S;
+    auto next = [&x]() {
+        x += 0x9E3779B97F4A7C15ull;
+        uint64_t z = x;
+        z = (z ^ (z >> 30)) * 0xBF58476D1CE4E5B9ull;
+        z = (z ^ (z >> 27)) * 0x94D049BB133111EBull;
+        return z ^ (z >> 31);
+    };
+    uint64_t sum[2] = {0, 0};
+    double dsum = 0.0, dsq = 0.0;
+    for (int q = 0; q < PACK_SAMPLE; ++q) {
+        int64_t t[4];
+        for (int k = 0; k < 4; ++k) {
+            bool again;
+            do {
+                t[k] = (int64_t)(next() % (uint64_t)T);
+                again = false;
+                for (int j = 0; j < k; ++j) again |= t[j] == t[k];
+            } while (again);
+        }
+        const uint8_t *a = tmparr + t[0] * S, *b = tmparr + t[1] * S, *c = tmparr + t[2] * S, *d = tmparr + t[3] * S;
+        std::fill(cn.begin(), cn.end(), (uint8_t)0);
+        std::fill(cp.begin(), cp.end(), (uint8_t)0);
+        for (const LocusRun &run : runs) {
+            for (int64_t s = run.start; s < run.start + run.len; ++s) {
+                const uint8_t va = a[s], vb = b[s], vc = c[s], vd = d[s];
+                if ((va | vb | vc | vd) > 3 || (va == vb && va == vc && va == vd)) continue;
+                cn[(size_t)(s >> 5)]++;
+                cp[pos[(size_t)s] >> 5]++;
+                break;
+            }
+        }
+        uint64_t tq[2] = {0, 0};
+        for (int64_t w = 0; w < Wn; w += WAVE) tq[0] += *std::max_element(cn.begin() + w, cn.begin() + w + WAVE);
+        for (int64_t w = 0; w < Wp; w += WAVE) tq[1] += *std::max_element(cp.begin() + w, cp.begin() + w + WAVE);
+        sum[0] += tq[0];
+        sum[1] += tq[1];
+        const double dq = (double)tq[0] - (double)tq[1];
+        dsum += dq;
+        dsq += dq * dq;
+    }
+    for (int k = 0; k < 2; ++k) {
+        trips[k] = (double)sum[k] / PACK_SAMPLE;
+        cost[k] += PACK_TRIP_COST * trips[k];
+    }
+    const double n = PACK_SAMPLE, mean = dsum / n, var = std::max(0.0, (dsq - n * mean * mean) / (n - 1));
+    const double se = std::sqrt(var / n) * PACK_TRIP_COST;
+    return cost[0] > 0.0 ? (cost[0] - cost[1] - 2.0 * se) / cost[0] : 0.0;
+}
+
+inline bool pack_pays(double gain_low) { return gain_low >= PACK_MIN_GAIN; }
diff --git a/tetrad_amd/csrc/prepare.hpp b/tetrad_amd/csrc/prepare.hpp
--- a/tetrad_amd/csrc/prepare.hpp
+++ b/tetrad_amd/csrc/prepare.hpp
@@ -11,6 +11,7 @@
 }
 
 __global__ void tq_prepare_rows(const uint8_t *__restrict__ raw, const uint32_t *__restrict__ locus,
+                                const uint32_t *__restrict__ site_src,
                                 int64_t S, int64_t Sp, int64_t W, int32_t T, uint8_t *__restrict__ rows,
                                 uint8_t *__restrict__ nib, uint8_t *__restrict__ nib5, uint4 *__restrict__ planes,
                                 uint32_t *__restrict__ planes3, uint32_t *__restrict__ runbeg)
@@ -18,16 +19,17 @@
     int64_t gid = (int64_t)blockIdx.x * blockDim.x + threadIdx.x;
     if (gid >= (int64_t)T * W) return;
     int64_t t = gid / W, w = gid - t * W;
-    const uint8_t *src = raw + t * S + w * 32;
+    const uint8_t *src = raw + t * S;
     uint8_t *dst = rows + t * Sp;
     uint32_t mm = 0, b0 = 0, b1 = 0, rb = 0;
     uint32_t nw[4] = {0, 0, 0, 0}, n5[4] = {0, 0, 0, 0};
     for (int i = 0; i < 32; ++i) {
-        int64_t s = w * 32 + i;
-        uint8_t v = (s < S) ? src[i] : (uint8_t)0xFF;
+        const int64_t p = w * 32 + i;
+        const int64_t s = site_src ? (site_src[p] == 0xFFFFFFFFu ? S : (int64_t)site_src[p]) : p;
+        uint8_t v = (s < S) ? src[s] : (uint8_t)0xFF;
         bool missing = v > 3;
         uint8_t code = missing ? (uint8_t)0 : v;
-        dst[row_offset(s)] = code;
+        dst[row_offset(p)] = code;
         nw[i >> 3] |= (uint32_t)code << (8 * (i & 3) + 4 * ((i >> 2) & 1));
         n5[i >> 3] |= (uint32_t)(missing ? 4 : code) << (8 * (i & 3) + 4 * ((i >> 2) & 1));
         mm |= (uint32_t)missing << i;
@@ -41,7 +43,7 @@
     planes[t * W + w] = make_uint4(mm, b0, b1, rb);
     store_planes3(planes3, runbeg, t, W, w, mm, b0, b1, rb);
     reinterpret_cast<uint4 *>(nib + t * (Sp / 2))[w] = make_uint4(nw[0], nw[1], nw[2], nw[3]);
-    reinterpret_cast<uint4 *>(nib5 + t * (Sp / 2))[w] = make_uint4(n5[0], n5[1], n5[2], n5[3]);
+    if (nib5) reinterpret_cast<uint4 *>(nib5 + t * (Sp / 2))[w] = make_uint4(n5[0], n5[1], n5[2], n5[3]);
 }
 
 __device__ __forceinline__ uint64_t choose_k(uint64_t n, int k)
diff --git a/tetrad_amd/csrc/tetrad_hip.hip b/tetrad_amd/csrc/tetrad_hip.hip
--- a/tetrad_amd/csrc/tetrad_hip.hip
+++ b/tetrad_amd/csrc/tetrad_hip.hip
@@ -24,6 +24,7 @@
 
 #include "common.hpp"
 #include "prepare.hpp"
+#include "pack.hpp"
 #include "scan.hpp"
 #include "scan_pb.hpp"
 #include "scan_dp.hpp"
@@ -112,6 +113,12 @@
     int species_method = -1;
     uint64_t data_gen = 0;
     uint64_t sp_tab_gen = ~0ull;
+    int site_pack = -1;
+    uint8_t *pk_rows = nullptr, *pk_nib = nullptr;
+    uint4 *pk_planes = nullptr;
+    uint32_t *pk_planes3 = nullptr;
+    int64_t pk_Sp = 0, pk_W = 0;
+    uint64_t pk_gen = ~0ull;
     hipStream_t sK = nullptr, sC = nullptr;
     std::vector<hipEvent_t> pipe_events;
     hipEvent_t evDevApi = nullptr;
@@ -241,6 +248,20 @@
     return a.type == hipMemoryTypeHost;
 }
 
+void free_packed(tq_ctx *ctx)
+{
+    if (ctx->pk_rows) (void)hipFree(ctx->pk_rows);
+    if (ctx->pk_nib) (void)hipFree(ctx->pk_nib);
+    if (ctx->pk_planes) (void)hipFree(ctx->pk_planes);
+    if (ctx->pk_planes3) (void)hipFree(ctx->pk_planes3);
+    ctx->pk_rows = nullptr;
+    ctx->pk_nib = nullptr;
+    ctx->pk_planes = nullptr;
+    ctx->pk_planes3 = nullptr;
+    ctx->pk_Sp = ctx->pk_W = 0;
+    ctx->pk_gen = ~0ull;
+}
+
 void free_data(tq_ctx *ctx)
 {
     if (ctx->d_rows) (void)hipFree(ctx->d_rows);
@@ -248,6 +269,7 @@
     if (ctx->d_nib5) (void)hipFree(ctx->d_nib5);
     if (ctx->d_planes) (void)hipFree(ctx->d_planes);
     if (ctx->d_planes3) (void)hipFree(ctx->d_planes3);
+    free_packed(ctx);
     ctx->d_rows = nullptr;
     ctx->d_nib = nullptr;
     ctx->d_nib5 = nullptr;
@@ -437,6 +459,22 @@
     return d;
 }
 
+DevData scan_data(const tq_ctx *ctx, int subsample)
+{
+    DevData d = dev_data(ctx);
+    if (!subsample || !ctx->site_pack || !ctx->pk_rows || ctx->pk_gen != ctx->data_gen) return d;
+    d.rows = ctx->pk_rows;
+    d.nib = ctx->pk_nib;
+    d.nib5 = nullptr;
+    d.planes = ctx->pk_planes;
+    d.planes3 = ctx->pk_planes3;
+    d.runbeg = ctx->pk_planes3 + (size_t)ctx->T * (size_t)ctx->pk_W * 3;
+    d.pitch = ctx->pk_Sp;
+    d.W = ctx->pk_W;
+    d.ntiles = (int32_t)(ctx->pk_Sp / TILE);
+    return d;
+}
+
 template <typename K>
 int grid_for(tq_ctx *ctx, K kern, int64_t items, int64_t *grid, int wpc_kernel = 0)
 {
@@ -454,19 +492,19 @@
 }
 
 template <int NREP, bool SUB, int METHOD>
-int launch_scan(tq_ctx *ctx, const uint32_t *dq, const uint32_t *order, int64_t Q, hipStream_t stream)
+int launch_scan(tq_ctx *ctx, const DevData &d, const uint32_t *dq, const uint32_t *order, int64_t Q, hipStream_t stream)
 {
     auto kern = tq_scan_kernel<NREP, SUB, METHOD>;
     int64_t grid;
     int rc = grid_for(ctx, kern, Q, &grid);
     if (rc) return rc;
-    hipLaunchKernelGGL(kern, dim3((unsigned)grid), dim3(WAVE), 0, stream, dev_data(ctx), dq, order, Q, ctx->d_cm);
+    hipLaunchKernelGGL(kern, dim3((unsigned)grid), dim3(WAVE), 0, stream, d, dq, order, Q, ctx->d_cm);
     TQ_HIP(ctx, hipGetLastError());
     return TQ_OK;
 }
 
 template <bool SUB, int METHOD, int NW, bool SHC = false, bool PARK_T = false>
-int launch_scan_wg(tq_ctx *ctx, const uint32_t *dq, const uint32_t *order, int64_t Q, hipStream_t stream)
+int launch_scan_wg(tq_ctx *ctx, const DevData &d, const uint32_t *dq, const uint32_t *order, int64_t Q, hipStream_t stream)
 {
     auto kern = tq_scan_wg_kernel<SUB, METHOD, NW, SHC, PARK_T>;
     const int wgs = ctx->waves_per_cu > 0 ? (ctx->waves_per_cu + NW - 1) / NW : 0;
@@ -481,14 +519,14 @@
         }
     }
     if (grid < 1) grid = 1;
-    hipLaunchKernelGGL(kern, dim3((unsigned)grid), dim3(NW * WAVE), 0, stream, dev_data(ctx), dq, order, Q,
+    hipLaunchKernelGGL(kern, dim3((unsigned)grid), dim3(NW * WAVE), 0, stream, d, dq, order, Q,
                        ctx->d_cm, xcd_chunk);
     TQ_HIP(ctx, hipGetLastError());
     return TQ_OK;
 }
 
 template <bool SUB>
-int launch_scan_pb(tq_ctx *ctx, const uint32_t *dq, const uint32_t *order, int64_t Q, hipStream_t stream)
+int launch_scan_pb(tq_ctx *ctx, const DevData &d, const uint32_t *dq, const uint32_t *order, int64_t Q, hipStream_t stream)
 {
     auto kern = tq_scan_pb_kernel<SUB>;
     const int64_t nblk = (Q + PB_NW - 1) / PB_NW;
@@ -498,7 +536,7 @@
         grid = xcd_chunk * 8;
     }
     if (grid < 1) grid = 1;
-    hipLaunchKernelGGL(kern, dim3((unsigned)grid), dim3(PB_NW * WAVE), 0, stream, dev_data(ctx), dq, order, Q, ctx->d_cm,
+    hipLaunchKernelGGL(kern, dim3((unsigned)grid), dim3(PB_NW * WAVE), 0, stream, d, dq, order, Q, ctx->d_cm,
                        xcd_chunk, (uint32_t *)nullptr);
     TQ_HIP(ctx, hipGetLastError());
     return TQ_OK;
@@ -525,7 +563,7 @@
 }
 
 template <bool SUB, int METHOD, int NW>
-int launch_scan_wg2(tq_ctx *ctx, const uint32_t *dq, const uint32_t *order, int64_t Q, hipStream_t stream)
+int launch_scan_wg2(tq_ctx *ctx, const DevData &d, const uint32_t *dq, const uint32_t *order, int64_t Q, hipStream_t stream)
 {
     auto kern = tq_scan_wg2_kernel<SUB, METHOD, NW>;
     const int64_t nblk = (Q + 2 * NW - 1) / (2 * NW);
@@ -535,7 +573,7 @@
         grid = xcd_chunk * 8;
     }
     if (grid < 1) grid = 1;
-    hipLaunchKernelGGL(kern, dim3((unsigned)grid), dim3(NW * WAVE), 0, stream, dev_data(ctx), dq, order, Q, ctx->d_cm,
+    hipLaunchKernelGGL(kern, dim3((unsigned)grid), dim3(NW * WAVE), 0, stream, d, dq, order, Q, ctx->d_cm,
                        xcd_chunk);
     TQ_HIP(ctx, hipGetLastError());
     return TQ_OK;
@@ -555,17 +593,18 @@
 int launch_scan_n(tq_ctx *ctx, const uint32_t *dq, const uint32_t *order, int64_t Q, int subsample,
                   hipStream_t stream)
 {
+    const DevData d = scan_data(ctx, subsample);
     if (ctx->scan_pair && ctx->scan_wg == 4 && Q >= 64 && !ctx->count_invariant && !ctx->share_c && ctx->waves_per_cu == 0 &&
-        ctx->scan_method < 2 && (uint64_t)ctx->T * (uint64_t)ctx->Sp < 0xFFFF0000ull) {
+        ctx->scan_method < 2 && (uint64_t)ctx->T * (uint64_t)d.pitch < 0xFFFF0000ull) {
         const int m = ctx->scan_method < 0 ? (subsample ? 1 : 0) : ctx->scan_method;
         if (subsample)
-            return m ? launch_scan_wg2<true, 1, 4>(ctx, dq, order, Q, stream) : launch_scan_wg2<true, 0, 4>(ctx, dq, order, Q, stream);
-        return m ? launch_scan_wg2<false, 1, 4>(ctx, dq, order, Q, stream) : launch_scan_wg2<false, 0, 4>(ctx, dq, order, Q, stream);
+            return m ? launch_scan_wg2<true, 1, 4>(ctx, d, dq, order, Q, stream) : launch_scan_wg2<true, 0, 4>(ctx, d, dq, order, Q, stream);
+        return m ? launch_scan_wg2<false, 1, 4>(ctx, d, dq, order, Q, stream) : launch_scan_wg2<false, 0, 4>(ctx, d, dq, order, Q, stream);
     }
     const bool f4 = ctx->scan_f4 < 0 ? (subsample != 0 && ctx->scan_method < 0 && ctx->park_t) : ctx->scan_f4 != 0;
     if (f4 && (ctx->scan_wg == 4 || ctx->scan_wg == 8 || ctx->scan_wg == 2) && Q >= ctx->wg_min_quartets && !ctx->count_invariant &&
         !ctx->share_c && !ctx->scan_pair && ctx->waves_per_cu == 0 && (ctx->scan_method < 0 || ctx->scan_method == 1) &&
-        (uint64_t)ctx->T * (uint64_t)ctx->Sp < 0xFFFF0000ull) {
+        (uint64_t)ctx->T * (uint64_t)d.pitch < 0xFFFF0000ull) {
         const int nw = ctx->scan_wg;
         const int64_t nblk = (Q + nw - 1) / nw;
         int64_t grid = nblk, xcd_chunk = 0;
@@ -576,46 +615,46 @@
 #define TQ_F4_CASE(SUBF, NWF)                                                                                         \
         if ((subsample != 0) == SUBF && nw == NWF)                                                                    \
             hipLaunchKernelGGL((tq_scan_f4_kernel<SUBF, NWF>), dim3((unsigned)grid), dim3(NWF * WAVE), 0, stream,      \
-                               dev_data(ctx), dq, order, Q, ctx->d_cm, xcd_chunk);
+                               d, dq, order, Q, ctx->d_cm, xcd_chunk);
         TQ_F4_CASE(true, 4) TQ_F4_CASE(false, 4) TQ_F4_CASE(true, 8) TQ_F4_CASE(false, 8) TQ_F4_CASE(true, 2) TQ_F4_CASE(false, 2)
 #undef TQ_F4_CASE
         TQ_HIP(ctx, hipGetLastError());
         return TQ_OK;
     }
     const bool pb_fits = ctx->pb_ok == 1 && ctx->scan_wg == 4 && Q >= 64 && !ctx->count_invariant && !ctx->share_c &&
-                         !ctx->scan_pair && ctx->waves_per_cu == 0 && ctx->Sp / TILE <= PB_MAX_TILES &&
-                         (uint64_t)ctx->T * (uint64_t)ctx->Sp < 0xFFFF0000ull;
+                         !ctx->scan_pair && ctx->waves_per_cu == 0 && d.pitch / TILE <= PB_MAX_TILES &&
+                         (uint64_t)ctx->T * (uint64_t)d.pitch < 0xFFFF0000ull;
     if (pb_fits && ctx->scan_method == 6)
-        return subsample ? launch_scan_pb<true>(ctx, dq, order, Q, stream) : launch_scan_pb<false>(ctx, dq, order, Q, stream);
+        return subsample ? launch_scan_pb<true>(ctx, d, dq, order, Q, stream) : launch_scan_pb<false>(ctx, d, dq, order, Q, stream);
     if (ctx->scan_wg >= 2 && Q >= ctx->wg_min_quartets && !ctx->count_invariant &&
-        (uint64_t)ctx->T * (uint64_t)ctx->Sp < 0xFFFF0000ull) {
+        (uint64_t)ctx->T * (uint64_t)d.pitch < 0xFFFF0000ull) {
         int m = ctx->scan_method < 0 ? (subsample ? 1 : 0) : ctx->scan_method;
         if (m == 6) m = subsample ? 1 : 0;
 #define TQ_WG_CASE(NW)                                                                                   \
     if (ctx->scan_wg == NW) {                                                                            \
-        if (m == 2) return launch_scan_wg<true, 2, NW>(ctx, dq, order, Q, stream);                       \
-        if (m == 3) return launch_scan_wg<true, 3, NW>(ctx, dq, order, Q, stream);                       \
-        if (NW == 4 && m == 4) return launch_scan_wg<true, 4, 4>(ctx, dq, order, Q, stream);             \
-        if (NW == 4 && m == 5) return launch_scan_wg<true, 5, 4>(ctx, dq, order, Q, stream);             \
+        if (m == 2) return launch_scan_wg<true, 2, NW>(ctx, d, dq, order, Q, stream);                       \
+        if (m == 3) return launch_scan_wg<true, 3, NW>(ctx, d, dq, order, Q, stream);                       \
+        if (NW == 4 && m == 4) return launch_scan_wg<true, 4, 4>(ctx, d, dq, order, Q, stream);             \
+        if (NW == 4 && m == 5) return launch_scan_wg<true, 5, 4>(ctx, d, dq, order, Q, stream);             \
         if (subsample)                                                                                   \
-            return m ? launch_scan_wg<true, 1, NW>(ctx, dq, order, Q, stream)                            \
-                     : launch_scan_wg<true, 0, NW>(ctx, dq, order, Q, stream);                           \
-        return m ? launch_scan_wg<false, 1, NW>(ctx, dq, order, Q, stream)                               \
-                 : launch_scan_wg<false, 0, NW>(ctx, dq, order, Q, stream);                              \
+            return m ? launch_scan_wg<true, 1, NW>(ctx, d, dq, order, Q, stream)                            \
+                     : launch_scan_wg<true, 0, NW>(ctx, d, dq, order, Q, stream);                           \
+        return m ? launch_scan_wg<false, 1, NW>(ctx, d, dq, order, Q, stream)                               \
+                 : launch_scan_wg<false, 0, NW>(ctx, d, dq, order, Q, stream);                              \
     }
         TQ_WG_CASE(2)
         if (ctx->scan_wg == 4 && ctx->park_t && m == 1 && !ctx->share_c)
-            return subsample ? launch_scan_wg<true, 1, 4, false, true>(ctx, dq, order, Q, stream)
-                             : launch_scan_wg<false, 1, 4, false, true>(ctx, dq, order, Q, stream);
+            return subsample ? launch_scan_wg<true, 1, 4, false, true>(ctx, d, dq, order, Q, stream)
+                             : launch_scan_wg<false, 1, 4, false, true>(ctx, d, dq, order, Q, stream);
         if ((ctx->scan_wg == 8 || ctx->scan_wg == 6) && ctx->park_t && m == 1 && subsample && !ctx->share_c)
-            return ctx->scan_wg == 8 ? launch_scan_wg<true, 1, 8, false, true>(ctx, dq, order, Q, stream)
-                                     : launch_scan_wg<true, 1, 6, false, true>(ctx, dq, order, Q, stream);
+            return ctx->scan_wg == 8 ? launch_scan_wg<true, 1, 8, false, true>(ctx, d, dq, order, Q, stream)
+                                     : launch_scan_wg<true, 1, 6, false, true>(ctx, d, dq, order, Q, stream);
         if (ctx->scan_wg == 4 && ctx->share_c && m <= 1) {
             if (subsample)
-                return m ? launch_scan_wg<true, 1, 4, true>(ctx, dq, order, Q, stream)
-                         : launch_scan_wg<true, 0, 4, true>(ctx, dq, order, Q, stream);
-            return m ? launch_scan_wg<false, 1, 4, true>(ctx, dq, order, Q, stream)
-                     : launch_scan_wg<false, 0, 4, true>(ctx, dq, order, Q, stream);
+                return m ? launch_scan_wg<true, 1, 4, true>(ctx, d, dq, order, Q, stream)
+                         : launch_scan_wg<true, 0, 4, true>(ctx, d, dq, order, Q, stream);
+            return m ? launch_scan_wg<false, 1, 4, true>(ctx, d, dq, order, Q, stream)
+                     : launch_scan_wg<false, 0, 4, true>(ctx, d, dq, order, Q, stream);
         }
         TQ_WG_CASE(4)
         TQ_WG_CASE(3)
@@ -627,10 +666,10 @@
 #define TQ_SCAN_CASE(N)                                                                              \
     case N:                                                                                          \
         if (method == 0)                                                                             \
-            return subsample ? launch_scan<N, true, 0>(ctx, dq, order, Q, stream)                    \
-                             : launch_scan<N, false, 0>(ctx, dq, order, Q, stream);                  \
-        return subsample ? launch_scan<N, true, 1>(ctx, dq, order, Q, stream)                        \
-                         : launch_scan<N, false, 1>(ctx, dq, order, Q, stream)
+            return subsample ? launch_scan<N, true, 0>(ctx, d, dq, order, Q, stream)                    \
+                             : launch_scan<N, false, 0>(ctx, d, dq, order, Q, stream);                  \
+        return subsample ? launch_scan<N, true, 1>(ctx, d, dq, order, Q, stream)                        \
+                         : launch_scan<N, false, 1>(ctx, d, dq, order, Q, stream)
     const int method = (ctx->scan_method < 0 || ctx->scan_method == 6) ? (subsample ? 1 : 0) : ctx->scan_method;
     switch (ctx->nrep) {
         TQ_SCAN_CASE(2);
@@ -1483,6 +1522,24 @@
     }
     ctx->locus_runs_ok = ok;
 
+    std::vector<uint32_t> pack_src;
+    if (ok && ctx->site_pack != 0 && S < 0xFFFFFFFFll) {
+        try {
+            std::vector<LocusRun> runs;
+            locus_runs(loc.data(), S, runs);
+            pack_sites(runs, pack_src);
+            if (ctx->site_pack < 0) {
+                double cost[2], trips[2];
+                const double gain_low = pack_estimate(tmparr, T, S, runs, pack_src, cost, trips);
+                const bool fits = (uint64_t)T * (uint64_t)pack_src.size() < 0xFFFF0000ull ||
+                                  (uint64_t)T * (uint64_t)align_up((size_t)S, TILE) >= 0xFFFF0000ull;
+                if (!pack_pays(gain_low) || !fits) pack_src.clear();
+            }
+        } catch (const std::bad_alloc &) {
+            return fail(ctx, TQ_ERR_OOM, "tq_set_data: out of host memory");
+        }
+    }
+
     const int64_t Sp = (int64_t)align_up((size_t)S, TILE);
     const int64_t W = Sp / 32;
     ctx->T = T; ctx->S = S; ctx->Sp = Sp; ctx->W = W;
@@ -1497,9 +1554,19 @@
     ctx->plane_cap_W = W;
     if (e == hipSuccess) e = hipMalloc((void **)&d_raw, (size_t)(T * S));
     if (e == hipSuccess) e = hipMalloc((void **)&d_loc, (size_t)S * sizeof(uint32_t));
+    uint32_t *d_src = nullptr;
+    const int64_t pSp = (int64_t)pack_src.size(), pW = pSp / 32;
+    if (pSp) {
+        if (e == hipSuccess) e = hipMalloc((void **)&ctx->pk_rows, (size_t)(T * pSp));
+        if (e == hipSuccess) e = hipMalloc((void **)&ctx->pk_nib, (size_t)(T * pSp / 2));
+        if (e == hipSuccess) e = hipMalloc((void **)&ctx->pk_planes, (size_t)(T * pW) * sizeof(uint4));
+        if (e == hipSuccess) e = hipMalloc((void **)&ctx->pk_planes3, (size_t)(T * pW * 3 + pW) * sizeof(uint32_t));
+        if (e == hipSuccess) e = hipMalloc((void **)&d_src, (size_t)pSp * sizeof(uint32_t));
+    }
     if (e != hipSuccess) {
         if (d_raw) (void)hipFree(d_raw);
         if (d_loc) (void)hipFree(d_loc);
+        if (d_src) (void)hipFree(d_src);
         free_data(ctx);
         return fail(ctx, e == hipErrorOutOfMemory ? TQ_ERR_OOM : TQ_ERR_HIP, "tq_set_data: hipMalloc failed: %s",
                     hipGetErrorString(e));
@@ -1508,20 +1575,74 @@
     if (e == hipSuccess) e = hipMemcpy(d_loc, loc.data(), (size_t)S * sizeof(uint32_t), hipMemcpyHostToDevice);
     if (e == hipSuccess) {
         const int64_t n = T * W;
-        hipLaunchKernelGGL(tq_prepare_rows, dim3((unsigned)((n + 255) / 256)), dim3(256), 0, 0, d_raw, d_loc, S, Sp,
-                           W, (int32_t)T, ctx->d_rows, ctx->d_nib, ctx->d_nib5, ctx->d_planes,
+        hipLaunchKernelGGL(tq_prepare_rows, dim3((unsigned)((n + 255) / 256)), dim3(256), 0, 0, d_raw, d_loc,
+                           (const uint32_t *)nullptr, S, Sp, W, (int32_t)T, ctx->d_rows, ctx->d_nib, ctx->d_nib5, ctx->d_planes,
                            ctx->d_planes3,
                            ctx->d_planes3 + (size_t)T * (size_t)W * 3);
         e = hipGetLastError();
+        if (e == hipSuccess && pSp) {
+            e = hipMemcpy(d_src, pack_src.data(), (size_t)pSp * sizeof(uint32_t), hipMemcpyHostToDevice);
+            if (e == hipSuccess) {
+                const int64_t np = T * pW;
+                hipLaunchKernelGGL(tq_prepare_rows, dim3((unsigned)((np + 255) / 256)), dim3(256), 0, 0, d_raw, d_loc,
+                                   (const uint32_t *)d_src, S, pSp, pW, (int32_t)T, ctx->pk_rows, ctx->pk_nib,
+                                   (uint8_t *)nullptr, ctx->pk_planes, ctx->pk_planes3,
+                                   ctx->pk_planes3 + (size_t)T * (size_t)pW * 3);
+                e = hipGetLastError();
+            }
+        }
         if (e == hipSuccess) e = hipDeviceSynchronize();
     }
     (void)hipFree(d_raw);
     (void)hipFree(d_loc);
+    if (d_src) (void)hipFree(d_src);
     if (e != hipSuccess) {
         free_data(ctx);
         return fail(ctx, TQ_ERR_HIP, "tq_set_data: %s", hipGetErrorString(e));
     }
     ctx->have_data = true;
+    if (pSp) {
+        ctx->pk_Sp = pSp;
+        ctx->pk_W = pW;
+        ctx->pk_gen = ctx->data_gen;
+    }
+    return TQ_OK;
+}
+
+int tq_pack_sites(const uint8_t *tmparr, int64_t T, int64_t S, const uint32_t *locus, int64_t locus_stride, uint32_t *src,
+                  int64_t cap, int64_t *packed_sites, int32_t *pays, double *estimate)
+{
+    if (!locus || S < 1 || S >= 0xFFFFFFFFll || locus_stride < 1 || cap < 0 || (cap > 0 && !src) || (tmparr && T < 1))
+        return TQ_ERR_INVALID_ARG;
+    try {
+        std::vector<uint32_t> loc((size_t)S);
+        std::unordered_set<uint32_t> seen;
+        for (int64_t i = 0; i < S; ++i) {
+            loc[(size_t)i] = locus[i * locus_stride];
+            if (loc[(size_t)i] == 0xFFFFFFFFu) return TQ_ERR_LOCUS_ORDER;
+            if ((!i || loc[(size_t)i] != loc[(size_t)i - 1]) && !seen.insert(loc[(size_t)i]).second) return TQ_ERR_LOCUS_ORDER;
+        }
+        std::vector<LocusRun> runs;
+        std::vector<uint32_t> map;
+        locus_runs(loc.data(), S, runs);
+        pack_sites(runs, map);
+        if (packed_sites) *packed_sites = (int64_t)map.size();
+        if (tmparr) {
+            double cost[2], trips[2];
+            const double gain_low = pack_estimate(tmparr, T, S, runs, map, cost, trips);
+            if (pays) *pays = pack_pays(gain_low) ? 1 : 0;
+            if (estimate) {
+                estimate[0] = cost[0];
+                estimate[1] = cost[1];
+                estimate[2] = trips[0];
+                estimate[3] = trips[1];
+                estimate[4] = gain_low;
+            }
+        }
+        if ((int64_t)map.size() <= cap) memcpy(src, map.data(), map.size() * sizeof(uint32_t));
+    } catch (const std::bad_alloc &) {
+        return TQ_ERR_OOM;
+    }
     return TQ_OK;
 }
 
@@ -1860,6 +1981,11 @@
     if (!strcmp(name, "scan_f4")) {
         if (value < -1 || value > 1) return fail(ctx, TQ_ERR_INVALID_ARG, "scan_f4 must be -1 (subsample mode only), 0 or 1");
         ctx->scan_f4 = (int)value;
+        return TQ_OK;
+    }
+    if (!strcmp(name, "site_pack")) {
+        if (value < -1 || value > 1) return fail(ctx, TQ_ERR_INVALID_ARG, "site_pack must be -1 (automatic), 0 or 1");
+        ctx->site_pack = (int)value;
         return TQ_OK;
     }
     if (!strcmp(name, "scan_dp")) {
@@ -2164,6 +2290,12 @@
 int tq_debug_fetch(tq_ctx *ctx, int which, void *dst, int64_t bytes)
 {
     if (!ctx || !dst || bytes < 0) return TQ_ERR_INVALID_ARG;
+    if (which == 4) {
+        const int64_t st[2] = {ctx->pk_rows ? ctx->pk_Sp : 0, scan_data(ctx, 1).rows == ctx->pk_rows && ctx->pk_rows ? 1 : 0};
+        if (bytes != (int64_t)sizeof st) return fail(ctx, TQ_ERR_INVALID_ARG, "tq_debug_fetch: which=4 takes 16 bytes");
+        memcpy(dst, st, sizeof st);
+        return TQ_OK;
+    }
     const void *src = which == 0 ? (const void *)ctx->d_cm : which == 1 ? (const void *)ctx->d_de
                       : which == 2 ? (const void *)ctx->d_sv : which == 3 ? (const void *)ctx->d_bdsqr_stats : nullptr;
     if (!src) return fail(ctx, TQ_ERR_INVALID_ARG, "tq_debug_fetch: nothing to fetch (which=%d)", which);
diff --git a/tetrad_amd/engine.py b/tetrad_amd/engine.py
--- a/tetrad_amd/engine.py
+++ b/tetrad_amd/engine.py
@@ -40,6 +40,39 @@
     n = int(np.prod(shape, dtype=np.int64)) * dtype.itemsize
     raw = np.asarray(_PinnedBlock(max(n, 1)))
     return raw[:n].view(dtype).reshape(shape)
+
+
+PACK_PAD = 0xFFFFFFFF
+
+
+def pack_sites(tmpmap: np.ndarray, tmparr: np.ndarray | None = None):
+    lib = _lib.load()
+    tm = np.asarray(tmpmap)
+    stride = tm.shape[1] if tm.ndim == 2 else 1
+    tm = np.ascontiguousarray(tm, dtype=np.uint32)
+    S = tm.shape[0]
+    arr = None
+    if tmparr is not None:
+        arr = np.ascontiguousarray(tmparr, dtype=np.uint8)
+        if arr.ndim != 2 or arr.shape[1] != S:
+            raise ValueError("tmparr must be [ntaxa, nsites] with one column per tmpmap row")
+    T = arr.shape[0] if arr is not None else 0
+    n = ctypes.c_int64()
+    pays = ctypes.c_int32(-1)
+    est = np.zeros(5, np.float64)
+
+    def call(src, cap):
+        rc = lib.tq_pack_sites(_ptr(arr), T, S, _ptr(tm), stride, _ptr(src), cap, ctypes.byref(n), ctypes.byref(pays),
+                               _ptr(est))
+        if rc != 0:
+            raise TetradHipError(rc, "tq_pack_sites failed")
+
+    call(None, 0)
+    src = np.empty(n.value, np.uint32)
+    call(src, src.shape[0])
+    if arr is None:
+        return src
+    return src, bool(pays.value), tuple(est.tolist())
 
 
 class QuartetEngine:
@@ -246,6 +279,11 @@
         self._check(self._lib.tq_debug_fetch(self._h, code, _ptr(out), out.nbytes))
         return out
 
+    def site_pack_state(self):
+        out = np.zeros(2, np.int64)
+        self._check(self._lib.tq_debug_fetch(self._h, 4, _ptr(out), out.nbytes))
+        return int(out[0]), bool(out[1])
+
     def debug_bdsqr(self, de: np.ndarray, reps: int = 5):
         de = np.ascontiguousarray(de, dtype=np.float64)
         nmat = de.shape[0]
```

New measurement: 118.2 million quartets/s, median of 6. 10.1% higher.
